# manuelbb-upb/Morbit.jl

Hardware: AMD Instinct MI355X
Metric: RBF build+solve+eval cycles/sec (higher is better)
Workload: dtype f64

## Files before the change

morbit.jl_amd/csrc/backsolve.hip:

```cpp
#include "common.hpp"

namespace mrbf {

namespace bsolve {

constexpr int NB = 128, NTHR = 512;
typedef double v2d __attribute__((ext_vector_type(2)));
typedef double v4d __attribute__((ext_vector_type(4)));
typedef __attribute__((address_space(1))) unsigned gu32;
typedef __attribute__((address_space(1))) double gf64;
typedef __attribute__((address_space(1))) v2d gv2d;

template <int KB>
struct Shared {
    double xs[2][KB][NB];
    int ok;
};

__global__ __launch_bounds__(256) void premul_kernel(const double *__restrict__ L, int64_t lda, const double *__restrict__ linv_all,
                                                     double *__restrict__ Mbuf, int nb, unsigned *__restrict__ flags, int nflags,
                                                     unsigned long long *__restrict__ xb, int nxb) {
    for (int e = blockIdx.x * 256 + threadIdx.x; e < nflags; e += gridDim.x * 256) flags[e] = 0u;
    for (int e = blockIdx.x * 256 + threadIdx.x; e < nxb; e += gridDim.x * 256) xb[e] = ~0ull;
    const int slab = blockIdx.x & 3, t = (blockIdx.x >> 2) & 1, j = blockIdx.x >> 3;
    const int i = j + 1 + t;
    if (i >= nb) return;
    const double *A = L + (int64_t)i * NB + (int64_t)j * NB * lda;
    const double *B = linv_all + (size_t)j * NB * NB;
    double *M = Mbuf + ((size_t)j * 2 + t) * NB * NB;
    const int lane = threadIdx.x & 63, wave = threadIdx.x >> 6, l15 = lane & 15, l4 = lane >> 4;
    const int i0 = 32 * wave, j0 = 32 * slab;
    v4d acc[2][2];
#pragma unroll
    for (int a = 0; a < 2; ++a)
#pragma unroll
        for (int b = 0; b < 2; ++b) acc[a][b] = (v4d){0.0, 0.0, 0.0, 0.0};
    const double *pa = A + (i0 + l15) + (int64_t)(j0 + l4) * lda;
    const double *pb = B + (j0 + l4) + (int64_t)(j0 + l15) * NB;
    constexpr int UK = 8;
    double fa0[2][UK], fa1[2][UK], fb0[2][UK], fb1[2][UK];
    auto burst = [&](int buf) {
#pragma unroll
        for (int u = 0; u < UK; ++u) {
            fa0[buf][u] = pa[(int64_t)4 * u * lda];
            fa1[buf][u] = pa[(int64_t)4 * u * lda + 16];
            fb0[buf][u] = pb[4 * u];
            fb1[buf][u] = pb[4 * u + 16 * NB];
        }
        pa += (int64_t)4 * UK * lda;
        pb += 4 * UK;
    };
    auto mma = [&](int buf) {
#pragma unroll
        for (int u = 0; u < UK; ++u) {
            acc[0][0] = __builtin_amdgcn_mfma_f64_16x16x4f64(fa0[buf][u], fb0[buf][u], acc[0][0], 0, 0, 0);
            acc[0][1] = __builtin_amdgcn_mfma_f64_16x16x4f64(fa0[buf][u], fb1[buf][u], acc[0][1], 0, 0, 0);
            acc[1][0] = __builtin_amdgcn_mfma_f64_16x16x4f64(fa1[buf][u], fb0[buf][u], acc[1][0], 0, 0, 0);
            acc[1][1] = __builtin_amdgcn_mfma_f64_16x16x4f64(fa1[buf][u], fb1[buf][u], acc[1][1], 0, 0, 0);
        }
    };
    const int nburst = (NB - j0) / (4 * UK);
    burst(0);
    for (int b = 0; b < nburst; b += 2) {
        if (b + 1 < nburst) burst(1);
        mma(0);
        if (b + 1 >= nburst) break;
        if (b + 2 < nburst) burst(0);
        mma(1);
    }
#pragma unroll
    for (int a = 0; a < 2; ++a)
#pragma unroll
        for (int b = 0; b < 2; ++b)
#pragma unroll
            for (int r = 0; r < 4; ++r) M[(i0 + 16 * a + l4 + 4 * r) + (size_t)(j0 + 16 * b + l15) * NB] = acc[a][b][r];
}

__device__ __forceinline__ void load_tile(const double *__restrict__ T, int64_t ldt, v2d (&r)[2][8]) {
    const int lane = threadIdx.x & 63, w = threadIdx.x >> 6;
    const double *p = T + (int64_t)(16 * w + 2 * (lane >> 3)) * ldt + 2 * (lane & 7);
#pragma unroll
    for (int cc = 0; cc < 2; ++cc)
#pragma unroll
        for (int u = 0; u < 8; ++u) r[cc][u] = *(const gv2d *)(p + cc * ldt + 16 * u);
}

template <int N>
__device__ __forceinline__ double shl_lanes(double v) {
    const long long b = __double_as_longlong(v);
    const int lo = __builtin_amdgcn_update_dpp((int)b, (int)b, 0x100 + N, 0xf, 0xf, false);
    const int hi = __builtin_amdgcn_update_dpp((int)(b >> 32), (int)(b >> 32), 0x100 + N, 0xf, 0xf, false);
    return __longlong_as_double(((long long)hi << 32) | (unsigned)lo);
}

template <int KB>
__device__ __forceinline__ void tile_dot(const double (*xs)[NB], const v2d (&r)[2][8], double (&out)[2][KB]) {
    const int q = threadIdx.x & 7;
    double acc[2][KB];
#pragma unroll
    for (int cc = 0; cc < 2; ++cc)
#pragma unroll
        for (int l = 0; l < KB; ++l) acc[cc][l] = 0.0;
#pragma unroll
    for (int u = 0; u < 8; ++u) {
#pragma unroll
        for (int l = 0; l < KB; ++l) {
            const v2d x = *(const v2d *)&xs[l][16 * u + 2 * q];
#pragma unroll
            for (int cc = 0; cc < 2; ++cc) acc[cc][l] = fma(r[cc][u][1], x[1], fma(r[cc][u][0], x[0], acc[cc][l]));
        }
    }
#pragma unroll
    for (int cc = 0; cc < 2; ++cc)
#pragma unroll
        for (int l = 0; l < KB; ++l) {
            double v = acc[cc][l];
            v += shl_lanes<4>(v);
            v += shl_lanes<2>(v);
            v += shl_lanes<1>(v);
            out[cc][l] = v;
        }
}

template <int KB>
__device__ __forceinline__ void await_block(Shared<KB> &sh, double (*xs)[NB], const double *glob, int i, double spec, int backoff,
                                            unsigned *abortw, unsigned epoch, unsigned long long spin_ticks, int *status, int code) {
    const int tid = threadIdx.x;
    if (tid >= KB * NB) return;
    const gf64 *src = (const gf64 *)&glob[((size_t)i * KB + tid / NB) * NB + (tid % NB)];
    double v = spec;
    if (__double_as_longlong(v) == -1ll) v = __hip_atomic_load(src, __ATOMIC_RELAXED, __HIP_MEMORY_SCOPE_AGENT);
    unsigned spins = 0;
    unsigned long long t0 = 0;
    while (__double_as_longlong(v) == -1ll) {
        if ((++spins & 63u) == 0u) {
            if (__hip_atomic_load((const gu32 *)abortw, __ATOMIC_RELAXED, __HIP_MEMORY_SCOPE_AGENT) != 0u) {
                sh.ok = 0;
                break;
            }
            const unsigned long long now = wall_clock64();
            if (t0 == 0) t0 = now;
            if (now - t0 > spin_ticks) {
                __hip_atomic_store((gu32 *)abortw, epoch, __ATOMIC_RELAXED, __HIP_MEMORY_SCOPE_AGENT);
                *(__attribute__((address_space(1))) int *)status = code + (i & 0xff);
                sh.ok = 0;
                break;
            }
        }
        for (int b = 0; b < backoff; ++b) __builtin_amdgcn_s_sleep(8);
        v = __hip_atomic_load(src, __ATOMIC_RELAXED, __HIP_MEMORY_SCOPE_AGENT);
    }
    xs[tid / NB][tid % NB] = v;
}

__device__ __forceinline__ void lds_barrier() { asm volatile("s_waitcnt lgkmcnt(0)\n\ts_barrier" ::: "memory"); }

__device__ __forceinline__ void publish(double *dst, v2d v) {
    if (__double_as_longlong(v[0]) == -1ll) v[0] = __longlong_as_double(0x7ff8000000000000ll);
    if (__double_as_longlong(v[1]) == -1ll) v[1] = __longlong_as_double(0x7ff8000000000000ll);
    asm volatile("global_store_dwordx4 %0, %1, off sc1" ::"v"(dst), "v"(v) : "memory");
}

template <int KB>
__global__ __launch_bounds__(NTHR, 1) void backsolve_persistent_kernel(const double *__restrict__ L, int64_t lda, const double *__restrict__ linv_all,
                                                                        const double *__restrict__ Mbuf, double *__restrict__ Y, int64_t ldy, int k0,
                                                                        int nb, unsigned *flags, unsigned epoch, unsigned long long spin_ticks,
                                                                        int *status, int fault, double *__restrict__ xb, double *__restrict__ zb,
                                                                        long long *stamps) {
    __shared__ __attribute__((aligned(16))) Shared<KB> sh;
    const int p = (int)blockIdx.x >> 1;
    const bool finisher = blockIdx.x & 1;
    const int j = nb - 1 - p, tid = threadIdx.x;
    const int lane = tid & 63, col = 16 * (tid >> 6) + 2 * (lane >> 3), q = lane & 7;
    unsigned *abortw = flags + (size_t)nb * 32;
    const int na = nb - 1 - j, npm = na < 2 ? na : 2, npl = na - npm;
    if (tid == 0) sh.ok = 1;
    __syncthreads();
    const double fillv = __longlong_as_double(-1ll);
    if (!finisher) {
        double w[2][KB];
#pragma unroll
        for (int cc = 0; cc < 2; ++cc)
#pragma unroll
            for (int l = 0; l < KB; ++l) w[cc][l] = *(const gf64 *)&Y[(int64_t)(k0 + l) * ldy + (int64_t)j * NB + col + cc];
        const int nst = npl + 1;
        auto fetch = [&](int s, v2d(&r)[2][8]) {
            const double *src = s < npl ? L + (int64_t)(nb - 1 - s) * NB + (int64_t)j * NB * lda : linv_all + (size_t)j * NB * NB;
            load_tile(src, s < npl ? lda : (int64_t)NB, r);
        };
        auto look = [&](int s) {
            const int i = nb - 1 - (s < npl ? s : (npl > 0 ? npl - 1 : 0));
            const int e = tid < KB * NB ? tid : 0;
            return __hip_atomic_load((const gf64 *)&xb[((size_t)i * KB + e / NB) * NB + (e % NB)], __ATOMIC_RELAXED, __HIP_MEMORY_SCOPE_AGENT);
        };
        double spec = fillv, spec2 = fillv;
        auto step = [&](int s, const v2d(&r)[2][8]) -> bool {
            double(*xs)[NB] = sh.xs[s & 1];
            if (s < npl) {
                const int i = nb - 1 - s;
                const int backoff = (i - j - 3) < 24 ? (i - j - 3) : 24;
                await_block<KB>(sh, xs, xb, i, spec, backoff, abortw, epoch, spin_ticks, status, 0x700);
                if (stamps && tid == 0 && s == npl - 1) stamps[256 * 5 + j * 4 + 0] = (long long)wall_clock64();
            } else if (q == 0) {
#pragma unroll
                for (int l = 0; l < KB; ++l) *(v2d *)&xs[l][col] = (v2d){w[0][l], w[1][l]};
            }
            spec = spec2;
            spec2 = look(s + 2);
            if (s + 2 >= npl) spec2 = fillv;
            lds_barrier();
            if (!sh.ok) return false;
            double dsum[2][KB];
            tile_dot<KB>(xs, r, dsum);
#pragma unroll
            for (int cc = 0; cc < 2; ++cc)
#pragma unroll
                for (int l = 0; l < KB; ++l) w[cc][l] = s == npl ? dsum[cc][l] : w[cc][l] - dsum[cc][l];
            return true;
        };
        v2d t0[2][8], t1[2][8], t2[2][8];
        const int o = (3 - nst % 3) % 3, G = (nst + o) / 3;
        if (0 - o >= 0) fetch(0 - o, t0);
        if (1 - o >= 0) fetch(1 - o, t1);
        fetch(2 - o, t2);
        spec = look(0);
        if (npl == 0) spec = fillv;
        spec2 = look(1);
        if (npl <= 1) spec2 = fillv;
        int g = 0;
        if (G >= 2) {
            const int s = -o;
            if (s >= 0 && !step(s, t0)) return;
            fetch(s + 3, t0);
            if (s + 1 >= 0 && !step(s + 1, t1)) return;
            fetch(s + 4, t1);
            if (!step(s + 2, t2)) return;
            fetch(s + 5, t2);
            g = 1;
        }
        for (; g < G - 1; ++g) {
            const int s = 3 * g - o;
            if (!step(s, t0)) return;
            fetch(s + 3, t0);
            if (!step(s + 1, t1)) return;
            fetch(s + 4, t1);
            if (!step(s + 2, t2)) return;
            fetch(s + 5, t2);
        }
        {
            const int s = 3 * (G - 1) - o;
            if (s >= 0 && !step(s, t0)) return;
            if (s + 1 >= 0 && !step(s + 1, t1)) return;
            if (!step(s + 2, t2)) return;
        }
        if (stamps && tid == 0) stamps[256 * 5 + j * 4 + 1] = (long long)wall_clock64();
        if (q == 0) {
#pragma unroll
            for (int l = 0; l < KB; ++l) publish(&zb[((size_t)j * KB + l) * NB + col], (v2d){w[0][l], w[1][l]});
        }
        return;
    }
    v2d tm2[2][8], tm1[2][8];
    if (npm == 2) load_tile(Mbuf + ((size_t)j * 2 + 1) * NB * NB, NB, tm2);
    if (npm >= 1) load_tile(Mbuf + (size_t)j * 2 * NB * NB, NB, tm1);
    double acc[2][KB];
#pragma unroll
    for (int cc = 0; cc < 2; ++cc)
#pragma unroll
        for (int l = 0; l < KB; ++l) acc[cc][l] = 0.0;
    if (npm == 2) {
        await_block<KB>(sh, sh.xs[0], xb, j + 2, fillv, 1, abortw, epoch, spin_ticks, status, 0x700);
        lds_barrier();
        if (!sh.ok) return;
        if (stamps && tid == 0) stamps[256 * 5 + j * 4 + 3] = (long long)wall_clock64();
        tile_dot<KB>(sh.xs[0], tm2, acc);
    }
    v2d zj[KB];
    if (q == 0) {
        unsigned spins = 0;
        unsigned long long t0 = 0;
#pragma unroll
        for (int l = 0; l < KB; ++l) {
            const double *src = &zb[((size_t)j * KB + l) * NB + col];
            while (true) {
                v2d v;
                asm volatile("global_load_dwordx4 %0, %1, off sc1\n\ts_waitcnt vmcnt(0)" : "=v"(v) : "v"(src) : "memory");
                if (__double_as_longlong(v[0]) != -1ll && __double_as_longlong(v[1]) != -1ll) {
                    zj[l] = v;
                    break;
                }
                if ((++spins & 63u) == 0u) {
                    if (__hip_atomic_load((const gu32 *)abortw, __ATOMIC_RELAXED, __HIP_MEMORY_SCOPE_AGENT) != 0u) {
                        sh.ok = 0;
                        break;
                    }
                    const unsigned long long now = wall_clock64();
                    if (t0 == 0) t0 = now;
                    if (now - t0 > spin_ticks) {
                        __hip_atomic_store((gu32 *)abortw, epoch, __ATOMIC_RELAXED, __HIP_MEMORY_SCOPE_AGENT);
                        *(__attribute__((address_space(1))) int *)status = 0x600 + (j & 0xff);
                        sh.ok = 0;
                        break;
                    }
                }
                __builtin_amdgcn_s_sleep(2);
            }
            if (!sh.ok) break;
        }
    }
    if (stamps && tid == 0) stamps[256 * 5 + j * 4 + 2] = (long long)wall_clock64();
    double last[2][KB];
#pragma unroll
    for (int cc = 0; cc < 2; ++cc)
#pragma unroll
        for (int l = 0; l < KB; ++l) last[cc][l] = 0.0;
    if (npm >= 1) {
        if (stamps && tid == 0) stamps[256 * 4 + j] = (long long)wall_clock64();
        await_block<KB>(sh, sh.xs[1], xb, j + 1, fillv, 0, abortw, epoch, spin_ticks, status, 0x700);
        if (stamps && tid == 0) stamps[j * 4 + 0] = (long long)wall_clock64();
        lds_barrier();
        if (!sh.ok) return;
        if (stamps && tid == 0) stamps[j * 4 + 1] = (long long)wall_clock64();
        tile_dot<KB>(sh.xs[1], tm1, last);
    } else {
        lds_barrier();
        if (!sh.ok) return;
    }
    if ((fault & 1) && j == nb / 2) return;
    if (stamps && tid == 0) stamps[j * 4 + 2] = (long long)wall_clock64();
    if (q == 0) {
#pragma unroll
        for (int l = 0; l < KB; ++l) {
            const v2d v = (v2d){(zj[l][0] - acc[0][l]) - last[0][l], (zj[l][1] - acc[1][l]) - last[1][l]};
            publish(&xb[((size_t)j * KB + l) * NB + col], v);
            *(v2d *)&Y[(int64_t)(k0 + l) * ldy + (int64_t)j * NB + col] = v;
        }
    }
}

}

int backsolve_blocked(mrbf_ctx *ctx, int64_t npad, const double *L, int64_t lda, const double *linv_all, double *Y, int64_t ldy, int k);

int backsolve_persistent(mrbf_ctx *ctx, int64_t npad, const double *L, int64_t lda, const double *linv_all, double *Y, int64_t ldy, int k,
                         int *status) {
    using namespace bsolve;
    const int nb = (int)(npad / NB);
    static const int force_old = mrbf_env("MRBF_BACKSOLVE_LAUNCHES") ? atoi(mrbf_env("MRBF_BACKSOLVE_LAUNCHES")) : 0;
    const int ncu = ctx->ncu;
    if (force_old || nb < 3 || nb > ncu || (lda & 1) || (reinterpret_cast<uintptr_t>(L) & 15))
        return backsolve_blocked(ctx, npad, L, lda, linv_all, Y, ldy, k);
    unsigned *flags;
    MRBF_TRY(get_buf(ctx, S_BSOLVE_FLAGS, (size_t)(nb + 1) * 32, &flags));
    const unsigned long long spin_ticks = (unsigned long long)std::max(1, ctx->spin_ms) * 100000ull;
    const int fault = (ctx->debug_fault & 2) ? 1 : 0;
    double *xb, *Mbuf;
    MRBF_TRY(get_buf(ctx, S_BSOLVE_X, (size_t)2 * nb * 4 * NB, &xb));
    MRBF_TRY(get_buf(ctx, S_BSOLVE_M, (size_t)nb * 2 * NB * NB, &Mbuf));
    hipLaunchKernelGGL(premul_kernel, dim3((unsigned)(8 * (nb - 1))), dim3(256), 0, ctx->stream, L, lda, linv_all, Mbuf, nb, flags, (nb + 1) * 32,
                       reinterpret_cast<unsigned long long *>(xb), 2 * nb * 4 * NB);
    static const bool want_stamps = mrbf_env("MRBF_BSOLVE_STAMPS") && atoi(mrbf_env("MRBF_BSOLVE_STAMPS")) != 0;
    long long *stamps = nullptr;
    if (want_stamps) {
        static long long *dbg = nullptr;
        if (!dbg) MRBF_HIP(ctx, hipMalloc(&dbg, (size_t)256 * 9 * sizeof(long long)));
        stamps = dbg;
    }
    unsigned epoch = 0;
    for (int k0 = 0; k0 < k; k0 += 4) {
        const int kb = std::min(4, k - k0);
        ++epoch;
        if (k0 > 0) MRBF_HIP(ctx, hipMemsetAsync(xb, 0xff, (size_t)2 * nb * 4 * NB * sizeof(double), ctx->stream));
#define MRBF_BSP(KBV)                                                                                                          \
    hipLaunchKernelGGL((backsolve_persistent_kernel<KBV>), dim3((unsigned)(2 * nb)), dim3(NTHR), 0, ctx->stream, L, lda, linv_all, Mbuf, Y, ldy, k0, nb, \
                       flags, epoch, spin_ticks, status, fault, xb, xb + (size_t)nb * 4 * NB, stamps)
        if (kb == 1) MRBF_BSP(1); else if (kb == 2) MRBF_BSP(2); else if (kb == 3) MRBF_BSP(3); else MRBF_BSP(4);
#undef MRBF_BSP
    }
    MRBF_HIP(ctx, hipGetLastError());
    if (want_stamps) {
        std::vector<long long> h((size_t)256 * 9);
        MRBF_HIP(ctx, hipMemcpyAsync(h.data(), stamps, h.size() * sizeof(long long), hipMemcpyDeviceToHost, ctx->stream));
        MRBF_HIP(ctx, hipStreamSynchronize(ctx->stream));
        double seen = 0, bar = 0, dot = 0, hop = 0, late = 0;
        int cnt = 0;
        for (int j = 1; j + 2 < nb; ++j) {
            seen += (double)(h[j * 4 + 0] - h[(j + 1) * 4 + 2]);
            bar += (double)(h[j * 4 + 1] - h[j * 4 + 0]);
            dot += (double)(h[j * 4 + 2] - h[j * 4 + 1]);
            hop += (double)(h[j * 4 + 2] - h[(j + 1) * 4 + 2]);
            late += (double)(h[256 * 4 + j] - h[(j + 1) * 4 + 2]);
            ++cnt;
        }
        double a3 = 0, zt = 0, zs = 0, x2 = 0;
        int c2 = 0;
        for (int j = 2; j + 4 < nb; ++j) {
            const long long *S = &h[256 * 5 + j * 4];
            a3 += (double)(S[0] - h[(j + 3) * 4 + 2]);
            zt += (double)(S[1] - S[0]);
            zs += (double)(S[2] - S[1]);
            x2 += (double)(S[3] - h[(j + 2) * 4 + 2]);
            ++c2;
        }
        fprintf(stderr, "[backsolve stamps] streamer: x_{j+3} seen %.2f us after its publication, z_j published %.2f us later, finisher has z_j %.2f us "
                "later; finisher past x_{j+2} %.2f us after that block's publication\n", a3 / c2 / 100.0, zt / c2 / 100.0, zs / c2 / 100.0, x2 / c2 / 100.0);
        fprintf(stderr, "[backsolve stamps] nb %d: publish -> seen %.2f us, seen -> barrier %.2f us, barrier -> publish %.2f us, step %.2f us; "
                "the finisher starts polling %.2f us after the publication\n", nb, seen / cnt / 100.0, bar / cnt / 100.0, dot / cnt / 100.0,
                hop / cnt / 100.0, late / cnt / 100.0);
    }
    return 0;
}

}
```

morbit.jl_amd/csrc/common.hpp:

```cpp
#pragma once
#include <hip/hip_runtime.h>
#include <rocblas/rocblas.h>
#include <rocsolver/rocsolver.h>

#include <cmath>
#include <cstdlib>
#include <cstdint>
#include <cstdio>
#include <cstring>
#include <map>
#include <string>
#include <vector>

#include "../../include/mrbf.h"
#include "descent_problem.hpp"
#include "model_pool.hpp"

namespace mrbf {

struct KP {
    int kid;
    double a, b;
    double a2;
    double sgn;
    int fast;
    int ik;
    double phi0;
};
KP make_kp(int kid, double a, double b);
inline bool kp_nonsmooth(const KP &p) { return (p.kid == MRBF_CUBIC && p.a == 1.0) || (p.kid == MRBF_THIN_PLATE_SPLINE && p.ik == 1); }
int cpd_order(int kid, double a, double b);
inline int poly_dim(int d, int deg) { return deg < 0 ? 0 : (deg == 0 ? 1 : d + 1); }

enum Slot {
    S_XC = 0, S_SQ, S_MEAN, S_PHI, S_PI, S_Q1, S_W1, S_G, S_R, S_TAU, S_RHS, S_T1, S_T2, S_IPIV, S_INFO,
    S_STAGE_A, S_STAGE_B, S_STAGE_C, S_STAGE_D, S_EVAL_E, S_EVAL_A, S_EVAL_J, S_EVAL_SA, S_EVAL_XC, S_EVAL_XSQ,
    S_OUT_A, S_OUT_B, S_CHOL_WS, S_MISC, S_MEGA_JOBS, S_MEGA_FLAGS, S_MEGA_WQ, S_MEGA_IT, S_BSOLVE_FLAGS, S_MEGA_TRACE, S_MEGA_JLOG,
    S_T1W, S_PS_STATE, S_PS_STAT, S_PS_POLISH, S_BSOLVE_X, S_V0, S_QR_INV, S_DIAG_SCR, S_SMALL_WS, S_SMALL_DESC, S_SMALL_FLAGS, S_MEGA_STAT, S_BSOLVE_M, S_SMALL_CL, S_GW_PART, S_GW_RS, S_GW_GP, S_GW_M, S_CHECK_SCAL, S_TAIL_PART, S_PS_RANK, S_SD_IN, S_SD_OUT, S_SD_WS, S_NS_IN, S_NS_OUT, S_NS_WS, S_SD_STEP, S_SD_BATCH, S_AFF_BATCH, S_NS_BATCH, S_R4_BATCH, S_DB_BOX, S_DB_GATHER, S_DB_WS, S_SMALL_LU, S_EVAL_BATCH, S_HESS_WS, S_HESS_OUT, S_NSLOTS
};
}

namespace mrbf {
namespace mega {
struct Edge {
    int head, tail_c0, srows_edge, pstream_edge;
    int shalf, sh_head, sh_tail_c0;
    int tfull1;
    int xhalf;
};
struct TableParams {
    int slack, slack_chain, first, win, srows, half_cols, tail_half, tail_half_w, chainq;
    Edge edge;
};
constexpr bool operator==(const TableParams &a, const TableParams &b) {
    return a.slack == b.slack && a.slack_chain == b.slack_chain && a.first == b.first && a.win == b.win && a.srows == b.srows &&
           a.half_cols == b.half_cols && a.tail_half == b.tail_half && a.tail_half_w == b.tail_half_w && a.chainq == b.chainq &&
           a.edge.head == b.edge.head && a.edge.tail_c0 == b.edge.tail_c0 && a.edge.srows_edge == b.edge.srows_edge &&
           a.edge.pstream_edge == b.edge.pstream_edge && a.edge.shalf == b.edge.shalf && a.edge.sh_head == b.edge.sh_head &&
           a.edge.sh_tail_c0 == b.edge.sh_tail_c0 && a.edge.tfull1 == b.edge.tfull1 && a.edge.xhalf == b.edge.xhalf;
}
struct Knobs {
    int grid = 512, dedicated = 64, look = 2, quiet = 1, slack = 3, half_cols = 0, first_window = 1, wbias = 4, xhalf = 1, chainq = 0, cboost = 12, panel_dma = 1;
    int min = 256, max = 32768;
    int chain = 0, slack_chain = 0, win = 0, pstream = 0, srows = 0;
    int shalf = -1, shalf_head = -1, head = -1, tail = -1, reserve = -1, tail_half = -1, tail_half_w = -1, xchain = -1, quiet_tail = -1;
    int tfull = -1;
};
}
struct MegaTables {
    int nt, mt;
    mega::TableParams params;
    void *block, *jobs, *wq;
    int npanel, nbulk, nchainjobs, nwin;
    unsigned long long stamp;
};
struct PotrfOpts {
    int impl = 0;
    bool any_size = false;
    int xreal = 0;
    bool info_clean = false;
};
struct EvalHints {
    bool population = false;
    bool check_call = false;
    const double *pre_xq = nullptr;
};
}

struct mrbf_ctx {
    int device = 0;
    int ncu = 256;
    hipStream_t own_stream = nullptr;
    hipStream_t stream = nullptr;
    rocblas_handle blas = nullptr;
    mrbf::Buf slots[mrbf::S_NSLOTS];
    hipEvent_t ev[8] = {};
    hipStream_t panel_stream = nullptr;
    hipEvent_t evx[4] = {};
    hipStream_t bulk_stream = nullptr;
    int bulk_masked = 0;
    int bulk_grid = 384;
    mrbf::mega::Knobs mega;
    std::string err;
    std::vector<mrbf::Buf> model_pool;
    int gram_mode = 0, residual = 1, force_path = 0, chol_impl = 0, eval_impl = 0, timing = 1, diag_impl = 0, chol_window = 0;
    int spin_ms = 1000, debug_fault = 0;
    unsigned long long *mega_stat_dev = nullptr;
    long mega_stat_shape = 0;
    int mega_stat_pending = 0;
    char *pin_base = nullptr;
    size_t pin_off = 0;
    bool pin_armed = false;
    struct PinOut {
        void *user;
        const void *pin;
        size_t bytes;
    };
    std::vector<PinOut> pin_out;
    unsigned long long *hpin = nullptr;
    float last_device_ms = 0.f;
    int slow_launches = 0;
    int small_nc = 4;
    int small_cluster_ok = 0;
    int small_timeouts = 0;
    int small_fit_max_n = 512;
    int small_lu = 0;
    int live_models = 0, live_round4 = 0;
    int live_dbs = 0;
    unsigned ps_rank_epoch = 0;
    int ps_multi_off = 0;
    std::map<long, float> mega_best_ms;
    std::vector<mrbf::MegaTables> mega_tables;
    unsigned long long mega_table_clock = 0;
};

struct mrbf_model {
    int64_t n = 0, npad = 0;
    int d = 0, dpad = 0, k = 0, q = 0, deg = -1;
    mrbf::KP kp{};
    double *C = nullptr;
    double *Xc = nullptr;
    double *sq = nullptr;
    double *mean = nullptr;
    double *W = nullptr;
    double *Wc = nullptr;
    double *lam = nullptr;
    void *block = nullptr;
    size_t block_bytes = 0;
    mrbf_ctx *owner = nullptr;
    mrbf::ModelSlab *slab = nullptr;
};

struct mrbf_db {
    mrbf_ctx *ctx = nullptr;
    int d = 0, k = 0;
    int64_t n = 0, cap = 0;
    double *sites = nullptr, *values = nullptr;
};

namespace mrbf {

int fail(mrbf_ctx *ctx, int code, const char *fmt, ...);
#define MRBF_HIP(ctx, call)                                                                                  \
    do {                                                                                                      \
        hipError_t e__ = (call);                                                                              \
        if (e__ != hipSuccess)                                                                                \
            return mrbf::fail(ctx, e__ == hipErrorOutOfMemory ? MRBF_ENOMEM : MRBF_EHIP, "%s: %s (%s:%d)", #call, \
                              hipGetErrorString(e__), __FILE__, __LINE__);                                    \
    } while (0)
#define MRBF_BLAS(ctx, call)                                                                                 \
    do {                                                                                                      \
        rocblas_status s__ = (call);                                                                          \
        if (s__ != rocblas_status_success)                                                                    \
            return mrbf::fail(ctx, MRBF_EBLAS, "%s: rocblas status %d (%s:%d)", #call, (int)s__, __FILE__, __LINE__); \
    } while (0)
#define MRBF_TRY(call)             \
    do {                           \
        int rc__ = (call);         \
        if (rc__ != 0) return rc__; \
    } while (0)

int get_buf(mrbf_ctx *ctx, Slot s, size_t bytes, void **out);
template <class T>
inline int get_buf(mrbf_ctx *ctx, Slot s, size_t count, T **out) {
    return get_buf(ctx, s, count * sizeof(T), (void **)out);
}
bool is_device_ptr(const void *p);
int db_reserve(mrbf_ctx *ctx, mrbf_db *db, int64_t needed);
int stage_in(mrbf_ctx *ctx, Slot s, const double *user, size_t count, const double **dev);
int stage_out(mrbf_ctx *ctx, Slot s, double *user, size_t count, double **dev);
int finish_out(mrbf_ctx *ctx, double *user, const double *dev, size_t count);
int input_fetch(mrbf_ctx *ctx, const double *src, size_t count, double *dst);
int input_view(mrbf_ctx *ctx, const double *user, size_t count, double *&arena, const double **dev);
int output_put(mrbf_ctx *ctx, double *dst, const double *src, size_t count);
int fetch_linear_rows(mrbf_ctx *ctx, const mrbf_ps_problem *prob, int d, double *A, double *b);
descent::Shape descent_shape(const mrbf_ps_problem *prob, const mrbf_model *const *models, int64_t n_starts,
                             std::vector<descent::SlotShape> &slots);
void pin_reset(mrbf_ctx *ctx);
void pin_flush(mrbf_ctx *ctx);
void pin_discard(mrbf_ctx *ctx);
char *pin_take(mrbf_ctx *ctx, size_t bytes);
struct PinGuard {
    mrbf_ctx *ctx;
    bool flushed = false;
    explicit PinGuard(mrbf_ctx *c) : ctx(c) { pin_reset(c); }
    void flush() {
        pin_flush(ctx);
        flushed = true;
    }
    ~PinGuard() {
        if (!flushed) pin_discard(ctx);
    }
    PinGuard(const PinGuard &) = delete;
    PinGuard &operator=(const PinGuard &) = delete;
};
enum HpinSlot : int {
    HPIN_FIT_FLAGS = 0,
    HPIN_FIT_SCAL = 4,
    HPIN_SMALL_FLAGS = 8,
    HPIN_SMALL_SCAL = 12,
    HPIN_SMALL_CHK = 16,
    HPIN_RESIDUAL = 20,
    HPIN_R4_COUNT = 24,
    HPIN_MEGA_STAT = 63,
};

inline int64_t round_up(int64_t x, int64_t m) { return (x + m - 1) / m * m; }

inline const char *mrbf_env(const char *name) {
    const char *gate = std::getenv("MRBF_EXPERIMENTS");
    if (!gate || std::atoi(gate) == 0) return nullptr;
    return std::getenv(name);
}

int launch_center_pad(mrbf_ctx *ctx, const double *X, int64_t n, int d, const double *mean_or_null, double *mean_out,
                      double *Xc, int64_t npad, int dpad, double *sq);
int launch_poly_matrix(mrbf_ctx *ctx, const double *C, int64_t n, int d, int q, double *Pi, int64_t ldpi);
int launch_transpose(mrbf_ctx *ctx, const double *in, int64_t rows, int64_t cols, double *out);
int launch_gram(mrbf_ctx *ctx, int mode, const double *C, const double *Xc, const double *sq, int64_t n, int64_t npad,
                int d, int dpad, const KP &kp, double *Phi, int64_t ld);
int launch_cross_gram(mrbf_ctx *ctx, const double *X, int64_t m, const double *C, int64_t n, int d, const KP &kp, double *K);
bool gram_w_applies(const mrbf_ctx *ctx, const mrbf_model *M);
int launch_gram_w(mrbf_ctx *ctx, const mrbf_model *M, double *Phi, int64_t ld, double **Wpart_out, double **rspart_out, int *nseg_out);
int launch_projection_small(mrbf_ctx *ctx, const mrbf_model *M, const double *Wpart, const double *rspart, int nseg, const double *linv,
                            const double *Q1, double *W1, double *G, double *scal, int *flags, int K2, int skip, double *PA, double *PB,
                            double *v0);
int eval_model(mrbf_ctx *ctx, const mrbf_model *M, int64_t m, const double *Xdev, double *vals_dev, double *jac_dev,
               mrbf_eval_info *info, EvalHints hints = {});
int hess_call(mrbf_ctx *ctx, const mrbf_model *M, int64_t m, const double *X, const std::vector<int32_t> &rows, double *hess_out,
              mrbf_hess_info *info, int64_t stage_bytes);
int potrf_blocked_tall(mrbf_ctx *ctx, int64_t ncols, int64_t mrows, double *A, int64_t lda, int *dinfo, double *linv_all, PotrfOpts opt = {});
int potrf_mega_tall(mrbf_ctx *ctx, int64_t ncols, int64_t mrows, double *A, int64_t lda, int *dinfo, double *linv_all, PotrfOpts opt = {});
mega::Knobs mega_knobs_from_env();
int potrf_lower(mrbf_ctx *ctx, int impl, int64_t n, double *A, int64_t lda, int *info_host);
int fit_model(mrbf_ctx *ctx, mrbf_model *M, const double *Ydev, mrbf_fit_info *info);
int build_model_shell(mrbf_ctx *ctx, int64_t n, int d, int k, const double *Cdev, int kid, double a, double b, int deg,
                      mrbf_model **out);
void destroy_model(mrbf_ctx *ctx, mrbf_model *M);
void model_set_dims(mrbf_model *M, int64_t n, int d, int k, int kid, double a, double b, int deg);
size_t model_block_layout(const mrbf_model *M, size_t off[7]);
void model_carve(mrbf_model *M, char *base, const size_t off[7]);
int model_block_acquire(mrbf_ctx *ctx, size_t total, void **p, size_t *bytes);
void model_block_release(mrbf_ctx *ctx, void *p, size_t bytes, bool slab = false);
int fit_check(mrbf_ctx *ctx, mrbf_model *M, const double *Y, mrbf_fit_info *info);
int mega_collect_stat(mrbf_ctx *ctx);
int mega_stat_enqueue(mrbf_ctx *ctx);
int mega_stat_finish(mrbf_ctx *ctx);

}
```

morbit.jl_amd/csrc/eval_fused.hip:

```cpp
#include <type_traits>

#include "radial.hpp"
#ifndef MRBF_EVAL_DBG
#define MRBF_EVAL_DBG 0
#endif
#include "small.hpp"

namespace mrbf {

typedef double v4d __attribute__((ext_vector_type(4)));
typedef double v2d __attribute__((ext_vector_type(2)));

constexpr int EQ = 64;
constexpr int EC = 64;

template <int KID, bool FAST, int KOUT, bool JAC, bool FINAL>
__global__ __launch_bounds__(256, 2) void eval_fused_kernel(EvalDesc one, const EvalDesc *__restrict__ many, int l0) {
    constexpr int D = 64, DT = D / 16, LDC = D + 2;
    __shared__ __attribute__((aligned(16))) double Cs[EC * LDC];
    __shared__ double Ws[KOUT * EC];
    __shared__ double Sq[EC];
    const EvalDesc &E = many ? many[blockIdx.z] : one;
    if (many && ((int64_t)blockIdx.x * EQ >= E.mpad || (int)blockIdx.y >= E.nsplit)) return;
    const double *__restrict__ Xq = E.Xq;
    const double *__restrict__ Cc = E.Cc;
    const double *__restrict__ csq = E.csq;
    const double *__restrict__ Wc = E.Wc;
    const int64_t npad = E.npad, mpad = E.mpad;
    const int tiles_per_split = E.tiles_per_split;
    const KP kp = E.kp;
    const int tid = threadIdx.x, lane = tid & 63, wave = tid >> 6;
    const int l15 = lane & 15, l4 = lane >> 4;
    const int64_t q0 = (int64_t)blockIdx.x * EQ;
    const int split = blockIdx.y;
    const int64_t qrow = q0 + wave * 16 + l15;

    double xb[D / 4];
#pragma unroll
    for (int s = 0; s < D / 4; ++s) xb[s] = Xq[qrow * D + 4 * s + l4];
    const double xs = E.xsq[qrow];

    v4d JT[KOUT][DT];
    double vsum[KOUT], sasum[KOUT];
#pragma unroll
    for (int l = 0; l < KOUT; ++l) {
        vsum[l] = 0.0;
        sasum[l] = 0.0;
#pragma unroll
        for (int t = 0; t < DT; ++t) JT[l][t] = (v4d){0.0, 0.0, 0.0, 0.0};
    }

    const int64_t c_begin = (int64_t)split * tiles_per_split * EC;
    const int ntiles_all = E.ntiles;
    const int nsub = __builtin_amdgcn_readfirstlane(E.nsub);
    const int my_tiles = min(tiles_per_split, ntiles_all - split * tiles_per_split);
    constexpr int NLD = 2 * DT;
    v2d stg[NLD];
    auto load_tile = [&](int64_t c0) {
        const v2d *src = reinterpret_cast<const v2d *>(Cc + c0 * D);
#pragma unroll
        for (int u = 0; u < NLD; ++u) stg[u] = src[tid + 256 * u];
    };
    auto store_tile = [&]() {
#pragma unroll
        for (int u = 0; u < NLD; ++u) {
            const int e = (tid + 256 * u) * 2;
            const int row = e / D, col = e % D;
            *(v2d *)&Cs[row * LDC + col] = stg[u];
        }
    };
    constexpr int NSC = ((KOUT + 1) * EC + 255) / 256;
    double stg_s[NSC];
    auto load_scalars = [&](int64_t c0) {
#pragma unroll
        for (int u = 0; u < NSC; ++u) {
            const int e = tid + 256 * u;
            if (e < EC)
                stg_s[u] = csq[c0 + e];
            else if (e < (KOUT + 1) * EC)
                stg_s[u] = Wc[(int64_t)(l0 + (e - EC) / EC) * npad + c0 + ((e - EC) % EC)];
        }
    };
    load_tile(c_begin);
    load_scalars(c_begin);
    for (int tile = 0; tile < my_tiles; ++tile) {
        const int64_t c0 = c_begin + (int64_t)tile * EC;
        __syncthreads();
        store_tile();
#pragma unroll
        for (int u = 0; u < NSC; ++u) {
            const int e = tid + 256 * u;
            if (e < EC)
                Sq[e] = stg_s[u];
            else if (e < (KOUT + 1) * EC)
                Ws[e - EC] = stg_s[u];
        }
        __syncthreads();
        if (tile + 1 < my_tiles) {
            load_tile(c0 + EC);
            load_scalars(c0 + EC);
        }
#pragma unroll
        for (int ct = 0; ct < 4; ++ct) {
            if ((int)(c0 >> 4) + ct >= nsub) break;
            v4d S = {0.0, 0.0, 0.0, 0.0};
            const double *crow = &Cs[(16 * ct + l15) * LDC + l4];
#pragma unroll
            for (int s = 0; s < D / 4; ++s) S = __builtin_amdgcn_mfma_f64_16x16x4f64(crow[4 * s], xb[s], S, 0, 0, 0);
            v4d Aw[KOUT];
#pragma unroll
            for (int r = 0; r < 4; ++r) {
                const int c = 16 * ct + l4 + 4 * r;
                double s2 = fma(-2.0, S[r], xs + Sq[c]);
                s2 = s2 > 0.0 ? s2 : 0.0;
                double phi, psi;
                rbf_phi_psi_t<KID, FAST>(s2, kp, phi, psi);
#pragma unroll
                for (int l = 0; l < KOUT; ++l) {
                    const double w = Ws[l * EC + c];
                    vsum[l] = fma(w, phi, vsum[l]);
                    if constexpr (JAC) {
                        const double a = w * psi;
                        sasum[l] += a;
                        Aw[l][r] = a;
                    }
                }
            }
            if (JAC) {
#pragma unroll
                for (int tt = 0; tt < DT; ++tt) {
#pragma unroll
                    for (int s = 0; s < 4; ++s) {
                        const double cop = Cs[(16 * ct + 4 * s + l4) * LDC + 16 * tt + l15];
#pragma unroll
                        for (int l = 0; l < KOUT; ++l) JT[l][tt] = __builtin_amdgcn_mfma_f64_16x16x4f64(cop, Aw[l][s], JT[l][tt], 0, 0, 0);
                    }
                }
            }
        }
    }
#pragma unroll
    for (int l = 0; l < KOUT; ++l) {
        vsum[l] += __shfl_xor(vsum[l], 16);
        vsum[l] += __shfl_xor(vsum[l], 32);
        sasum[l] += __shfl_xor(sasum[l], 16);
        sasum[l] += __shfl_xor(sasum[l], 32);
    }
    if constexpr (!FINAL) {
        double *__restrict__ vpart = E.vpart, *__restrict__ sapart = E.sapart, *__restrict__ gpart = E.gpart;
        if (l4 == 0) {
#pragma unroll
            for (int l = 0; l < KOUT; ++l) {
                vpart[((int64_t)split * mpad + qrow) * KOUT + l] = vsum[l];
                sapart[((int64_t)split * mpad + qrow) * KOUT + l] = sasum[l];
            }
        }
        if (JAC) {
            __syncthreads();
            double *T = Cs + wave * 16 * LDC;
#pragma unroll
            for (int l = 0; l < KOUT; ++l) {
#pragma unroll
                for (int tt = 0; tt < DT; ++tt)
#pragma unroll
                    for (int r = 0; r < 4; ++r) T[l15 * LDC + 16 * tt + l4 + 4 * r] = JT[l][tt][r];
                __syncthreads();
                for (int e = lane; e < 16 * D; e += 64) {
                    const int qq = e / D, t = e % D;
                    gpart[(((int64_t)split * mpad + q0 + wave * 16 + qq) * KOUT + l) * D + t] = T[qq * LDC + t];
                }
                __syncthreads();
            }
        }
    } else {
        const int d = E.d, k = E.k, q = E.q;
        const int64_t m = E.m;
        const double *__restrict__ lam = E.lam;
        double *__restrict__ vals = E.vals;
        double *__restrict__ jac = E.jac;
        if (vals) {
            __syncthreads();
            double *Lm = Cs;
            for (int e = tid; e < (KOUT + 1) * D; e += 256) {
                const int l = e / D, t = e % D;
                Lm[e] = (t < d && q > 1) ? (l < KOUT ? (l0 + l < k ? lam[(int64_t)(t + 1) * k + l0 + l] : 0.0) : E.mean[t]) : 0.0;
            }
            __syncthreads();
#pragma unroll
            for (int l = 0; l < KOUT; ++l) {
                double acc = 0.0, cst = 0.0;
#pragma unroll
                for (int s = 0; s < D / 4; ++s) acc = fma(Lm[l * D + 4 * s + l4], xb[s], acc);
                for (int t = lane; t < D; t += 64) cst = fma(Lm[l * D + t], Lm[KOUT * D + t], cst);
                for (int off = 32; off > 0; off >>= 1) cst += __shfl_xor(cst, off);
                acc += __shfl_xor(acc, 16);
                acc += __shfl_xor(acc, 32);
                double v = vsum[l];
                if (q > 0 && l0 + l < k) v += lam[l0 + l];
                if (q > 1) v += acc + cst;
                if (l4 == 0 && qrow < m && l0 + l < k) vals[qrow * k + l0 + l] = v;
            }
        }
        if (JAC && jac) {
            __syncthreads();
            double *T = Cs + wave * 16 * LDC;
            double *SA = Ws;
#pragma unroll
            for (int l = 0; l < KOUT; ++l)
                if (l4 == 0) SA[l * EQ + wave * 16 + l15] = sasum[l];
#pragma unroll
            for (int l = 0; l < KOUT; ++l) {
#pragma unroll
                for (int tt = 0; tt < DT; ++tt)
#pragma unroll
                    for (int r = 0; r < 4; ++r) T[l15 * LDC + 16 * tt + l4 + 4 * r] = JT[l][tt][r];
                __syncthreads();
                if (l0 + l < k) {
                    for (int e = lane; e < 16 * D; e += 64) {
                        const int qq = e / D, t = e % D;
                        const int64_t row = q0 + wave * 16 + qq;
                        if (row < m && t < d) {
                            double v = fma(SA[l * EQ + wave * 16 + qq], Xq[row * D + t], -T[qq * LDC + t]);
                            if (q > 1) v += lam[(int64_t)(t + 1) * k + l0 + l];
                            jac[row * (int64_t)k * d + (int64_t)t * k + l0 + l] = v;
                        }
                    }
                }
                __syncthreads();
            }
        }
    }
}

template <int KID, bool FAST, int KOUT, int H, int ECT, bool JAC, bool FINAL>
__global__ __launch_bounds__(512, 2) void eval_fused_split_kernel(EvalDesc one, const EvalDesc *__restrict__ many, int l0) {
    constexpr int D = 2 * H, LDC = D + 2, LDT = 65, NCT = ECT / 16, HT = H / 16;
    static_assert(8 * 16 * LDT <= ECT * LDC + 2 * 8 * 256, "epilogue transpose area");
    __shared__ __attribute__((aligned(16))) double smem[ECT * LDC + 2 * 8 * 256];
    double *Cs = smem;
    double *Sx = smem + ECT * LDC;
    __shared__ double Ws[KOUT * ECT];
    __shared__ double Sq[ECT];
    const EvalDesc &E = many ? many[blockIdx.z] : one;
    if (many && ((int64_t)blockIdx.x * EQ >= E.mpad || (int)blockIdx.y >= E.nsplit)) return;
    const double *__restrict__ Xq = E.Xq;
    const double *__restrict__ Cc = E.Cc;
    const double *__restrict__ csq = E.csq;
    const double *__restrict__ Wc = E.Wc;
    const int64_t npad = E.npad, mpad = E.mpad;
    const KP kp = E.kp;
    const int tid = threadIdx.x, lane = tid & 63, wave = tid >> 6, grp = wave >> 2, qw = wave & 3;
    const int l15 = lane & 15, l4 = lane >> 4;
    const int64_t q0 = (int64_t)blockIdx.x * EQ;
    const int split = blockIdx.y;
    const int64_t qrow = q0 + qw * 16 + l15;
    double xb[H / 4];
#pragma unroll
    for (int s = 0; s < H / 4; ++s) xb[s] = Xq[qrow * D + H * grp + 4 * s + l4];
    const double xs = E.xsq[qrow];
    v4d JT[KOUT][HT];
    double vsum[KOUT], sasum[KOUT];
#pragma unroll
    for (int l = 0; l < KOUT; ++l) {
        vsum[l] = 0.0;
        sasum[l] = 0.0;
#pragma unroll
        for (int t = 0; t < HT; ++t) JT[l][t] = (v4d){0.0, 0.0, 0.0, 0.0};
    }
    const int64_t c_begin = (int64_t)split * E.tiles_per_split * EC;
    const int ntiles_all = E.ntiles;
    const int nsub = __builtin_amdgcn_readfirstlane(E.nsub);
    const int my_tiles = min(E.tiles_per_split, ntiles_all - split * E.tiles_per_split) * (EC / ECT);
    constexpr int NLD = ECT * D / 2 / 512;
    v2d stg[NLD];
    auto load_tile = [&](int64_t c0) {
        const v2d *src = reinterpret_cast<const v2d *>(Cc + c0 * D);
#pragma unroll
        for (int u = 0; u < NLD; ++u) stg[u] = src[tid + 512 * u];
    };
    auto store_tile = [&]() {
#pragma unroll
        for (int u = 0; u < NLD; ++u) {
            const int e = (tid + 512 * u) * 2;
            const int row = e / D, col = e % D;
            *(v2d *)&Cs[row * LDC + col] = stg[u];
        }
    };
    static_assert((KOUT + 1) * ECT <= 512, "one staged scalar per thread");
    double stg_w = 0.0;
    auto load_scalars = [&](int64_t c0) {
        if (tid < ECT)
            stg_w = csq[c0 + tid];
        else if (tid < (KOUT + 1) * ECT)
            stg_w = Wc[(int64_t)(l0 + (tid - ECT) / ECT) * npad + c0 + ((tid - ECT) % ECT)];
    };
    load_tile(c_begin);
    load_scalars(c_begin);
    for (int tile = 0; tile < my_tiles; ++tile) {
        const int64_t c0 = c_begin + (int64_t)tile * ECT;
        __syncthreads();
        store_tile();
        if (tid < ECT)
            Sq[tid] = stg_w;
        else if (tid < (KOUT + 1) * ECT)
            Ws[tid - ECT] = stg_w;
        __syncthreads();
        if (tile + 1 < my_tiles) {
            load_tile(c0 + ECT);
            load_scalars(c0 + ECT);
        }
#pragma unroll
        for (int ct = 0; ct < NCT; ++ct) {
            if ((int)(c0 >> 4) + ct >= nsub) break;
            v4d Sp = {0.0, 0.0, 0.0, 0.0};
            const double *crow = &Cs[(16 * ct + l15) * LDC + H * grp + l4];
#pragma unroll
            for (int s = 0; s < H / 4; ++s) Sp = __builtin_amdgcn_mfma_f64_16x16x4f64(crow[4 * s], xb[s], Sp, 0, 0, 0);
            const int par = (tile * NCT + ct) & 1;
            double *mine = &Sx[(par * 8 + wave) * 256];
            const double *theirs = &Sx[(par * 8 + (wave ^ 4)) * 256];
#pragma unroll
            for (int r = 0; r < 4; ++r) mine[r * 64 + lane] = Sp[r];
            __syncthreads();
            v4d S;
#pragma unroll
            for (int r = 0; r < 4; ++r) {
                const double o = theirs[r * 64 + lane];
                S[r] = grp == 0 ? Sp[r] + o : o + Sp[r];
            }
            v4d Aw[KOUT];
#pragma unroll
            for (int r = 0; r < 4; ++r) {
                const int c = 16 * ct + l4 + 4 * r;
                double s2 = fma(-2.0, S[r], xs + Sq[c]);
                s2 = s2 > 0.0 ? s2 : 0.0;
                double phi, psi;
                rbf_phi_psi_t<KID, FAST>(s2, kp, phi, psi);
#pragma unroll
                for (int l = 0; l < KOUT; ++l) {
                    const double w = Ws[l * ECT + c];
                    vsum[l] = fma(w, phi, vsum[l]);
                    if constexpr (JAC) {
                        const double a = w * psi;
                        sasum[l] += a;
                        Aw[l][r] = a;
                    }
                }
            }
            if (JAC && !(MRBF_EVAL_DBG & 2)) {
#pragma unroll
                for (int tt = 0; tt < HT; ++tt) {
#pragma unroll
                    for (int s = 0; s < 4; ++s) {
                        const double cop = Cs[(16 * ct + 4 * s + l4) * LDC + H * grp + 16 * tt + l15];
#pragma unroll
                        for (int l = 0; l < KOUT; ++l) JT[l][tt] = __builtin_amdgcn_mfma_f64_16x16x4f64(cop, Aw[l][s], JT[l][tt], 0, 0, 0);
                    }
                }
            }
        }
    }
#pragma unroll
    for (int l = 0; l < KOUT; ++l) {
        vsum[l] += __shfl_xor(vsum[l], 16);
        vsum[l] += __shfl_xor(vsum[l], 32);
        sasum[l] += __shfl_xor(sasum[l], 16);
        sasum[l] += __shfl_xor(sasum[l], 32);
    }
    const int d = E.d, k = E.k, q = E.q;
    const int64_t m = E.m;
    const double *__restrict__ lam = E.lam;
    double *__restrict__ vals = E.vals;
    double *__restrict__ jac = E.jac;
    if constexpr (!FINAL) {
        if (l4 == 0 && grp == 0) {
#pragma unroll
            for (int l = 0; l < KOUT; ++l) {
                E.vpart[((int64_t)split * mpad + qrow) * KOUT + l] = vsum[l];
                E.sapart[((int64_t)split * mpad + qrow) * KOUT + l] = sasum[l];
            }
        }
    } else if (vals) {
        __syncthreads();
        double *Lm = Sx;
        double *Pp = Sx + (KOUT + 1) * D;
        for (int e = tid; e < (KOUT + 1) * D; e += 512) {
            const int l = e / D, t = e % D;
            Lm[e] = (t < d && q > 1) ? (l < KOUT ? (l0 + l < k ? lam[(int64_t)(t + 1) * k + l0 + l] : 0.0) : E.mean[t]) : 0.0;
        }
        __syncthreads();
        double accs[KOUT], csts[KOUT];
#pragma unroll
        for (int l = 0; l < KOUT; ++l) {
            double acc = 0.0, cst = 0.0;
#pragma unroll
            for (int s = 0; s < H / 4; ++s) acc = fma(Lm[l * D + H * grp + 4 * s + l4], xb[s], acc);
            for (int t = lane; t < D; t += 64) cst = fma(Lm[l * D + t], Lm[KOUT * D + t], cst);
            for (int off = 32; off > 0; off >>= 1) cst += __shfl_xor(cst, off);
            acc += __shfl_xor(acc, 16);
            acc += __shfl_xor(acc, 32);
            accs[l] = acc;
            csts[l] = cst;
            if (grp == 1 && l4 == 0) Pp[l * EQ + qw * 16 + l15] = acc;
        }
        __syncthreads();
        if (grp == 0 && l4 == 0 && qrow < m) {
#pragma unroll
            for (int l = 0; l < KOUT; ++l) {
                if (l0 + l >= k) continue;
                double v = vsum[l];
                if (q > 0) v += lam[l0 + l];
                if (q > 1) v += (accs[l] + Pp[l * EQ + qw * 16 + l15]) + csts[l];
                vals[qrow * k + l0 + l] = v;
            }
        }
    }
    if (JAC && (!FINAL || jac) && !(MRBF_EVAL_DBG & 1)) {
        __syncthreads();
        double *T = smem + wave * 16 * LDT;
        double *SA = Ws;
        __shared__ double SAs[KOUT * EQ];
        SA = SAs;
        if (FINAL && grp == 0 && l4 == 0) {
#pragma unroll
            for (int l = 0; l < KOUT; ++l) SA[l * EQ + qw * 16 + l15] = sasum[l];
        }
        bool paired = false;
        if constexpr (FINAL && KOUT == 2)
            paired = (k & 1) == 0 && (l0 & 1) == 0 && l0 + 1 < k && !(MRBF_EVAL_DBG & 64) &&
                     (((uintptr_t)jac | (uintptr_t)lam) & 15) == 0;
        if constexpr (FINAL && KOUT == 2) {
            if (paired) {
                constexpr int LDP = 33;
                static_assert(8 * 2 * 16 * LDP <= ECT * LDC + 2 * 8 * 256, "paired Jacobian transpose area");
                double *T2 = smem + wave * (2 * 16 * LDP);
#pragma unroll
                for (int hq = 0; hq < H / 32; ++hq) {
#pragma unroll
                    for (int l = 0; l < 2; ++l)
#pragma unroll
                        for (int tt = 0; tt < 2; ++tt)
#pragma unroll
                            for (int r = 0; r < 4; ++r) T2[(l * 16 + l15) * LDP + 16 * tt + l4 + 4 * r] = JT[l][2 * hq + tt][r];
                    __syncthreads();
                    for (int e = lane; e < 16 * 32; e += 64) {
                        const int qq = e >> 5, t = e & 31, col = H * grp + 32 * hq + t;
                        const int64_t row = q0 + qw * 16 + qq;
                        if (row < m && col < d) {
                            const double x = Xq[row * D + col];
                            v2d v;
                            v.x = fma(SA[qw * 16 + qq], x, -T2[qq * LDP + t]);
                            v.y = fma(SA[EQ + qw * 16 + qq], x, -T2[(16 + qq) * LDP + t]);
                            if (q > 1) {
                                const v2d lm = *(const v2d *)&lam[(int64_t)(col + 1) * k + l0];
                                v.x += lm.x;
                                v.y += lm.y;
                            }
                            *(v2d *)&jac[row * (int64_t)k * d + (int64_t)col * k + l0] = v;
                        }
                    }
                    __syncthreads();
                }
            }
        }
#pragma unroll
        for (int l = 0; l < KOUT; ++l) {
            if (paired) break;
#pragma unroll
            for (int hc = 0; hc < H / 64; ++hc) {
#pragma unroll
                for (int tt = 0; tt < 4; ++tt)
#pragma unroll
                    for (int r = 0; r < 4; ++r) T[l15 * LDT + 16 * tt + l4 + 4 * r] = JT[l][4 * hc + tt][r];
                __syncthreads();
                for (int e = lane; e < 16 * 64; e += 64) {
                    const int qq = e / 64, t = e % 64, col = H * grp + 64 * hc + t;
                    const int64_t row = q0 + qw * 16 + qq;
                    if constexpr (!FINAL) {
                        E.gpart[(((int64_t)split * mpad + row) * KOUT + l) * D + col] = T[qq * LDT + t];
                    } else {
                        if (l0 + l < k && row < m && col < d) {
                            double v = fma(SA[l * EQ + qw * 16 + qq], Xq[row * D + col], -T[qq * LDT + t]);
                            if (q > 1) v += lam[(int64_t)(col + 1) * k + l0 + l];
                            jac[row * (int64_t)k * d + (int64_t)col * k + l0 + l] = v;
                        }
                    }
                }
                __syncthreads();
            }
        }
    }
}

template <int KID, bool FAST, int KOUT>
__global__ __launch_bounds__(512, 1) void eval_vals256_kernel(EvalDesc one, const EvalDesc *__restrict__ many, int l0) {
    constexpr int D = 256, H = 128, ECT = 32, LDC = D + 2, NCT = ECT / 16, EQW = 128;
    __shared__ __attribute__((aligned(16))) double Cs[ECT * LDC];
    __shared__ double Ws[KOUT * ECT];
    __shared__ double Sq[ECT];
    const EvalDesc &E = many ? many[blockIdx.z] : one;
    if (many && ((int64_t)blockIdx.x * EQW >= E.mpad || (int)blockIdx.y >= E.nsplit)) return;
    const double *__restrict__ Xq = E.Xq;
    const double *__restrict__ Cc = E.Cc;
    const double *__restrict__ csq = E.csq;
    const double *__restrict__ Wc = E.Wc;
    const int64_t npad = E.npad, mpad = E.mpad;
    const KP kp = E.kp;
    const int tid = threadIdx.x, lane = tid & 63, wave = tid >> 6;
    const int l15 = lane & 15, l4 = lane >> 4;
    const int64_t q0 = (int64_t)blockIdx.x * EQW;
    const int split = blockIdx.y;
    const int64_t qrow = q0 + wave * 16 + l15;
    const bool qin = qrow < mpad;
    const int64_t qld = qin ? qrow : mpad - 1;
    double xb[D / 4];
#pragma unroll
    for (int s = 0; s < D / 4; ++s) xb[s] = Xq[qld * D + 4 * s + l4];
    const double xs = E.xsq[qld];
    double vsum[KOUT];
#pragma unroll
    for (int l = 0; l < KOUT; ++l) vsum[l] = 0.0;
    const int64_t c_begin = (int64_t)split * E.tiles_per_split * EC;
    const int nsub = __builtin_amdgcn_readfirstlane(E.nsub);
    const int my_tiles = min(E.tiles_per_split, E.ntiles - split * E.tiles_per_split) * (EC / ECT);
    constexpr int NLD = ECT * D / 2 / 512;
    v2d stg[NLD];
    auto load_tile = [&](int64_t c0) {
        const v2d *src = reinterpret_cast<const v2d *>(Cc + c0 * D);
#pragma unroll
        for (int u = 0; u < NLD; ++u) stg[u] = src[tid + 512 * u];
    };
    static_assert((KOUT + 1) * ECT <= 512, "one staged scalar per thread");
    double stg_w = 0.0;
    auto load_scalars = [&](int64_t c0) {
        if (tid < ECT)
            stg_w = csq[c0 + tid];
        else if (tid < (KOUT + 1) * ECT)
            stg_w = Wc[(int64_t)(l0 + (tid - ECT) / ECT) * npad + c0 + ((tid - ECT) % ECT)];
    };
    load_tile(c_begin);
    load_scalars(c_begin);
    for (int tile = 0; tile < my_tiles; ++tile) {
        const int64_t c0 = c_begin + (int64_t)tile * ECT;
        __syncthreads();
#pragma unroll
        for (int u = 0; u < NLD; ++u) {
            const int e = (tid + 512 * u) * 2;
            *(v2d *)&Cs[(e / D) * LDC + (e % D)] = stg[u];
        }
        if (tid < ECT)
            Sq[tid] = stg_w;
        else if (tid < (KOUT + 1) * ECT)
            Ws[tid - ECT] = stg_w;
        __syncthreads();
        if (tile + 1 < my_tiles) {
            load_tile(c0 + ECT);
            load_scalars(c0 + ECT);
        }
#pragma unroll
        for (int ct = 0; ct < NCT; ++ct) {
            if ((int)(c0 >> 4) + ct >= nsub) break;
            v4d S0 = {0.0, 0.0, 0.0, 0.0}, S1 = {0.0, 0.0, 0.0, 0.0};
            const double *crow = &Cs[(16 * ct + l15) * LDC + l4];
#pragma unroll
            for (int s = 0; s < H / 4; ++s) {
                S0 = __builtin_amdgcn_mfma_f64_16x16x4f64(crow[4 * s], xb[s], S0, 0, 0, 0);
                S1 = __builtin_amdgcn_mfma_f64_16x16x4f64(crow[H + 4 * s], xb[H / 4 + s], S1, 0, 0, 0);
            }
#pragma unroll
            for (int r = 0; r < 4; ++r) {
                const int c = 16 * ct + l4 + 4 * r;
                double s2 = fma(-2.0, S0[r] + S1[r], xs + Sq[c]);
                s2 = s2 > 0.0 ? s2 : 0.0;
                double phi, psi;
                rbf_phi_psi_t<KID, FAST>(s2, kp, phi, psi);
#pragma unroll
                for (int l = 0; l < KOUT; ++l) vsum[l] = fma(Ws[l * ECT + c], phi, vsum[l]);
            }
        }
    }
#pragma unroll
    for (int l = 0; l < KOUT; ++l) {
        vsum[l] += __shfl_xor(vsum[l], 16);
        vsum[l] += __shfl_xor(vsum[l], 32);
    }
    if (l4 == 0 && qin) {
#pragma unroll
        for (int l = 0; l < KOUT; ++l) {
            E.vpart[((int64_t)split * mpad + qrow) * KOUT + l] = vsum[l];
            E.sapart[((int64_t)split * mpad + qrow) * KOUT + l] = 0.0;
        }
    }
}

template <int KOUT>
__global__ __launch_bounds__(128) void eval_combine_kernel(EvalDesc one, const EvalDesc *__restrict__ many, int l0, int D) {
    const EvalDesc &E = many ? many[blockIdx.y] : one;
    const int64_t p = blockIdx.x, m = E.m, mpad = E.mpad;
    if (p >= m) return;
    const double *__restrict__ vpart = E.vpart, *__restrict__ sapart = E.sapart, *__restrict__ gpart = E.gpart;
    const double *__restrict__ Xq = E.Xq, *__restrict__ Xorig = E.X, *__restrict__ lam = E.lam;
    double *__restrict__ vals = E.vals, *__restrict__ jac = E.jac;
    const int nsplit = E.nsplit, d = E.d, k = E.k, q = E.q;
    __shared__ double sa[KOUT], sv[KOUT];
    __shared__ double pdot[KOUT][128];
    const int tid = threadIdx.x;
    if (tid < KOUT && l0 + tid < k) {
        double v = 0.0, a = 0.0;
        for (int s0 = 0; s0 < nsplit; s0 += 8) {
            double xv[8], xa[8];
#pragma unroll
            for (int u = 0; u < 8; ++u) {
                xv[u] = s0 + u < nsplit ? vpart[((int64_t)(s0 + u) * mpad + p) * KOUT + tid] : 0.0;
                xa[u] = s0 + u < nsplit ? sapart[((int64_t)(s0 + u) * mpad + p) * KOUT + tid] : 0.0;
            }
#pragma unroll
            for (int u = 0; u < 8; ++u)
                if (s0 + u < nsplit) {
                    v += xv[u];
                    a += xa[u];
                }
        }
        sa[tid] = a;
        sv[tid] = v;
    }
    if (vals && q > 1) {
#pragma unroll
        for (int l = 0; l < KOUT; ++l) {
            double acc = 0.0;
            if (l0 + l < k)
                for (int t = tid; t < d; t += 128) acc = fma(lam[(int64_t)(t + 1) * k + l0 + l], Xorig[p * d + t], acc);
            pdot[l][tid] = acc;
        }
    }
    __syncthreads();
    if (vals && tid < KOUT && l0 + tid < k) {
        double v = sv[tid];
        if (q > 0) v += lam[l0 + tid];
        if (q > 1) {
            const int nt = d < 128 ? d : 128;
            double dsum = 0.0;
            for (int t = 0; t < nt; ++t) dsum += pdot[tid][t];
            v += dsum;
        }
        vals[p * k + l0 + tid] = v;
    }
    for (int e = tid; e < KOUT * d; e += blockDim.x) {
        const int l = e / d, t = e % d;
        if (l0 + l >= k) continue;
        double g = 0.0;
        for (int s0 = 0; s0 < nsplit; s0 += 8) {
            double x[8];
#pragma unroll
            for (int u = 0; u < 8; ++u) x[u] = s0 + u < nsplit ? gpart[(((int64_t)(s0 + u) * mpad + p) * KOUT + l) * D + t] : 0.0;
#pragma unroll
            for (int u = 0; u < 8; ++u)
                if (s0 + u < nsplit) g += x[u];
        }
        double v = fma(sa[l], Xq[p * D + t], -g);
        if (q > 1) v += lam[(int64_t)(t + 1) * k + l0 + l];
        jac[p * (int64_t)k * d + (int64_t)t * k + l0 + l] = v;
    }
}

template <int KOUT>
__global__ __launch_bounds__(256) void eval_combine_vals_kernel(EvalDesc one, const EvalDesc *__restrict__ many, int l0) {
    const EvalDesc &E = many ? many[blockIdx.y] : one;
    const int lane = threadIdx.x & 63, wave = threadIdx.x >> 6;
    const int64_t p = (int64_t)blockIdx.x * 4 + wave, m = E.m, mpad = E.mpad;
    const bool active = p < m;
    const double *__restrict__ vpart = E.vpart, *__restrict__ Xorig = E.X, *__restrict__ lam = E.lam;
    const int nsplit = E.nsplit, d = E.d, k = E.k, q = E.q;
    __shared__ double pdot[4][KOUT][128];
    double v = 0.0;
    if (active && lane < KOUT && l0 + lane < k) {
        for (int s0 = 0; s0 < nsplit; s0 += 8) {
            double x[8];
#pragma unroll
            for (int u = 0; u < 8; ++u) x[u] = s0 + u < nsplit ? vpart[((int64_t)(s0 + u) * mpad + p) * KOUT + lane] : 0.0;
#pragma unroll
            for (int u = 0; u < 8; ++u)
                if (s0 + u < nsplit) v += x[u];
        }
    }
    if (q > 1) {
#pragma unroll
        for (int l = 0; l < KOUT; ++l)
#pragma unroll
            for (int h = 0; h < 2; ++h) {
                const int t0 = lane + 64 * h;
                double acc = 0.0;
                if (active && l0 + l < k)
                    for (int t = t0; t < d; t += 128) acc = fma(lam[(int64_t)(t + 1) * k + l0 + l], Xorig[p * d + t], acc);
                pdot[wave][l][t0] = acc;
            }
    }
    __syncthreads();
    if (active && lane < KOUT && l0 + lane < k) {
        if (q > 0) v += lam[l0 + lane];
        if (q > 1) {
            const int nt = d < 128 ? d : 128;
            double dsum = 0.0;
            for (int t = 0; t < nt; ++t) dsum += pdot[wave][lane][t];
            v += dsum;
        }
        if (E.vals) E.vals[p * k + l0 + lane] = v;
    }
}

__global__ void center_pad_batch_kernel(const EvalDesc *__restrict__ many, int Dfixed) {
    const EvalDesc &E = many[blockIdx.y];
    const int D = Dfixed > 0 ? Dfixed : (E.d <= 64 ? 64 : 128);
    const int lane = threadIdx.x & 63;
    const int64_t row = (int64_t)blockIdx.x * (blockDim.x >> 6) + (threadIdx.x >> 6);
    if (row >= E.mpad) return;
    double s = 0.0;
    for (int t = lane; t < D; t += 64) {
        double v = 0.0;
        if (row < E.m && t < E.d) v = E.X[row * E.d + t] - E.mean[t];
        E.Xq[row * D + t] = v;
        s = fma(v, v, s);
    }
    for (int off = 32; off > 0; off >>= 1) s += __shfl_xor(s, off);
    if (lane == 0) E.xsq[row] = s;
}

int eval_nsplit(const mrbf_ctx *ctx, int64_t m, int ntiles, bool check_call, bool population) {
    const int64_t mpad = round_up(m, EQ);
    const int slots = 2 * ctx->ncu;
    const int64_t qtiles = mpad / EQ;
    constexpr int small_split = 8;
    const bool small_batch = !check_call && qtiles * 8 <= slots;
    if (ntiles >= 4 && ntiles <= 8 && small_batch) return std::min(small_split, ntiles);
    if (population && !check_call && ntiles >= 4 && ntiles <= 8 && qtiles * 2 <= slots) return (int)std::min<int64_t>(ntiles, slots / qtiles);
    if (ntiles <= 8) return 1;
    constexpr double comb_small = 0.1, comb = 0.75;
    int nsplit = 1;
    double best_cost = 1e300;
    for (int s = 1; s <= std::min(ntiles, 32); ++s) {
        const int tps_s = (ntiles + s - 1) / s;
        if ((int64_t)(s - 1) * tps_s >= ntiles) continue;
        const double rounds = std::ceil((double)(qtiles * s) / slots);
        const double cost = rounds * tps_s + (small_batch ? comb_small : comb) * s;
        if (cost < best_cost) {
            best_cost = cost;
            nsplit = s;
        }
    }
    const int force_split = mrbf_env("MRBF_EVAL_NSPLIT") ? atoi(mrbf_env("MRBF_EVAL_NSPLIT")) : 0;
    if (force_split > 0 && force_split <= ntiles && (int64_t)(force_split - 1) * ((ntiles + force_split - 1) / force_split) < ntiles)
        nsplit = force_split;
    return nsplit;
}

int outputs_per_pass(int k, int D, bool want_jac) { return (k < 2 || (D == 256 && want_jac)) ? 1 : 2; }

template <int KID, bool FAST, int KOUT, bool JAC, bool FINAL>
static int launch_pass(mrbf_ctx *ctx, int D, dim3 grid, dim3 cgrid, const EvalDesc &one, const EvalDesc *many, int l0) {
    hipStream_t st = ctx->stream;
    if (D == 64) {
        hipLaunchKernelGGL((eval_fused_kernel<KID, FAST, KOUT, JAC, FINAL>), grid, dim3(256), 0, st, one, many, l0);
    } else if (D == 128) {
        hipLaunchKernelGGL((eval_fused_split_kernel<KID, FAST, KOUT, 64, 64, JAC, FINAL>), grid, dim3(512), 0, st, one, many, l0);
    } else if constexpr (JAC && KOUT == 1) {
        hipLaunchKernelGGL((eval_fused_split_kernel<KID, FAST, 1, 128, 32, true, FINAL>), grid, dim3(512), 0, st, one, many, l0);
    } else if constexpr (JAC) {
        return fail(ctx, MRBF_EHIP, "eval_fused: a pass with Jacobians at D = 256 carries one output");
    } else if constexpr (FINAL) {
        hipLaunchKernelGGL((eval_fused_split_kernel<KID, FAST, KOUT, 128, 32, false, true>), grid, dim3(512), 0, st, one, many, l0);
    } else {
        hipLaunchKernelGGL((eval_vals256_kernel<KID, FAST, KOUT>), dim3((grid.x + 1) / 2, grid.y, grid.z), dim3(512), 0, st, one, many, l0);
    }
    if constexpr (!FINAL && JAC)
        hipLaunchKernelGGL(eval_combine_kernel<KOUT>, cgrid, dim3(128), 0, st, one, many, l0, D);
    else if constexpr (!FINAL)
        hipLaunchKernelGGL(eval_combine_vals_kernel<KOUT>, dim3((cgrid.x + 3) / 4, cgrid.y), dim3(256), 0, st, one, many, l0);
    return 0;
}

template <class F>
static int with_bool(bool b, F &&f) {
    return b ? f(std::true_type{}) : f(std::false_type{});
}

static int run_passes(mrbf_ctx *ctx, const KP &kp, int D, int k, bool want_jac, bool final_, dim3 grid, dim3 cgrid, const EvalDesc &one,
                      const EvalDesc *many) {
    const int KO = outputs_per_pass(k, D, want_jac);
    for (int l0 = 0; l0 < k; l0 += KO) {
        const bool two = std::min(KO, k - l0) == 2;
        MRBF_DISPATCH_KID(kp.kid, {
            constexpr bool HAS_FAST = KID == MRBF_MULTIQUADRIC || KID == MRBF_INV_MULTIQUADRIC || KID == MRBF_CUBIC;
            MRBF_TRY(with_bool(HAS_FAST && kp.fast, [&](auto fast) {
                return with_bool(two, [&](auto two_) {
                    return with_bool(want_jac, [&](auto jac) {
                        return with_bool(final_, [&](auto fin) {
                            return launch_pass<KID, HAS_FAST && decltype(fast)::value, decltype(two_)::value ? 2 : 1, decltype(jac)::value, decltype(fin)::value>(
                                ctx, D, grid, cgrid, one, many, l0);
                        });
                    });
                });
            }));
        });
    }
    MRBF_HIP(ctx, hipGetLastError());
    return 0;
}

int center_pad_batch(mrbf_ctx *ctx, const EvalDesc *dev_descs, int count, int64_t max_mpad) {
    if (count <= 0 || max_mpad <= 0) return 0;
    hipLaunchKernelGGL(center_pad_batch_kernel, dim3((unsigned)((max_mpad + 3) / 4), (unsigned)count), dim3(256), 0, ctx->stream, dev_descs, 0);
    MRBF_HIP(ctx, hipGetLastError());
    return 0;
}

constexpr int DIFF_CH = 256;

__device__ __forceinline__ void nonsmooth_phi_psi(const KP &p, double s, double &phi, double &psi) {
    if (s <= 0.0) {
        phi = 0.0;
        psi = 0.0;
    } else if (p.kid == MRBF_CUBIC) {
        const double r = sqrt(s);
        phi = p.sgn * r;
        psi = p.sgn / r;
    } else {
        const double lg = log(s);
        phi = p.sgn * s * (0.5 * lg);
        psi = p.sgn * (lg + 1.0);
    }
}

__global__ __launch_bounds__(256) void eval_diff_kernel(EvalDesc one, const EvalDesc *__restrict__ many, int want_jac) {
    extern __shared__ double dsm[];
    const EvalDesc &E = many ? many[blockIdx.y] : one;
    const int64_t p = blockIdx.x, n = E.n, npad = E.npad;
    if (p >= E.m) return;
    const int d = E.d, k = E.k, q = E.q;
    const double *__restrict__ C = E.C, *__restrict__ Wc = E.Wc, *__restrict__ lam = E.lam;
    double *__restrict__ vals = E.vals, *__restrict__ jac = want_jac ? E.jac : nullptr;
    const KP kp = E.kp;
    double *xs = dsm, *ph = dsm + d, *ps = ph + DIFF_CH;
    const int tid = threadIdx.x, lane = tid & 63, wave = tid >> 6;
    for (int t = tid; t < d; t += 256) xs[t] = E.X[p * d + t];
    __syncthreads();
    if (vals)
        for (int l = tid; l < k; l += 256) {
            double v = q > 0 ? lam[l] : 0.0;
            if (q > 1)
                for (int t = 0; t < d; ++t) v = fma(lam[(int64_t)(t + 1) * k + l], xs[t], v);
            vals[p * k + l] = v;
        }
    if (jac)
        for (int64_t e = tid; e < (int64_t)k * d; e += 256) jac[p * (int64_t)k * d + e] = q > 1 ? lam[k + e] : 0.0;
    for (int64_t c0 = 0; c0 < n; c0 += DIFF_CH) {
        const int nc = (int)min((int64_t)DIFF_CH, n - c0);
        __syncthreads();
        for (int ci = wave; ci < nc; ci += 4) {
            const double *cr = C + (c0 + ci) * d;
            double s = 0.0;
            for (int t = lane; t < d; t += 64) {
                const double df = xs[t] - cr[t];
                s = fma(df, df, s);
            }
            for (int off = 32; off > 0; off >>= 1) s += __shfl_xor(s, off);
            if (lane == 0) nonsmooth_phi_psi(kp, s, ph[ci], ps[ci]);
        }
        __syncthreads();
        if (vals)
            for (int l = tid; l < k; l += 256) {
                const double *w = Wc + (int64_t)l * npad + c0;
                double v = vals[p * k + l];
                for (int ci = 0; ci < nc; ++ci) v = fma(w[ci], ph[ci], v);
                vals[p * k + l] = v;
            }
        if (jac)
            for (int64_t e = tid; e < (int64_t)k * d; e += 256) {
                const int t = (int)(e / k), l = (int)(e % k);
                const double *w = Wc + (int64_t)l * npad + c0;
                const double x = xs[t];
                double g = jac[p * (int64_t)k * d + e];
                for (int ci = 0; ci < nc; ++ci) g = fma(w[ci] * ps[ci], x - C[(c0 + ci) * d + t], g);
                jac[p * (int64_t)k * d + e] = g;
            }
    }
}

static int launch_eval_diff(mrbf_ctx *ctx, int64_t max_m, int max_d, const EvalDesc &one, const EvalDesc *many, int count, bool want_jac) {
    if (max_m <= 0 || count <= 0) return 0;
    const size_t lds = ((size_t)max_d + 2 * DIFF_CH) * sizeof(double);
    hipLaunchKernelGGL(eval_diff_kernel, dim3((unsigned)max_m, (unsigned)count), dim3(256), lds, ctx->stream, one, many, want_jac ? 1 : 0);
    MRBF_HIP(ctx, hipGetLastError());
    return 0;
}

int eval_diff(mrbf_ctx *ctx, const mrbf_model *M, int64_t m, const double *X, double *vals, double *jac) {
    EvalDesc E;
    std::memset(&E, 0, sizeof(E));
    eval_desc_model(E, M, m, 1);
    E.X = X;
    E.vals = vals;
    E.jac = jac;
    return launch_eval_diff(ctx, m, M->d, E, nullptr, 1, jac != nullptr);
}

int eval_fused_batch(mrbf_ctx *ctx, const KP &kp, int D, int k, bool want_jac, const EvalDesc *host_descs, const EvalDesc *dev_descs, int count,
                     bool centred) {
    if (count <= 0) return 0;
    if (D != 64 && D != 128 && D != 256) return fail(ctx, MRBF_EHIP, "eval_fused_batch needs dpad in {64, 128, 256}");
    for (int p = 0; p < count; ++p)
        if (kp_nonsmooth(host_descs[p].kp) != kp_nonsmooth(kp))
            return fail(ctx, MRBF_EHIP, "eval_fused_batch: descriptor %d and its group differ in kp_nonsmooth", p);
    if (kp_nonsmooth(kp)) {
        int64_t max_m = 0;
        for (int p = 0; p < count; ++p) max_m = std::max(max_m, host_descs[p].m);
        return launch_eval_diff(ctx, max_m, D, host_descs[0], dev_descs, count, want_jac);
    }
    int64_t max_mpad = 0, max_m = 0;
    int max_split = 1;
    for (int p = 0; p < count; ++p) {
        max_mpad = std::max(max_mpad, host_descs[p].mpad);
        max_m = std::max(max_m, host_descs[p].m);
        max_split = std::max(max_split, host_descs[p].nsplit);
    }
    if (max_split > 1)
        for (int p = 0; p < count; ++p)
            if (host_descs[p].nsplit == 1 && host_descs[p].m > 0)
                return fail(ctx, MRBF_EHIP, "eval_fused_batch: descriptor %d is unsplit in a group that splits the centre range", p);
    if (!centred)
        hipLaunchKernelGGL(center_pad_batch_kernel, dim3((unsigned)((max_mpad + 3) / 4), (unsigned)count), dim3(256), 0, ctx->stream, dev_descs, D);
    dim3 grid((unsigned)(max_mpad / EQ), (unsigned)max_split, (unsigned)count);
    dim3 cgrid((unsigned)max_m, (unsigned)count);
    return run_passes(ctx, kp, D, k, want_jac, max_split == 1, grid, cgrid, host_descs[0], dev_descs);
}

int eval_fused(mrbf_ctx *ctx, const mrbf_model *M, int64_t m, const double *X, double *vals, double *jac, mrbf_eval_info *info, EvalHints hints) {
    const int d = M->d, k = M->k;
    const int D = (M->dpad <= 64) ? 64 : (M->dpad <= 128 ? 128 : 256);
    if (M->dpad > 256) return fail(ctx, MRBF_EHIP, "eval_fused supports d <= 256");
    if (D != M->dpad) return fail(ctx, MRBF_EHIP, "eval_fused needs dpad in {64, 128, 256} (got %d)", M->dpad);
    const int64_t mpad = round_up(m, EQ);
    const int ntiles = (int)((M->n + EC - 1) / EC);
    const int nsplit = eval_nsplit(ctx, m, ntiles, hints.check_call, hints.population);
    const int KO = outputs_per_pass(k, D, jac != nullptr);
    EvalDesc E;
    std::memset(&E, 0, sizeof(E));
    eval_desc_model(E, M, m, nsplit);
    E.X = X;
    MRBF_TRY(get_buf(ctx, S_EVAL_XC, (size_t)mpad * D, &E.Xq));
    MRBF_TRY(get_buf(ctx, S_EVAL_XSQ, (size_t)mpad, &E.xsq));
    if (nsplit > 1) {
        MRBF_TRY(get_buf(ctx, S_EVAL_SA, (size_t)nsplit * mpad * KO * 2, &E.vpart));
        E.sapart = E.vpart + (size_t)nsplit * mpad * KO;
        if (jac) MRBF_TRY(get_buf(ctx, S_EVAL_J, (size_t)nsplit * mpad * KO * D, &E.gpart));
    }
    E.vals = vals;
    E.jac = jac;
    const bool timing = ctx->timing && info;
    if (timing) MRBF_HIP(ctx, hipEventRecord(ctx->ev[4], ctx->stream));
    if (!(hints.pre_xq && hints.pre_xq == E.Xq)) MRBF_TRY(launch_center_pad(ctx, X, m, d, M->mean, nullptr, E.Xq, mpad, D, E.xsq));
    dim3 grid((unsigned)(mpad / EQ), (unsigned)nsplit);
    MRBF_TRY(run_passes(ctx, M->kp, D, k, jac != nullptr, nsplit == 1, grid, dim3((unsigned)m), E, nullptr));
    if (timing) {
        MRBF_HIP(ctx, hipEventRecord(ctx->ev[7], ctx->stream));
        MRBF_HIP(ctx, hipEventSynchronize(ctx->ev[7]));
        float t;
        MRBF_HIP(ctx, hipEventElapsedTime(&t, ctx->ev[4], ctx->ev[7]));
        info->ms_total = t;
        info->ms_kernel = t;
    }
    return 0;
}

}
```

morbit.jl_amd/csrc/gram_fused.hip:

```cpp
#include "radial.hpp"

namespace mrbf {

typedef double v4d __attribute__((ext_vector_type(4)));
typedef double v2d __attribute__((ext_vector_type(2)));

constexpr int GW_LDT = 66;

template <int KID, bool FAST>
__global__ __launch_bounds__(256, 2) void gram_w_kernel(const double *__restrict__ Xc, const double *__restrict__ sq, int64_t n,
                                                        int64_t npad, double *__restrict__ Phi, int64_t ld, KP p, int nt, int nseg,
                                                        int seglen, double *__restrict__ Wpart, double *__restrict__ rspart, int dbg) {
    __shared__ __attribute__((aligned(16))) double T[2][64 * GW_LDT];
    __shared__ double Tsq[2][64];
    const int tid = threadIdx.x, lane = tid & 63, wave = tid >> 6;
    const int l15 = lane & 15, l4 = lane >> 4;
    const int seg = blockIdx.x % nseg, I = nt - 1 - (int)(blockIdx.x / nseg);
    const int jt0 = seg * seglen;
    const int jt1 = (jt0 + seglen < nt) ? jt0 + seglen : nt;
    const int64_t iw0 = (int64_t)I * 128 + 32 * wave;
    double bI[2][16];
#pragma unroll
    for (int it = 0; it < 2; ++it)
#pragma unroll
        for (int ks = 0; ks < 16; ++ks) bI[it][ks] = Xc[(iw0 + it * 16 + l15) * 64 + ks * 4 + l4];
    double sqi[2];
#pragma unroll
    for (int it = 0; it < 2; ++it) sqi[it] = sq[iw0 + it * 16 + l15];
    v4d wacc[4][2];
#pragma unroll
    for (int tt = 0; tt < 4; ++tt)
#pragma unroll
        for (int it = 0; it < 2; ++it) wacc[tt][it] = (v4d){0.0, 0.0, 0.0, 0.0};
    double rs[2] = {0.0, 0.0};
    const int nh = 2 * (jt1 - jt0);
    if (nh > 0) {
        const double *src = Xc + (int64_t)jt0 * 128 * 64;
        const double *ssq = sq + (int64_t)jt0 * 128;
        v2d pf[4];
        double pfsq = 0.0;
        if (tid < 64) pfsq = ssq[tid];
#pragma unroll 1
        for (int half = 0; half < 2; ++half) {
#pragma unroll
            for (int u = 0; u < 4; ++u) pf[u] = *(const v2d *)(src + (tid + 256 * (4 * half + u)) * 2);
#pragma unroll
            for (int u = 0; u < 4; ++u) {
                const int e = (tid + 256 * (4 * half + u)) * 2;
                *(v2d *)&T[0][(e >> 6) * GW_LDT + (e & 63)] = pf[u];
            }
        }
        if (tid < 64) Tsq[0][tid] = pfsq;
        __syncthreads();
#pragma unroll 1
        for (int h = 0; h < nh; ++h) {
            const int buf = h & 1;
            const double *Tb = T[buf];
            const int64_t jb = (int64_t)jt0 * 128 + 64 * h;
            const bool store = (jt0 + (h >> 1)) <= I && !(dbg & 1);
            const bool full = jb + 64 <= n && (int64_t)I * 128 + 128 <= n;
            const bool edge = jb + 64 > n || (jt0 + (h >> 1)) == I;
            const bool more = h + 1 < nh && !(dbg & 16);
            const double *s2 = src + (int64_t)(h + 1) * 64 * 64;
            if (more && tid < 64) pfsq = ssq[64 * (h + 1) + tid];
#pragma unroll 1
            for (int sub = 0; sub < 2; ++sub) {
                const double *Ts = Tb + sub * 32 * GW_LDT;
                if (more) {
#pragma unroll
                    for (int u = 0; u < 4; ++u) pf[u] = *(const v2d *)(s2 + (tid + 256 * (4 * sub + u)) * 2);
                }
                v4d acc[2][2];
#pragma unroll
                for (int jt = 0; jt < 2; ++jt)
#pragma unroll
                    for (int it = 0; it < 2; ++it) acc[jt][it] = (v4d){0.0, 0.0, 0.0, 0.0};
                if (!(dbg & 8))
#pragma unroll
                for (int ks = 0; ks < 16; ++ks) {
                    double a[2];
#pragma unroll
                    for (int jt = 0; jt < 2; ++jt) a[jt] = Ts[(jt * 16 + l15) * GW_LDT + ks * 4 + l4];
#pragma unroll
                    for (int jt = 0; jt < 2; ++jt)
#pragma unroll
                        for (int it = 0; it < 2; ++it)
                            acc[jt][it] = __builtin_amdgcn_mfma_f64_16x16x4f64(a[jt], bI[it][ks], acc[jt][it], 0, 0, 0);
                }
                if (more) {
#pragma unroll
                    for (int u = 0; u < 4; ++u) {
                        const int e = (tid + 256 * (4 * sub + u)) * 2;
                        *(v2d *)&T[buf ^ 1][(e >> 6) * GW_LDT + (e & 63)] = pf[u];
                    }
                    if (sub == 0 && tid < 64) Tsq[buf ^ 1][tid] = pfsq;
                }
                if (edge || !FAST) {
#pragma unroll
                    for (int jt = 0; jt < 2; ++jt)
#pragma unroll
                        for (int r = 0; r < 4; ++r) {
                            const int jl = sub * 32 + jt * 16 + l4 + 4 * r;
                            const int64_t gj = jb + jl;
                            const double sqj = Tsq[buf][jl];
#pragma unroll
                            for (int it = 0; it < 2; ++it) {
                                const int64_t gi = iw0 + it * 16 + l15;
                                double s = fma(-2.0, acc[jt][it][r], sqi[it] + sqj);
                                s = s > 0.0 ? s : 0.0;
                                if (gi == gj) s = 0.0;
                                double v = (dbg & 2) ? s : rbf_phi_t<KID, FAST>(s, p);
                                v = gj < n ? v : 0.0;
                                acc[jt][it][r] = v;
                                rs[it] += v;
                            }
                        }
                } else {
#pragma unroll
                    for (int jt = 0; jt < 2; ++jt)
#pragma unroll
                        for (int r = 0; r < 4; ++r) {
                            const double sqj = Tsq[buf][sub * 32 + jt * 16 + l4 + 4 * r];
#pragma unroll
                            for (int it = 0; it < 2; ++it) {
                                double s = fma(-2.0, acc[jt][it][r], sqi[it] + sqj);
                                s = s > 0.0 ? s : 0.0;
                                const double v = (dbg & 2) ? s : rbf_phi_t<KID, FAST>(s, p);
                                acc[jt][it][r] = v;
                                rs[it] += v;
                            }
                        }
                }
                if (store) {
                    double *dst = Phi + (jb + sub * 32 + l4) * ld + iw0 + l15;
                    if (full) {
#pragma unroll
                        for (int jt = 0; jt < 2; ++jt)
#pragma unroll
                            for (int r = 0; r < 4; ++r)
#pragma unroll
                                for (int it = 0; it < 2; ++it) dst[(int64_t)(jt * 16 + 4 * r) * ld + it * 16] = acc[jt][it][r];
                    } else {
#pragma unroll
                        for (int jt = 0; jt < 2; ++jt)
#pragma unroll
                            for (int r = 0; r < 4; ++r)
#pragma unroll
                                for (int it = 0; it < 2; ++it) {
                                    const int64_t gj = jb + sub * 32 + jt * 16 + l4 + 4 * r, gi = iw0 + it * 16 + l15;
                                    if (gi < n && gj < n) dst[(int64_t)(jt * 16 + 4 * r) * ld + it * 16] = acc[jt][it][r];
                                }
                    }
                }
                if (!(dbg & 4))
#pragma unroll
                for (int jt = 0; jt < 2; ++jt) {
#pragma unroll
                    for (int r = 0; r < 4; ++r) {
                        double aw[4];
#pragma unroll
                        for (int tt = 0; tt < 4; ++tt) aw[tt] = Ts[(jt * 16 + 4 * r + l4) * GW_LDT + tt * 16 + l15];
#pragma unroll
                        for (int tt = 0; tt < 4; ++tt)
#pragma unroll
                            for (int it = 0; it < 2; ++it)
                                wacc[tt][it] = __builtin_amdgcn_mfma_f64_16x16x4f64(aw[tt], acc[jt][it][r], wacc[tt][it], 0, 0, 0);
                    }
                }
            }
            __syncthreads();
        }
    }
#pragma unroll
    for (int tt = 0; tt < 4; ++tt)
#pragma unroll
        for (int r = 0; r < 4; ++r) {
            const int t = tt * 16 + l4 + 4 * r;
#pragma unroll
            for (int it = 0; it < 2; ++it) Wpart[((int64_t)seg * 64 + t) * npad + iw0 + it * 16 + l15] = wacc[tt][it][r];
        }
#pragma unroll
    for (int it = 0; it < 2; ++it) {
        double x = rs[it];
        x += __shfl_xor(x, 16);
        x += __shfl_xor(x, 32);
        if (l4 == 0) rspart[(int64_t)seg * npad + iw0 + it * 16 + l15] = x;
    }
}

__device__ __forceinline__ double sum_partials(const double *__restrict__ p, int cnt, int64_t stride) {
    double sp[8] = {0.0, 0.0, 0.0, 0.0, 0.0, 0.0, 0.0, 0.0};
    int c = 0;
    for (; c + 32 <= cnt; c += 32) {
        double v[32];
#pragma unroll
        for (int u = 0; u < 32; ++u) v[u] = p[(int64_t)(c + u) * stride];
#pragma unroll
        for (int u = 0; u < 32; ++u) sp[u & 7] += v[u];
    }
    for (; c + 8 <= cnt; c += 8) {
        double v[8];
#pragma unroll
        for (int u = 0; u < 8; ++u) v[u] = p[(int64_t)(c + u) * stride];
#pragma unroll
        for (int u = 0; u < 8; ++u) sp[u] += v[u];
    }
    for (int u = 0; c + u < cnt; ++u) sp[u] += p[(int64_t)(c + u) * stride];
    return ((sp[0] + sp[1]) + (sp[2] + sp[3])) + ((sp[4] + sp[5]) + (sp[6] + sp[7]));
}

constexpr int PJ_LS = 68;
constexpr int PJ_QP = 80;

__device__ __forceinline__ v4d pj_tile(const double *As, const double *Bs, int mt, int nt, int K, int l15, int l4) {
    v4d acc = {0.0, 0.0, 0.0, 0.0};
    const double *ap = As + (mt * 16 + l15) * PJ_LS + l4;
    const double *bp = Bs + (nt * 16 + l15) * PJ_LS + l4;
    for (int k = 0; k < K; k += 4) acc = __builtin_amdgcn_mfma_f64_16x16x4f64(ap[k], bp[k], acc, 0, 0, 0);
    return acc;
}

__global__ __launch_bounds__(256) void proj_reduce_kernel(const double *__restrict__ Wpart, const double *__restrict__ rspart, int nseg,
                                                          int64_t npad, int64_t n, int d, int q, const double *__restrict__ linv,
                                                          const double *__restrict__ Q1, double rsqrtn, double *__restrict__ W1,
                                                          double *__restrict__ Gp, double *__restrict__ trp) {
    __shared__ double Ws[64 * PJ_LS];
    __shared__ double Ls[64 * PJ_LS];
    __shared__ double W1s[PJ_QP * PJ_LS];
    __shared__ double Qs[PJ_QP * PJ_LS];
    const int tid = threadIdx.x, i = tid & 63, g = tid >> 6;
    const int lane = tid & 63, wave = tid >> 6, l15 = lane & 15, l4 = lane >> 4;
    const int64_t R0 = (int64_t)blockIdx.x * 64;
    const bool live = R0 + i < n;
    constexpr int Q4 = PJ_QP / 4;
    double qv[Q4];
#pragma unroll
    for (int u = 0; u < Q4; ++u) {
        const int a = g + 4 * u;
        qv[u] = (a < q && live) ? Q1[R0 + i + (int64_t)a * npad] : 0.0;
    }
    const double rsv = (g == 0 && live) ? sum_partials(rspart + R0 + i, nseg, npad) * rsqrtn : 0.0;
    if (q > 1) {
        double lv[16];
#pragma unroll
        for (int u = 0; u < 16; ++u) {
            const int e = tid + 256 * u, c = e & 63, t = e >> 6;
            lv[u] = (c < d && t <= c) ? linv[c + (int64_t)t * 128] : 0.0;
        }
#pragma unroll
        for (int half = 0; half < 2; ++half) {
            double sv[8] = {0.0, 0.0, 0.0, 0.0, 0.0, 0.0, 0.0, 0.0};
            for (int s0 = 0; s0 < nseg; s0 += 8) {
                double wv[8][8];
#pragma unroll
                for (int u = 0; u < 8; ++u)
#pragma unroll
                    for (int sgm = 0; sgm < 8; ++sgm) {
                        const int t = g * 16 + half * 8 + u;
                        wv[u][sgm] = s0 + sgm < nseg ? Wpart[((int64_t)(s0 + sgm) * 64 + t) * npad + R0 + i] : 0.0;
                    }
#pragma unroll
                for (int u = 0; u < 8; ++u)
                    sv[u] += ((wv[u][0] + wv[u][1]) + (wv[u][2] + wv[u][3])) + ((wv[u][4] + wv[u][5]) + (wv[u][6] + wv[u][7]));
            }
#pragma unroll
            for (int u = 0; u < 8; ++u) Ws[i * PJ_LS + (g * 16 + half * 8 + u)] = live ? sv[u] : 0.0;
        }
#pragma unroll
        for (int u = 0; u < 16; ++u) {
            const int e = tid + 256 * u;
            Ls[(e & 63) * PJ_LS + (e >> 6)] = lv[u];
        }
    }
#pragma unroll
    for (int u = 0; u < Q4; ++u) {
        const int a = g + 4 * u;
        Qs[a * PJ_LS + i] = qv[u];
        if (a > d || q == 1) W1s[a * PJ_LS + i] = 0.0;
    }
    if (g == 0) {
        W1s[i] = rsv;
        W1[R0 + i] = rsv;
    }
    __syncthreads();
    if (q > 1) {
#pragma unroll 1
        for (int tile = wave; tile < 16; tile += 4) {
            const int ct = tile >> 2, it = tile & 3;
            const v4d acc = pj_tile(Ls, Ws, ct, it, 64, l15, l4);
#pragma unroll
            for (int r = 0; r < 4; ++r) {
                const int c = ct * 16 + l4 + 4 * r, ii = it * 16 + l15;
                if (c < d) {
                    W1s[(1 + c) * PJ_LS + ii] = acc[r];
                    W1[R0 + ii + (int64_t)(1 + c) * npad] = acc[r];
                }
            }
        }
    }
    __syncthreads();
    double *out = Gp + (size_t)blockIdx.x * q * q;
    const int qt = (q + 15) >> 4;
#pragma unroll 1
    for (int tile = wave; tile < qt * qt; tile += 4) {
        const int at = tile % qt, bt = tile / qt;
        const v4d acc = pj_tile(Qs, W1s, at, bt, 64, l15, l4);
#pragma unroll
        for (int r = 0; r < 4; ++r) {
            const int a = at * 16 + l4 + 4 * r, bb = bt * 16 + l15;
            if (a < q && bb < q) out[a + bb * q] = acc[r];
            if (at == bt && a == bb && a < q) Ls[a] = acc[r];
        }
    }
    __syncthreads();
    if (tid == 0) {
        double tr = 0.0;
        for (int a = 0; a < q; ++a) tr += Ls[a];
        trp[blockIdx.x] = tr;
    }
}

__global__ __launch_bounds__(256) void proj_shift_kernel(const double *__restrict__ Gp, const double *__restrict__ trp, int nchunks, int q,
                                                         double nphi0, double nmq, double *__restrict__ G, double *__restrict__ Mh,
                                                         double *__restrict__ scal, int *__restrict__ flags) {
    __shared__ double dg[256];
    __shared__ double smu;
    const int tid = threadIdx.x;
    const size_t qq = (size_t)q * q;
    const int idx = blockIdx.x * 256 + tid;
    const double *p0 = Gp + (idx < (int)qq ? idx : 0);
    double tv = 0.0;
    for (int c = tid; c < nchunks; c += 256) tv += trp[c];
    double s0[8] = {0, 0, 0, 0, 0, 0, 0, 0};
    int c = 0;
    for (; c + 64 <= nchunks; c += 64) {
        double v0[64];
#pragma unroll
        for (int u = 0; u < 64; ++u) v0[u] = p0[(size_t)(c + u) * qq];
#pragma unroll
        for (int u = 0; u < 64; ++u) s0[u & 7] += v0[u];
    }
    for (; c < nchunks; ++c) s0[c & 7] += p0[(size_t)c * qq];
    const double gv = ((s0[0] + s0[1]) + (s0[2] + s0[3])) + ((s0[4] + s0[5]) + (s0[6] + s0[7]));
    dg[tid] = tv;
    __syncthreads();
    for (int w = 128; w > 0; w >>= 1) {
        if (tid < w) dg[tid] += dg[tid + w];
        __syncthreads();
    }
    if (tid == 0) {
        const double tr = dg[0];
        const double mu = (nphi0 - tr) / nmq;
        const bool ok = mu > 0.0 && mu < 1e300;
        smu = ok ? mu : 1.0;
        if (blockIdx.x == 0) {
            scal[0] = tr;
            scal[1] = smu;
            flags[2] = ok ? 0 : 1;
        }
    }
    __syncthreads();
    if (idx < (int)qq) {
        G[idx] = gv;
        Mh[idx] = 0.5 * gv + ((idx % q) == (idx / q) ? 0.5 * smu : 0.0);
    }
}

__global__ __launch_bounds__(256) void proj_panels_kernel(const double *__restrict__ Q1, const double *__restrict__ W1,
                                                          const double *__restrict__ Mh, int64_t n, int64_t npad, int q, int K2, int skip,
                                                          double *__restrict__ PA, double *__restrict__ PB, double *__restrict__ v0) {
    __shared__ double Qs[64 * PJ_LS];
    __shared__ double Ms[PJ_QP * PJ_LS];
    const int tid = threadIdx.x, i = tid & 63, g = tid >> 6;
    const int lane = tid & 63, wave = tid >> 6, l15 = lane & 15, l4 = lane >> 4;
    const int64_t R0 = (int64_t)blockIdx.x * 64;
    const bool live = R0 + i < n;
    constexpr int QA = 17;
    double qv[QA];
#pragma unroll
    for (int u = 0; u < QA; ++u) {
        const int a = g + 4 * u;
        qv[u] = (a < q && live) ? Q1[R0 + i + (int64_t)a * npad] : 0.0;
    }
    constexpr int ME = (PJ_QP * PJ_LS + 255) / 256;
    double mv[ME];
#pragma unroll
    for (int u = 0; u < ME; ++u) {
        const int e = tid + 256 * u, bb = e / PJ_LS, a = e % PJ_LS;
        mv[u] = (a < q && bb < q) ? Mh[a + bb * q] : 0.0;
    }
#pragma unroll
    for (int u = 0; u < ME; ++u) {
        const int e = tid + 256 * u;
        if (e < PJ_QP * PJ_LS) Ms[e] = mv[u];
    }
#pragma unroll
    for (int u = 0; u < QA; ++u) Qs[i * PJ_LS + g + 4 * u] = qv[u];
    __syncthreads();
    const int qq = q - skip, qt = (q + 15) >> 4, K = (q + 3) & ~3;
#pragma unroll 1
    for (int tile = wave; tile < qt * 4; tile += 4) {
        const int bt = tile >> 2, it = tile & 3;
        const v4d acc = pj_tile(Ms, Qs, bt, it, K, l15, l4);
        const int ii = it * 16 + l15;
        const bool lv = R0 + ii < n;
        double w1[4], qb[4];
#pragma unroll
        for (int r = 0; r < 4; ++r) {
            const int b = bt * 16 + l4 + 4 * r;
            w1[r] = (b < q && lv) ? W1[R0 + ii + (int64_t)b * npad] : 0.0;
            qb[r] = b < q ? Qs[ii * PJ_LS + b] : 0.0;
        }
#pragma unroll
        for (int r = 0; r < 4; ++r) {
            const int b = bt * 16 + l4 + 4 * r;
            if (b >= q) continue;
            const double v = lv ? w1[r] - acc[r] : 0.0;
            if (b >= skip) {
                const int c = b - skip;
                PA[R0 + ii + (int64_t)c * npad] = qb[r];
                PB[R0 + ii + (int64_t)c * npad] = v;
                PA[R0 + ii + (int64_t)(qq + c) * npad] = v;
                PB[R0 + ii + (int64_t)(qq + c) * npad] = qb[r];
            } else {
                v0[R0 + ii] = v;
            }
        }
    }
    for (int c = 2 * qq + g; c < K2; c += 4) {
        PA[R0 + i + (int64_t)c * npad] = 0.0;
        PB[R0 + i + (int64_t)c * npad] = 0.0;
    }
}

bool gram_w_applies(const mrbf_ctx *ctx, const mrbf_model *M) {
    static const int on = mrbf_env("MRBF_GRAM_FUSED") ? atoi(mrbf_env("MRBF_GRAM_FUSED")) : 1;
    if (!on || ctx->gram_mode != 0) return false;
    if (M->dpad != 64 || M->q < 1 || M->q > 65 || M->n < 1024) return false;
    if (kp_nonsmooth(M->kp)) return false;
    return M->kp.fast || M->kp.kid == MRBF_GAUSSIAN || M->kp.kid == MRBF_THIN_PLATE_SPLINE;
}

int launch_gram_w(mrbf_ctx *ctx, const mrbf_model *M, double *Phi, int64_t ld, double **Wpart_out, double **rspart_out, int *nseg_out) {
    const int nt = (int)(M->npad / 128);
    static const int dbg = mrbf_env("MRBF_GW_DBG") ? atoi(mrbf_env("MRBF_GW_DBG")) : 0;
    static const int wgs = mrbf_env("MRBF_GW_WGS") ? atoi(mrbf_env("MRBF_GW_WGS")) : 512;
    int nseg = wgs / nt;
    if (nseg < 1) nseg = 1;
    if (nseg > nt) nseg = nt;
    const int seglen = (nt + nseg - 1) / nseg;
    nseg = (nt + seglen - 1) / seglen;
    double *Wpart, *rspart;
    MRBF_TRY(get_buf(ctx, S_GW_PART, (size_t)nseg * 64 * M->npad, &Wpart));
    MRBF_TRY(get_buf(ctx, S_GW_RS, (size_t)nseg * M->npad, &rspart));
    const dim3 grid((unsigned)(nt * nseg));
    if (M->kp.fast) {
        MRBF_DISPATCH_KID(M->kp.kid, hipLaunchKernelGGL((gram_w_kernel<KID, true>), grid, dim3(256), 0, ctx->stream, M->Xc, M->sq, M->n,
                                                        M->npad, Phi, ld, M->kp, nt, nseg, seglen, Wpart, rspart, dbg));
    } else if (M->kp.kid == MRBF_GAUSSIAN) {
        hipLaunchKernelGGL((gram_w_kernel<MRBF_GAUSSIAN, false>), grid, dim3(256), 0, ctx->stream, M->Xc, M->sq, M->n, M->npad, Phi, ld,
                           M->kp, nt, nseg, seglen, Wpart, rspart, dbg);
    } else {
        hipLaunchKernelGGL((gram_w_kernel<MRBF_THIN_PLATE_SPLINE, false>), grid, dim3(256), 0, ctx->stream, M->Xc, M->sq, M->n, M->npad,
                           Phi, ld, M->kp, nt, nseg, seglen, Wpart, rspart, dbg);
    }
    MRBF_HIP(ctx, hipGetLastError());
    *Wpart_out = Wpart;
    *rspart_out = rspart;
    *nseg_out = nseg;
    return 0;
}

int launch_projection_small(mrbf_ctx *ctx, const mrbf_model *M, const double *Wpart, const double *rspart, int nseg, const double *linv,
                            const double *Q1, double *W1, double *G, double *scal, int *flags, int K2, int skip, double *PA, double *PB,
                            double *v0) {
    const int64_t n = M->n, npad = M->npad;
    const int q = M->q, nch = (int)(npad / 64);
    double *Gp, *Mh;
    MRBF_TRY(get_buf(ctx, S_GW_GP, (size_t)nch * q * q + nch, &Gp));
    MRBF_TRY(get_buf(ctx, S_GW_M, (size_t)q * q, &Mh));
    double *trp = Gp + (size_t)nch * q * q;
    hipLaunchKernelGGL(proj_reduce_kernel, dim3((unsigned)nch), dim3(256), 0, ctx->stream, Wpart, rspart, nseg, npad, n, M->d, q, linv, Q1,
                       1.0 / std::sqrt((double)n), W1, Gp, trp);
    hipLaunchKernelGGL(proj_shift_kernel, dim3((unsigned)((q * q + 255) / 256)), dim3(256), 0, ctx->stream, Gp, trp, nch, q,
                       (double)n * M->kp.phi0, (double)std::max<int64_t>(n - q, 1), G, Mh, scal, flags);
    hipLaunchKernelGGL(proj_panels_kernel, dim3((unsigned)nch), dim3(256), 0, ctx->stream, Q1, W1, Mh, n, npad, q, K2, skip, PA, PB, v0);
    MRBF_HIP(ctx, hipGetLastError());
    return 0;
}

}
```

morbit.jl_amd/csrc/prep.hip:

```cpp
#include "common.hpp"

namespace mrbf {

__global__ void column_mean_kernel(const double *__restrict__ X, int64_t n, int d, double *__restrict__ mean) {
    __shared__ double red[256];
    const int t = blockIdx.x;
    if (t >= d) {
        if (threadIdx.x == 0) mean[t] = 0.0;
        return;
    }
    double s = 0.0;
    for (int64_t i = threadIdx.x; i < n; i += blockDim.x) s += X[i * d + t];
    red[threadIdx.x] = s;
    __syncthreads();
    for (int w = 128; w > 0; w >>= 1) {
        if ((int)threadIdx.x < w) red[threadIdx.x] += red[threadIdx.x + w];
        __syncthreads();
    }
    if (threadIdx.x == 0) mean[t] = red[0] / (double)n;
}

__global__ void center_pad_kernel(const double *__restrict__ X, int64_t n, int d, const double *__restrict__ mean,
                                  double *__restrict__ Xc, int64_t npad, int dpad, double *__restrict__ sq) {
    const int lane = threadIdx.x & 63;
    const int64_t row = (int64_t)blockIdx.x * (blockDim.x >> 6) + (threadIdx.x >> 6);
    if (row >= npad) return;
    double s = 0.0;
    for (int t = lane; t < dpad; t += 64) {
        double v = 0.0;
        if (row < n && t < d) v = X[row * d + t] - mean[t];
        Xc[row * dpad + t] = v;
        s = fma(v, v, s);
    }
    for (int off = 32; off > 0; off >>= 1) s += __shfl_xor(s, off);
    if (lane == 0) sq[row] = s;
}

int launch_center_pad(mrbf_ctx *ctx, const double *X, int64_t n, int d, const double *mean_or_null, double *mean_out,
                      double *Xc, int64_t npad, int dpad, double *sq) {
    const double *mean = mean_or_null;
    if (!mean) {
        hipLaunchKernelGGL(column_mean_kernel, dim3(dpad > d ? dpad : d), dim3(256), 0, ctx->stream, X, n, d, mean_out);
        mean = mean_out;
    }
    const int rows_per_block = 4;
    hipLaunchKernelGGL(center_pad_kernel, dim3((unsigned)((npad + rows_per_block - 1) / rows_per_block)), dim3(256), 0,
                       ctx->stream, X, n, d, mean, Xc, npad, dpad, sq);
    MRBF_HIP(ctx, hipGetLastError());
    return 0;
}

__global__ void poly_matrix_kernel(const double *__restrict__ C, int64_t n, int d, int q, double *__restrict__ Pi,
                                   int64_t ld) {
    const int64_t i = (int64_t)blockIdx.x * blockDim.x + threadIdx.x;
    if (i >= n) return;
    for (int t = 0; t < q; ++t) Pi[i + (int64_t)t * ld] = (t == 0) ? 1.0 : C[i * d + (t - 1)];
}

int launch_poly_matrix(mrbf_ctx *ctx, const double *C, int64_t n, int d, int q, double *Pi, int64_t ldpi) {
    if (q <= 0 || n <= 0) return 0;
    hipLaunchKernelGGL(poly_matrix_kernel, dim3((unsigned)((n + 255) / 256)), dim3(256), 0, ctx->stream, C, n, d, q, Pi,
                       ldpi);
    MRBF_HIP(ctx, hipGetLastError());
    return 0;
}

__global__ void transpose_kernel(const double *__restrict__ in, int64_t rows, int64_t cols, double *__restrict__ out) {
    const int64_t idx = (int64_t)blockIdx.x * blockDim.x + threadIdx.x;
    if (idx >= rows * cols) return;
    const int64_t r = idx / cols, c = idx % cols;
    out[c * rows + r] = in[idx];
}

int launch_transpose(mrbf_ctx *ctx, const double *in, int64_t rows, int64_t cols, double *out) {
    if (rows * cols <= 0) return 0;
    hipLaunchKernelGGL(transpose_kernel, dim3((unsigned)((rows * cols + 255) / 256)), dim3(256), 0, ctx->stream, in, rows,
                       cols, out);
    MRBF_HIP(ctx, hipGetLastError());
    return 0;
}

}
```

morbit.jl_amd/csrc/solve.hip:

```cpp
#include "common.hpp"
#include "small.hpp"

namespace mrbf {

__global__ void fit_publish_kernel(const int *__restrict__ dinfo, const double *__restrict__ scal, const unsigned long long *__restrict__ dstat,
                                   int *__restrict__ hflags, double *__restrict__ hscal, unsigned long long *__restrict__ hstat) {
    const int t = threadIdx.x;
    if (t < 4) hflags[t] = dinfo[t];
    if (t >= 4 && t < 6 && scal) hscal[t - 4] = scal[t - 4];
    if (t == 6 && dstat && hstat) hstat[0] = dstat[0];
}

__global__ void fill_saddle_kernel(const double *__restrict__ Pi, int64_t n, int q, double *__restrict__ S, int64_t N) {
    const int64_t idx = (int64_t)blockIdx.x * blockDim.x + threadIdx.x;
    const int64_t tot = n * q;
    if (idx < tot) {
        const int64_t i = idx % n;
        const int t = (int)(idx / n);
        const double v = Pi[idx];
        S[i + (n + t) * N] = v;
        S[(n + t) + i * N] = v;
    } else if (idx < tot + (int64_t)q * q) {
        const int64_t r = idx - tot;
        S[(n + r % q) + (n + r / q) * N] = 0.0;
    }
}

__global__ void rhs_from_values_kernel(const double *__restrict__ Y, int64_t n, int k, double *__restrict__ B, int64_t N) {
    const int64_t idx = (int64_t)blockIdx.x * blockDim.x + threadIdx.x;
    if (idx >= N * k) return;
    const int64_t i = idx % N;
    const int l = (int)(idx / N);
    B[idx] = (i < n) ? Y[i * k + l] : 0.0;
}

__global__ void scatter_solution_kernel(const double *__restrict__ B, int64_t ldB, int64_t n, int64_t npad, int k, int q,
                                        int64_t lam_row0, double *__restrict__ W, double *__restrict__ Wc,
                                        double *__restrict__ lam, const double *__restrict__ lamsrc, int64_t ldlam) {
    const int64_t idx = (int64_t)blockIdx.x * blockDim.x + threadIdx.x;
    if (idx < npad * k) {
        const int64_t i = idx % npad;
        const int l = (int)(idx / npad);
        const double v = (i < n) ? B[i + l * ldB] : 0.0;
        Wc[idx] = v;
        if (i < n) W[i * k + l] = v;
    } else if (idx < npad * k + (int64_t)q * k) {
        const int64_t r = idx - npad * k;
        const int t = (int)(r % q), l = (int)(r / q);
        lam[(int64_t)t * k + l] = lamsrc[lam_row0 + t + l * ldlam];
    }
}

__global__ void copy_upper_kernel(const double *__restrict__ A, int64_t lda, int q, double *__restrict__ R) {
    const int idx = blockIdx.x * blockDim.x + threadIdx.x;
    if (idx >= q * q) return;
    const int i = idx % q, j = idx / q;
    R[idx] = (i <= j) ? A[i + (int64_t)j * lda] : 0.0;
}

__global__ void trace_kernel(const double *__restrict__ G, int q, double *__restrict__ out) {
    __shared__ double red[256];
    double s = 0.0;
    for (int i = threadIdx.x; i < q; i += 256) s += G[i + (int64_t)i * q];
    red[threadIdx.x] = s;
    __syncthreads();
    for (int w = 128; w > 0; w >>= 1) {
        if ((int)threadIdx.x < w) red[threadIdx.x] += red[threadIdx.x + w];
        __syncthreads();
    }
    if (threadIdx.x == 0) out[0] = red[0];
}

__global__ void max_abs_kernel(const double *__restrict__ v, int64_t cnt, double *__restrict__ out) {
    __shared__ double red[256];
    double s = 0.0;
    for (int64_t i = threadIdx.x; i < cnt; i += 256) s = fmax(s, fabs(v[i]));
    red[threadIdx.x] = s;
    __syncthreads();
    for (int w = 128; w > 0; w >>= 1) {
        if ((int)threadIdx.x < w) red[threadIdx.x] = fmax(red[threadIdx.x], red[threadIdx.x + w]);
        __syncthreads();
    }
    if (threadIdx.x == 0) out[0] = red[0];
}

__global__ void residual_kernel(const double *__restrict__ a, const double *__restrict__ b, int64_t cnt,
                                double *__restrict__ out) {
    __shared__ double r0[256], r1[256];
    double s0 = 0.0, s1 = 0.0;
    for (int64_t i = threadIdx.x; i < cnt; i += 256) {
        const double df = a[i] - b[i];
        s0 = fma(df, df, s0);
        s1 = fma(b[i], b[i], s1);
    }
    r0[threadIdx.x] = s0;
    r1[threadIdx.x] = s1;
    __syncthreads();
    for (int w = 128; w > 0; w >>= 1) {
        if ((int)threadIdx.x < w) {
            r0[threadIdx.x] += r0[threadIdx.x + w];
            r1[threadIdx.x] += r1[threadIdx.x + w];
        }
        __syncthreads();
    }
    if (threadIdx.x == 0) {
        out[0] = r0[0];
        out[1] = r1[0];
    }
}

static inline unsigned nblk(int64_t cnt) { return (unsigned)((cnt + 255) / 256); }

void model_block_release(mrbf_ctx *ctx, void *p, size_t bytes, bool slab) {
    if (!ctx) {
        (void)hipFree(p);
        return;
    }
    model_pool_release(ctx->model_pool, p, bytes, slab, [](void *q) { (void)hipFree(q); });
}

void destroy_model(mrbf_ctx *ctx, mrbf_model *M) {
    if (!M) return;
    if (ctx && (M->block || M->slab)) --ctx->live_models;
    if (M->block) model_block_release(ctx, M->block, M->block_bytes);
    if (M->slab && slab_drop(M->slab)) {
        model_block_release(ctx, M->slab->p, M->slab->bytes, true);
        delete M->slab;
    }
    delete M;
}

void model_set_dims(mrbf_model *M, int64_t n, int d, int k, int kid, double a, double b, int deg) {
    M->n = n;
    M->d = d;
    M->k = k;
    M->deg = deg;
    M->q = poly_dim(d, deg);
    M->npad = round_up(n, 128);
    M->dpad = (d <= 64) ? 64 : (d <= 128 ? 128 : (d <= 256 ? 256 : (int)round_up(d, 16)));
    M->kp = make_kp(kid, a, b);
}

size_t model_block_layout(const mrbf_model *M, size_t off[7]) {
    const size_t cnt[7] = {(size_t)M->n * M->d, (size_t)M->npad * M->dpad, (size_t)M->npad, (size_t)M->dpad, (size_t)M->n * M->k,
                           (size_t)M->npad * M->k, (size_t)std::max(M->q, 1) * M->k};
    size_t at = 0;
    for (int i = 0; i < 7; ++i) {
        off[i] = at;
        at += (std::max<size_t>(cnt[i], 2) * sizeof(double) + 255) & ~size_t(255);
    }
    return at;
}

void model_carve(mrbf_model *M, char *base, const size_t off[7]) {
    M->C = (double *)(base + off[0]);
    M->Xc = (double *)(base + off[1]);
    M->sq = (double *)(base + off[2]);
    M->mean = (double *)(base + off[3]);
    M->W = (double *)(base + off[4]);
    M->Wc = (double *)(base + off[5]);
    M->lam = (double *)(base + off[6]);
}

int model_block_acquire(mrbf_ctx *ctx, size_t total, void **p, size_t *bytes) {
    hipError_t e = hipSuccess;
    auto alloc = [&](size_t b) -> void * {
        void *q = nullptr;
        e = hipMalloc(&q, b);
        return e == hipSuccess ? q : nullptr;
    };
    if (!model_pool_acquire(ctx->model_pool, total, p, bytes, alloc, [](void *q) { (void)hipFree(q); }))
        return fail(ctx, MRBF_ENOMEM, "model allocation failed: %s", hipGetErrorString(e));
    return 0;
}

int build_model_shell(mrbf_ctx *ctx, int64_t n, int d, int k, const double *Cdev, int kid, double a, double b, int deg,
                      mrbf_model **out) {
    mrbf_model *M = new mrbf_model();
    model_set_dims(M, n, d, k, kid, a, b, deg);
    size_t off[7];
    const size_t total = model_block_layout(M, off);
    const int rc_block = model_block_acquire(ctx, total, &M->block, &M->block_bytes);
    if (rc_block != 0) {
        delete M;
        return rc_block;
    }
    ++ctx->live_models;
    M->owner = ctx;
    model_carve(M, (char *)M->block, off);
    auto init = [&]() -> int {
        if (Cdev != M->C)
            MRBF_HIP(ctx, hipMemcpyAsync(M->C, Cdev, (size_t)n * d * sizeof(double), hipMemcpyDeviceToDevice, ctx->stream));
        MRBF_TRY(launch_center_pad(ctx, M->C, n, d, nullptr, M->mean, M->Xc, M->npad, M->dpad, M->sq));
        return 0;
    };
    const int rc = init();
    if (rc != 0) {
        destroy_model(ctx, M);
        return rc;
    }
    *out = M;
    return 0;
}

static int read_info(mrbf_ctx *ctx, const int *dinfo, int *hinfo) {
    MRBF_HIP(ctx, hipMemcpyAsync(hinfo, dinfo, sizeof(int), hipMemcpyDeviceToHost, ctx->stream));
    MRBF_HIP(ctx, hipStreamSynchronize(ctx->stream));
    return 0;
}

void fill_small_prob(const mrbf_ctx *ctx, const mrbf_model *M, const double *Y, double *ws, int *flags, double *scal, int *cl, smallfit::Prob *P);
static int fit_lu(mrbf_ctx *ctx, mrbf_model *M, const double *Y, mrbf_fit_info *info) {
    const int64_t n = M->n, N = n + M->q;
    const int k = M->k, q = M->q;
    double *S, *B, *Pi = nullptr;
    int *ipiv, *dinfo;
    MRBF_TRY(get_buf(ctx, S_PHI, (size_t)N * N, &S));
    MRBF_TRY(get_buf(ctx, S_RHS, (size_t)N * k, &B));
    MRBF_TRY(get_buf(ctx, S_IPIV, (size_t)N, &ipiv));
    MRBF_TRY(get_buf(ctx, S_INFO, (size_t)4, &dinfo));
    hipLaunchKernelGGL(rhs_from_values_kernel, dim3(nblk(N * k)), dim3(256), 0, ctx->stream, Y, n, k, B, N);
    MRBF_HIP(ctx, hipEventRecord(ctx->ev[0], ctx->stream));
    MRBF_TRY(launch_gram(ctx, ctx->gram_mode, M->C, M->Xc, M->sq, n, M->npad, M->d, M->dpad, M->kp, S, N));
    MRBF_HIP(ctx, hipEventRecord(ctx->ev[1], ctx->stream));
    if (q > 0) {
        MRBF_TRY(get_buf(ctx, S_PI, (size_t)n * q, &Pi));
        MRBF_TRY(launch_poly_matrix(ctx, M->C, n, M->d, q, Pi, n));
        hipLaunchKernelGGL(fill_saddle_kernel, dim3(nblk(n * q + (int64_t)q * q)), dim3(256), 0, ctx->stream, Pi, n, q, S, N);
    }
    MRBF_HIP(ctx, hipGetLastError());
    MRBF_HIP(ctx, hipEventRecord(ctx->ev[5], ctx->stream));
    MRBF_BLAS(ctx, rocsolver_dgetrf(ctx->blas, (int)N, (int)N, S, (int)N, ipiv, dinfo));
    MRBF_HIP(ctx, hipEventRecord(ctx->ev[2], ctx->stream));
    int hinfo = 0;
    MRBF_TRY(read_info(ctx, dinfo, &hinfo));
    info->factor_info = hinfo;
    info->path = MRBF_PATH_LU;
    if (hinfo != 0) return fail(ctx, MRBF_ESINGULAR, "saddle matrix is singular (getrf info = %d, N = %lld)", hinfo, (long long)N);
    MRBF_BLAS(ctx, rocsolver_dgetrs(ctx->blas, rocblas_operation_none, (int)N, k, S, (int)N, ipiv, B, (int)N));
    hipLaunchKernelGGL(scatter_solution_kernel, dim3(nblk(M->npad * k + (int64_t)q * k)), dim3(256), 0, ctx->stream, B, N, n,
                       M->npad, k, q, n, M->W, M->Wc, M->lam, B, N);
    MRBF_HIP(ctx, hipGetLastError());
    MRBF_HIP(ctx, hipEventRecord(ctx->ev[3], ctx->stream));
    MRBF_HIP(ctx, hipEventSynchronize(ctx->ev[3]));
    MRBF_HIP(ctx, hipEventElapsedTime(&info->ms_gram, ctx->ev[0], ctx->ev[1]));
    MRBF_HIP(ctx, hipEventElapsedTime(&info->ms_project, ctx->ev[1], ctx->ev[5]));
    MRBF_HIP(ctx, hipEventElapsedTime(&info->ms_factor, ctx->ev[5], ctx->ev[2]));
    MRBF_HIP(ctx, hipEventElapsedTime(&info->ms_solve, ctx->ev[2], ctx->ev[3]));
    return 0;
}

static int fit_small_lu(mrbf_ctx *ctx, mrbf_model *M, const double *Y, mrbf_fit_info *info) {
    smallfit::Prob P;
    double *ws, *scal;
    int *flags;
    MRBF_TRY(get_buf(ctx, S_SMALL_LU, small_lu_scratch_doubles(M->n, M->q), &ws));
    MRBF_TRY(get_buf(ctx, S_SMALL_FLAGS, (size_t)4, &flags));
    MRBF_TRY(get_buf(ctx, S_MISC, (size_t)8, &scal));
    fill_small_prob(ctx, M, Y, ws, flags, scal, nullptr, &P);
    int hflags_local[4] = {0, 0, 0, 0};
    int *hflags = ctx->hpin ? reinterpret_cast<int *>(ctx->hpin + HPIN_SMALL_FLAGS) : hflags_local;
    MRBF_HIP(ctx, hipEventRecord(ctx->ev[0], ctx->stream));
    MRBF_TRY(launch_small_lu(ctx, &P, 1, nullptr));
    MRBF_HIP(ctx, hipEventRecord(ctx->ev[1], ctx->stream));
    MRBF_HIP(ctx, hipMemcpyAsync(hflags, flags, 4 * sizeof(int), hipMemcpyDeviceToHost, ctx->stream));
    MRBF_HIP(ctx, hipStreamSynchronize(ctx->stream));
    info->factor_info = hflags[0];
    info->path = MRBF_PATH_LU;
    if (hflags[0] != 0)
        return fail(ctx, MRBF_ESINGULAR, "saddle matrix is singular (getrf info = %d, N = %lld)", hflags[0], (long long)(M->n + M->q));
    MRBF_HIP(ctx, hipEventElapsedTime(&info->ms_factor, ctx->ev[0], ctx->ev[1]));
    return 0;
}

__global__ void scale_rows_pinv_kernel(double *__restrict__ T, int N, int k, const double *__restrict__ sv) {
    const int idx = blockIdx.x * blockDim.x + threadIdx.x;
    if (idx >= N * k) return;
    const int i = idx % N;
    const double s = sv[i], cut = (double)N * 2.220446049250313e-16 * sv[0];
    T[idx] = (s > cut) ? T[idx] / s : 0.0;
}

static int fit_minnorm(mrbf_ctx *ctx, mrbf_model *M, const double *Y, mrbf_fit_info *info) {
    const int64_t n = M->n, N = n + M->q;
    const int k = M->k, q = M->q;
    const double one = 1.0, zero = 0.0;
    double *S, *B, *Pi, *U, *VT, *sv, *E, *T;
    int *dinfo;
    MRBF_TRY(get_buf(ctx, S_PHI, (size_t)N * N, &S));
    MRBF_TRY(get_buf(ctx, S_RHS, (size_t)N * k, &B));
    MRBF_TRY(get_buf(ctx, S_PI, (size_t)n * q, &Pi));
    MRBF_TRY(get_buf(ctx, S_Q1, (size_t)N * N, &U));
    MRBF_TRY(get_buf(ctx, S_W1, (size_t)N * N, &VT));
    MRBF_TRY(get_buf(ctx, S_TAU, (size_t)2 * N, &sv));
    MRBF_TRY(get_buf(ctx, S_T1, (size_t)N * k, &T));
    MRBF_TRY(get_buf(ctx, S_INFO, (size_t)4, &dinfo));
    E = sv + N;
    hipLaunchKernelGGL(rhs_from_values_kernel, dim3(nblk(N * k)), dim3(256), 0, ctx->stream, Y, n, k, B, N);
    MRBF_HIP(ctx, hipEventRecord(ctx->ev[0], ctx->stream));
    MRBF_TRY(launch_gram(ctx, ctx->gram_mode, M->C, M->Xc, M->sq, n, M->npad, M->d, M->dpad, M->kp, S, N));
    MRBF_HIP(ctx, hipEventRecord(ctx->ev[1], ctx->stream));
    MRBF_TRY(launch_poly_matrix(ctx, M->C, n, M->d, q, Pi, n));
    hipLaunchKernelGGL(fill_saddle_kernel, dim3(nblk(n * q + (int64_t)q * q)), dim3(256), 0, ctx->stream, Pi, n, q, S, N);
    MRBF_HIP(ctx, hipGetLastError());
    MRBF_BLAS(ctx, rocsolver_dgesvd(ctx->blas, rocblas_svect_all, rocblas_svect_all, (int)N, (int)N, S, (int)N, sv, U, (int)N, VT,
                                    (int)N, E, rocblas_outofplace, dinfo));
    MRBF_HIP(ctx, hipEventRecord(ctx->ev[2], ctx->stream));
    int hinfo = 0;
    MRBF_TRY(read_info(ctx, dinfo, &hinfo));
    info->factor_info = hinfo;
    info->path = MRBF_PATH_MINNORM;
    if (hinfo != 0) return fail(ctx, MRBF_ESINGULAR, "SVD of the saddle matrix did not converge (info = %d)", hinfo);
    MRBF_BLAS(ctx, rocblas_dgemm(ctx->blas, rocblas_operation_transpose, rocblas_operation_none, (int)N, k, (int)N, &one, U, (int)N,
                                 B, (int)N, &zero, T, (int)N));
    hipLaunchKernelGGL(scale_rows_pinv_kernel, dim3(nblk(N * k)), dim3(256), 0, ctx->stream, T, (int)N, k, sv);
    MRBF_BLAS(ctx, rocblas_dgemm(ctx->blas, rocblas_operation_transpose, rocblas_operation_none, (int)N, k, (int)N, &one, VT, (int)N,
                                 T, (int)N, &zero, B, (int)N));
    hipLaunchKernelGGL(scatter_solution_kernel, dim3(nblk(M->npad * k + (int64_t)q * k)), dim3(256), 0, ctx->stream, B, N, n,
                       M->npad, k, q, n, M->W, M->Wc, M->lam, B, N);
    MRBF_HIP(ctx, hipGetLastError());
    MRBF_HIP(ctx, hipEventRecord(ctx->ev[3], ctx->stream));
    MRBF_HIP(ctx, hipEventSynchronize(ctx->ev[3]));
    MRBF_HIP(ctx, hipEventElapsedTime(&info->ms_gram, ctx->ev[0], ctx->ev[1]));
    MRBF_HIP(ctx, hipEventElapsedTime(&info->ms_factor, ctx->ev[1], ctx->ev[2]));
    MRBF_HIP(ctx, hipEventElapsedTime(&info->ms_solve, ctx->ev[2], ctx->ev[3]));
    return 0;
}

int backsolve_blocked(mrbf_ctx *ctx, int64_t npad, const double *L, int64_t lda, const double *linv_all, double *Y, int64_t ldy, int k);
int backsolve_persistent(mrbf_ctx *ctx, int64_t npad, const double *L, int64_t lda, const double *linv_all, double *Y, int64_t ldy, int k,
                         int *status);
int launch_update_lower(mrbf_ctx *ctx, const double *A, int64_t lda, const double *B, int64_t ldb, double *C, int64_t ldc, int64_t nt, int K,
                        const double *cvec, double cs, int64_t cn);
int launch_pad_identity(mrbf_ctx *ctx, double *A, int64_t n, int64_t npad, int64_t ld);
int tsmm_tn(mrbf_ctx *ctx, int64_t n, int p, int r, double alpha, const double *A, int64_t lda, const double *B, int64_t ldb, double beta,
            double *C, int64_t ldc);
int symm_panel(mrbf_ctx *ctx, int64_t n, int64_t npad, int q, const double *Phi, int64_t ld, const double *Q, int64_t ldq, double *W,
               int64_t ldwo, bool const_first, double cval);

__global__ void set_rhs_rows_kernel(double *__restrict__ A, int64_t ld, int64_t npad, int xt, const double *__restrict__ B, int k) {
    const int64_t idx = (int64_t)blockIdx.x * blockDim.x + threadIdx.x;
    if (idx >= npad * xt) return;
    const int l = (int)(idx % xt);
    const int64_t i = idx / xt;
    A[(npad + l) + i * ld] = (l < k) ? B[i + (int64_t)l * npad] : 0.0;
}
__global__ void get_rhs_rows_kernel(const double *__restrict__ A, int64_t ld, int64_t npad, double *__restrict__ B, int k) {
    const int64_t idx = (int64_t)blockIdx.x * blockDim.x + threadIdx.x;
    if (idx >= npad * k) return;
    const int l = (int)(idx % k);
    const int64_t i = idx / k;
    B[i + (int64_t)l * npad] = A[(npad + l) + i * ld];
}
__global__ void xc_to_tall_kernel(const double *__restrict__ Xc, int64_t n, int d, int dpad, double *__restrict__ Tall, int64_t lt,
                                  int64_t dq) {
    const int64_t idx = (int64_t)blockIdx.x * blockDim.x + threadIdx.x;
    if (idx >= n * d) return;
    const int64_t i = idx / d;
    const int t = (int)(idx % d);
    Tall[(dq + i) + (int64_t)t * lt] = Xc[i * dpad + t];
}
__global__ void build_q1_kernel(const double *__restrict__ Tall, int64_t lt, int64_t dq, int64_t n, int64_t npad, int q,
                                double *__restrict__ Q1) {
    const int64_t idx = (int64_t)blockIdx.x * blockDim.x + threadIdx.x;
    if (idx >= npad * q) return;
    const int64_t i = idx % npad;
    const int t = (int)(idx / npad);
    double v = 0.0;
    if (i < n) v = (t == 0) ? 1.0 / sqrt((double)n) : Tall[(dq + i) + (int64_t)(t - 1) * lt];
    Q1[idx] = v;
}
__global__ void shift_from_trace_kernel(double *__restrict__ scal, double nphi0, double nmq, int *__restrict__ flags) {
    const double mu = (nphi0 - scal[0]) / nmq;
    const bool ok = mu > 0.0 && mu < 1e300;
    scal[1] = ok ? mu : 1.0;
    flags[2] = ok ? 0 : 1;
}

__global__ void build_panels_kernel(const double *__restrict__ Q1, const double *__restrict__ W, const double *__restrict__ scal,
                                    int64_t n, int64_t npad, int q, int K2, int skip, double *__restrict__ PA, double *__restrict__ PB,
                                    double *__restrict__ v0) {
    const int64_t idx = (int64_t)blockIdx.x * blockDim.x + threadIdx.x;
    if (idx >= npad * K2) return;
    const double mu = scal[1];
    const int64_t i = idx % npad;
    const int t = (int)(idx / npad);
    const int qq = q - skip;
    double a = 0.0, b = 0.0;
    if (i < n && t < 2 * qq) {
        const int tt = t % qq + skip;
        const double qv = Q1[i + (int64_t)tt * npad];
        const double vv = fma(-0.5 * mu, qv, W[i + (int64_t)tt * npad]);
        a = (t < qq) ? qv : vv;
        b = (t < qq) ? vv : qv;
    }
    PA[idx] = a;
    PB[idx] = b;
    if (skip && t == 0) v0[i] = (i < n) ? fma(-0.5 * mu, Q1[i], W[i]) : 0.0;
}
__global__ __launch_bounds__(64) void finish_lambda_kernel(double *__restrict__ T1, int q, int k, double sqrtn, const double *__restrict__ mean) {
    __shared__ double part[64];
    const int l = blockIdx.x, tid = threadIdx.x;
    if (l >= k) return;
    double acc = 0.0;
    for (int t = 1 + tid; t < q; t += 64) acc = fma(mean[t - 1], T1[t + (int64_t)l * q], acc);
    part[tid] = acc;
    __syncthreads();
    if (tid == 0) {
        double dsum = 0.0;
        for (int u = 0; u < 64; ++u) dsum += part[u];
        T1[(int64_t)l * q] = T1[(int64_t)l * q] / sqrtn - dsum;
    }
}

__global__ __launch_bounds__(256) void sub_qt_kernel(double *__restrict__ B, int64_t ldb, const double *__restrict__ Q, int64_t ldq,
                                                     const double *__restrict__ T, int64_t n, int q, int k) {
    __shared__ double part[4][64];
    const int r = threadIdx.x & 63, g = threadIdx.x >> 6;
    const int64_t row = (int64_t)blockIdx.x * 64 + r;
    for (int l = 0; l < k; ++l) {
        double s0 = 0.0, s1 = 0.0;
        if (row < n) {
            int t = g;
            for (; t + 4 < q; t += 8) {
                s0 = fma(Q[row + (int64_t)t * ldq], T[t + (int64_t)l * q], s0);
                s1 = fma(Q[row + (int64_t)(t + 4) * ldq], T[t + 4 + (int64_t)l * q], s1);
            }
            if (t < q) s0 = fma(Q[row + (int64_t)t * ldq], T[t + (int64_t)l * q], s0);
        }
        __syncthreads();
        part[g][r] = s0 + s1;
        __syncthreads();
        if (g == 0 && row < n) B[row + (int64_t)l * ldb] -= (part[0][r] + part[1][r]) + (part[2][r] + part[3][r]);
    }
}

__global__ __launch_bounds__(256) void apply_linv_t_kernel(const double *__restrict__ inv, int d, double *__restrict__ X, int64_t ldx, int k) {
    __shared__ double bs[128];
    const int j = threadIdx.x & 127, half = threadIdx.x >> 7;
    __shared__ double part[2][128];
    for (int l = 0; l < k; ++l) {
        __syncthreads();
        if (threadIdx.x < 128) bs[threadIdx.x] = threadIdx.x < d ? X[threadIdx.x + (int64_t)l * ldx] : 0.0;
        __syncthreads();
        double v = 0.0;
        if (j < d) {
            const double *col = inv + (int64_t)j * 128;
            for (int i = j + half; i < d; i += 2) v = fma(col[i], bs[i], v);
        }
        part[half][j] = v;
        __syncthreads();
        if (half == 0 && j < d) X[j + (int64_t)l * ldx] = part[0][j] + part[1][j];
    }
}

__global__ __launch_bounds__(256) void trsm_lt_small_kernel(const double *__restrict__ L, int64_t ldl, int d, double *__restrict__ X,
                                                            int64_t ldx, int k) {
    __shared__ double xs[256];
    const int j = threadIdx.x;
    for (int l = 0; l < k; ++l) {
        double v = j < d ? X[j + (int64_t)l * ldx] : 0.0;
        for (int c = d - 1; c >= 0; --c) {
            if (j == c) {
                v /= L[c + (int64_t)c * ldl];
                xs[c] = v;
            }
            __syncthreads();
            if (j < c) v -= L[c + (int64_t)j * ldl] * xs[c];
            __syncthreads();
        }
        if (j < d) X[j + (int64_t)l * ldx] = v;
    }
}

__global__ __launch_bounds__(256) void tail_dots_kernel(const double *__restrict__ Bw, int64_t ldb, const double *__restrict__ Q1,
                                                        const double *__restrict__ Wm, int64_t ldq, int64_t n, int q, int k,
                                                        double *__restrict__ part) {
    __shared__ double ws[64 * 16];
    __shared__ double red[4][2][64];
    const int tid = threadIdx.x, g = tid >> 6, lane = tid & 63;
    const int64_t R0 = (int64_t)blockIdx.x * 64;
    for (int e = tid; e < 64 * k; e += 256) {
        const int i = e & 63, l = e >> 6;
        ws[e] = R0 + i < n ? Bw[R0 + i + (int64_t)l * ldb] : 0.0;
    }
    __syncthreads();
    for (int a0 = 0; a0 < q; a0 += 64) {
        const int a = a0 + lane;
        double qv[16], wv[16];
#pragma unroll
        for (int u = 0; u < 16; ++u) {
            const int64_t r = R0 + 16 * g + u;
            const bool ok = a < q && r < n;
            qv[u] = ok ? Q1[r + (int64_t)a * ldq] : 0.0;
            wv[u] = ok ? Wm[r + (int64_t)a * ldq] : 0.0;
        }
        for (int l = 0; l < k; ++l) {
            double s0 = 0.0, s1 = 0.0;
#pragma unroll
            for (int u = 0; u < 16; ++u) {
                const double w = ws[l * 64 + 16 * g + u];
                s0 = fma(qv[u], w, s0);
                s1 = fma(wv[u], w, s1);
            }
            __syncthreads();
            red[g][0][lane] = s0;
            red[g][1][lane] = s1;
            __syncthreads();
            if (g == 0 && a < q) {
                double *o = part + ((size_t)blockIdx.x * 2 * k + l) * q + a;
                o[0] = (red[0][0][lane] + red[1][0][lane]) + (red[2][0][lane] + red[3][0][lane]);
                o[(size_t)k * q] = (red[0][1][lane] + red[1][1][lane]) + (red[2][1][lane] + red[3][1][lane]);
            }
        }
    }
}

__global__ __launch_bounds__(1024) void tail_coeff_kernel(const double *__restrict__ part, int nch, int q, int k, int d, const double *__restrict__ T1,
                                                         const double *__restrict__ G, double cg, const double *__restrict__ LxInv,
                                                         double sqrtn, const double *__restrict__ mean, double *__restrict__ T2,
                                                         double *__restrict__ lam_out) {
    __shared__ double t2[129 * 16], zz[129 * 16], xx[129 * 16];
    const int tid = threadIdx.x, nthr = blockDim.x;
    for (int e = tid; e < 2 * k * q; e += nthr) {
        double sv = 0.0;
        for (int c0 = 0; c0 < nch; c0 += 32) {
            double v[32];
#pragma unroll
            for (int u = 0; u < 32; ++u) v[u] = c0 + u < nch ? part[(size_t)(c0 + u) * 2 * k * q + e] : 0.0;
#pragma unroll
            for (int u = 0; u < 32; ++u) sv += v[u];
        }
        if (e < k * q)
            t2[e] = sv;
        else
            zz[e - k * q] = sv;
    }
    __syncthreads();
    for (int e = tid; e < k * q; e += nthr) {
        const int l = e / q, a = e % q;
        double corr = 0.0;
        for (int b0 = 0; b0 < q; b0 += 16) {
            double gv[16];
#pragma unroll
            for (int u = 0; u < 16; ++u) gv[u] = b0 + u < q ? G[b0 + u + (int64_t)a * q] : 0.0;
#pragma unroll
            for (int u = 0; u < 16; ++u) corr = fma(gv[u], b0 + u < q ? t2[l * q + b0 + u] : 0.0, corr);
        }
        zz[e] = T1[a + (int64_t)l * q] - zz[e] + cg * corr;
        T2[a + (int64_t)l * q] = t2[e];
    }
    __syncthreads();
    for (int e = tid; e < k * d; e += nthr) {
        const int l = e / d, j = e % d;
        double acc = 0.0;
        for (int i0 = j; i0 < d; i0 += 16) {
            double iv[16];
#pragma unroll
            for (int u = 0; u < 16; ++u) iv[u] = i0 + u < d ? LxInv[i0 + u + (int64_t)j * 128] : 0.0;
#pragma unroll
            for (int u = 0; u < 16; ++u) acc = fma(iv[u], i0 + u < d ? zz[l * q + 1 + i0 + u] : 0.0, acc);
        }
        xx[l * q + 1 + j] = acc;
    }
    __syncthreads();
    if (tid < k) {
        const int l = tid;
        double dsum = 0.0;
        for (int t0 = 1; t0 < q; t0 += 16) {
            double mv[16];
#pragma unroll
            for (int u = 0; u < 16; ++u) mv[u] = t0 + u < q ? mean[t0 + u - 1] : 0.0;
#pragma unroll
            for (int u = 0; u < 16; ++u) dsum = fma(mv[u], t0 + u < q ? xx[l * q + t0 + u] : 0.0, dsum);
        }
        xx[l * q] = zz[l * q] / sqrtn - dsum;
    }
    __syncthreads();
    for (int e = tid; e < k * q; e += nthr) lam_out[(e % q) + (int64_t)(e / q) * q] = xx[e];
}

__global__ __launch_bounds__(256) void tail_apply_kernel(const double *__restrict__ Bw, int64_t ldb, const double *__restrict__ Q1, int64_t ldq,
                                                         const double *__restrict__ T2, const double *__restrict__ lamsrc, int64_t n,
                                                         int64_t npad, int q, int k, double *__restrict__ W, double *__restrict__ Wc,
                                                         double *__restrict__ lam) {
    __shared__ double part4[4][64];
    const int tid = threadIdx.x, r = tid & 63, g = tid >> 6;
    const int64_t row = (int64_t)blockIdx.x * 64 + r;
    for (int l = 0; l < k; ++l) {
        double s0 = 0.0, s1 = 0.0;
        if (row < n) {
            int t = g;
            for (; t + 4 < q; t += 8) {
                s0 = fma(Q1[row + (int64_t)t * ldq], T2[t + (int64_t)l * q], s0);
                s1 = fma(Q1[row + (int64_t)(t + 4) * ldq], T2[t + 4 + (int64_t)l * q], s1);
            }
            if (t < q) s0 = fma(Q1[row + (int64_t)t * ldq], T2[t + (int64_t)l * q], s0);
        }
        __syncthreads();
        part4[g][r] = s0 + s1;
        __syncthreads();
        if (g == 0 && row < npad) {
            const double v = row < n ? Bw[row + (int64_t)l * ldb] - ((part4[0][r] + part4[1][r]) + (part4[2][r] + part4[3][r])) : 0.0;
            Wc[row + (int64_t)l * npad] = v;
            if (row < n) W[row * k + l] = v;
        }
    }
    if (blockIdx.x == 0)
        for (int e = tid; e < q * k; e += 256) lam[(int64_t)(e % q) * k + e / q] = lamsrc[(e % q) + (int64_t)(e / q) * q];
}

static int fit_chol(mrbf_ctx *ctx, mrbf_model *M, const double *Y, mrbf_fit_info *info, int *not_pd, int *gave_up, int impl = 0) {
    const int64_t n = M->n, npad = M->npad;
    const int k = M->k, q = M->q, d = M->d;
    const double one = 1.0, mhalf = -0.5;
    *not_pd = 0;
    *gave_up = 0;
    if (impl == 0) impl = ctx->chol_impl;
    const bool builtin = impl != 1;
    PotrfOpts popt;
    popt.impl = impl;
    const int xt = builtin ? (int)round_up(k, 128) : 0;
    const int64_t ld = npad + xt;
    double *Phi, *B;
    int *dinfo;
    MRBF_TRY(get_buf(ctx, S_PHI, (size_t)ld * npad, &Phi));
    MRBF_TRY(get_buf(ctx, S_RHS, (size_t)npad * k, &B));
    MRBF_TRY(get_buf(ctx, S_INFO, (size_t)4, &dinfo));
    MRBF_HIP(ctx, hipMemsetAsync(dinfo, 0, 4 * sizeof(int), ctx->stream));
    const bool tailq = q > 1 && tail_basis_applies(M) && M->k == k;
    if (!tailq) hipLaunchKernelGGL(rhs_from_values_kernel, dim3(nblk(npad * k)), dim3(256), 0, ctx->stream, Y, n, k, B, npad);
    double *Q1 = nullptr, *Wm = nullptr, *G = nullptr, *T1 = nullptr, *scal = nullptr, *Tall = nullptr, *LxInv = nullptr;
    int64_t lt = 0, dq = 0;
    info->mu = 0.0;
    hipStream_t main_stream = ctx->stream;
    const bool side = q > 0 && ctx->panel_stream && ctx->panel_stream != main_stream && n >= 2048;
    const bool fused = q > 0 && gram_w_applies(ctx, M) && (q == 1 || round_up(d, 128) == 128);
    if (q > 0) {
        MRBF_TRY(get_buf(ctx, S_Q1, (size_t)npad * q, &Q1));
        MRBF_TRY(get_buf(ctx, S_W1, (size_t)npad * q, &Wm));
        MRBF_TRY(get_buf(ctx, S_G, (size_t)q * q, &G));
        MRBF_TRY(get_buf(ctx, S_T1, (size_t)q * k, &T1));
        MRBF_TRY(get_buf(ctx, S_MISC, (size_t)8, &scal));
        if (side) {
            MRBF_HIP(ctx, hipEventRecord(ctx->evx[0], main_stream));
            MRBF_HIP(ctx, hipStreamWaitEvent(ctx->panel_stream, ctx->evx[0], 0));
            ctx->stream = ctx->panel_stream;
        }
        struct RestoreStream {
            mrbf_ctx *c;
            hipStream_t s;
            ~RestoreStream() { c->stream = s; }
        } restore{ctx, main_stream};
        if (tailq) {
            double *scratch;
            MRBF_TRY(get_buf(ctx, S_PI, tail_basis_scratch_doubles(), &scratch));
            MRBF_TRY(get_buf(ctx, S_QR_INV, (size_t)128 * 128, &LxInv));
            MRBF_TRY(launch_tail_basis(ctx, M, Y, scratch, LxInv, T1, Q1, B, builtin ? Phi : nullptr, ld, xt, dinfo));
        } else if (q > 1) {
            dq = round_up(d, 128);
            lt = dq + npad;
            MRBF_TRY(get_buf(ctx, S_PI, (size_t)lt * dq, &Tall));
            MRBF_HIP(ctx, hipMemsetAsync(Tall, 0, (size_t)lt * dq * sizeof(double), ctx->stream));
            hipLaunchKernelGGL(xc_to_tall_kernel, dim3(nblk(n * d)), dim3(256), 0, ctx->stream, M->Xc, n, d, M->dpad, Tall, lt, dq);
            MRBF_TRY(tsmm_tn(ctx, n, d, d, 1.0, Tall + dq, lt, Tall + dq, lt, 0.0, Tall, lt));
            MRBF_TRY(launch_pad_identity(ctx, Tall, d, dq, lt));
            if (dq == 128) MRBF_TRY(get_buf(ctx, S_QR_INV, (size_t)128 * 128, &LxInv));
            MRBF_TRY(potrf_blocked_tall(ctx, dq, lt, Tall, lt, dinfo + 1, LxInv, popt));
        }
        if (!tailq) hipLaunchKernelGGL(build_q1_kernel, dim3(nblk(npad * q)), dim3(256), 0, ctx->stream, Tall, lt, dq, n, npad, q, Q1);
        if (!fused) MRBF_HIP(ctx, hipMemsetAsync(Wm, 0, (size_t)npad * q * sizeof(double), ctx->stream));
        if (!tailq) {
            MRBF_TRY(tsmm_tn(ctx, n, q, k, 1.0, Q1, npad, B, npad, 0.0, T1, q));
            hipLaunchKernelGGL(sub_qt_kernel, dim3((unsigned)((n + 63) / 64)), dim3(256), 0, ctx->stream, B, npad, Q1, npad, T1, n, q, k);
            if (builtin) hipLaunchKernelGGL(set_rhs_rows_kernel, dim3(nblk(npad * xt)), dim3(256), 0, ctx->stream, Phi, ld, npad, xt, B, k);
        }
        if (side) MRBF_HIP(ctx, hipEventRecord(ctx->evx[1], ctx->stream));
    }
    ctx->stream = main_stream;
    MRBF_HIP(ctx, hipEventRecord(ctx->ev[0], ctx->stream));
    double *Wpart = nullptr, *rspart = nullptr;
    int nseg = 0;
    if (fused)
        MRBF_TRY(launch_gram_w(ctx, M, Phi, ld, &Wpart, &rspart, &nseg));
    else
        MRBF_TRY(launch_gram(ctx, ctx->gram_mode, M->C, M->Xc, M->sq, n, M->npad, M->d, M->dpad, M->kp, Phi, ld));
    MRBF_HIP(ctx, hipEventRecord(ctx->ev[1], ctx->stream));
    if (side) MRBF_HIP(ctx, hipStreamWaitEvent(ctx->stream, ctx->evx[1], 0));
    if (fused) {
        const int skip = (q > 1 && round_up(2 * (q - 1), 16) < round_up(2 * q, 16)) ? 1 : 0;
        const int K2 = (int)round_up(2 * (q - skip), 16);
        double *PA, *PB, *v0 = nullptr;
        MRBF_TRY(get_buf(ctx, S_STAGE_C, (size_t)npad * K2, &PA));
        MRBF_TRY(get_buf(ctx, S_STAGE_D, (size_t)npad * K2, &PB));
        if (skip) MRBF_TRY(get_buf(ctx, S_V0, (size_t)npad, &v0));
        MRBF_TRY(launch_projection_small(ctx, M, Wpart, rspart, nseg, LxInv, Q1, Wm, G, scal, dinfo, K2, skip, PA, PB, v0));
        MRBF_TRY(launch_update_lower(ctx, PA, npad, PB, npad, Phi, ld, npad / 128, K2, v0, 1.0 / std::sqrt((double)n), n));
    } else if (q > 0) {
        MRBF_TRY(symm_panel(ctx, n, npad, q, Phi, ld, Q1, npad, Wm, npad, true, 1.0 / std::sqrt((double)n)));
        MRBF_TRY(tsmm_tn(ctx, n, q, q, 1.0, Q1, npad, Wm, npad, 0.0, G, q));
        hipLaunchKernelGGL(trace_kernel, dim3(1), dim3(256), 0, ctx->stream, G, q, scal);
        MRBF_BLAS(ctx, rocblas_dgemm(ctx->blas, rocblas_operation_none, rocblas_operation_none, (int)n, q, q, &mhalf, Q1, (int)npad,
                                     G, q, &one, Wm, (int)npad));
        hipLaunchKernelGGL(shift_from_trace_kernel, dim3(1), dim3(1), 0, ctx->stream, scal, (double)n * M->kp.phi0,
                           (double)std::max<int64_t>(n - q, 1), dinfo);
        const int skip = (q > 1 && round_up(2 * (q - 1), 16) < round_up(2 * q, 16)) ? 1 : 0;
        const int K2 = (int)round_up(2 * (q - skip), 16);
        double *PA, *PB, *v0 = nullptr;
        MRBF_TRY(get_buf(ctx, S_STAGE_C, (size_t)npad * K2, &PA));
        MRBF_TRY(get_buf(ctx, S_STAGE_D, (size_t)npad * K2, &PB));
        if (skip) MRBF_TRY(get_buf(ctx, S_V0, (size_t)npad, &v0));
        hipLaunchKernelGGL(build_panels_kernel, dim3(nblk(npad * K2)), dim3(256), 0, ctx->stream, Q1, Wm, scal, n, npad, q, K2, skip, PA, PB, v0);
        MRBF_TRY(launch_update_lower(ctx, PA, npad, PB, npad, Phi, ld, npad / 128, K2, v0, 1.0 / std::sqrt((double)n), n));
    }
    MRBF_HIP(ctx, hipEventRecord(ctx->ev[2], ctx->stream));
    int hinfo = 0;
    double *linv_all = nullptr;
    if (builtin) {
        MRBF_TRY(get_buf(ctx, S_CHOL_WS, (size_t)npad * 128, &linv_all));
        MRBF_TRY(launch_pad_identity(ctx, Phi, n, npad, ld));
        if (q == 0) hipLaunchKernelGGL(set_rhs_rows_kernel, dim3(nblk(npad * xt)), dim3(256), 0, ctx->stream, Phi, ld, npad, xt, B, k);
        popt.xreal = k;
        popt.info_clean = true;
        MRBF_TRY(potrf_blocked_tall(ctx, npad, npad + xt, Phi, ld, dinfo, linv_all, popt));
        MRBF_HIP(ctx, hipEventRecord(ctx->ev[3], ctx->stream));
    } else {
        int *dpot;
        MRBF_TRY(get_buf(ctx, S_IPIV, (size_t)4, &dpot));
        MRBF_BLAS(ctx, rocsolver_dpotrf(ctx->blas, rocblas_fill_lower, (int)n, Phi, (int)ld, dpot));
        MRBF_HIP(ctx, hipMemcpyAsync(dinfo, dpot, sizeof(int), hipMemcpyDeviceToDevice, ctx->stream));
        MRBF_HIP(ctx, hipEventRecord(ctx->ev[3], ctx->stream));
    }
    double *T1w = nullptr;
    if (q > 0) MRBF_TRY(get_buf(ctx, S_T1W, (size_t)q * k, &T1w));
    auto solve_tail = [&](bool persistent) -> int {
        if (builtin) {
            hipLaunchKernelGGL(get_rhs_rows_kernel, dim3(nblk(npad * k)), dim3(256), 0, ctx->stream, Phi, ld, npad, B, k);
            if (persistent)
                MRBF_TRY(backsolve_persistent(ctx, npad, Phi, ld, linv_all, B, npad, k, dinfo + 3));
            else
                MRBF_TRY(backsolve_blocked(ctx, npad, Phi, ld, linv_all, B, npad, k));
        } else {
            MRBF_BLAS(ctx, rocsolver_dpotrs(ctx->blas, rocblas_fill_lower, (int)n, k, Phi, (int)ld, B, (int)npad));
        }
        static const int tail3 = mrbf_env("MRBF_TAIL3") ? atoi(mrbf_env("MRBF_TAIL3")) : 1;
        if (tail3 && q > 0 && q <= 129 && k <= 16 && (q == 1 || LxInv)) {
            const int nch = (int)(npad / 64);
            double *T2, *part;
            MRBF_TRY(get_buf(ctx, S_T2, (size_t)q * k, &T2));
            MRBF_TRY(get_buf(ctx, S_TAIL_PART, (size_t)nch * 2 * k * q, &part));
            hipLaunchKernelGGL(tail_dots_kernel, dim3((unsigned)nch), dim3(256), 0, ctx->stream, B, npad, Q1, Wm, npad, n, q, k, part);
            hipLaunchKernelGGL(tail_coeff_kernel, dim3(1), dim3(1024), 0, ctx->stream, part, nch, q, k, q > 1 ? d : 0, T1, G, fused ? 1.0 : 0.5, LxInv,
                               std::sqrt((double)n), M->mean, T2, T1w);
            hipLaunchKernelGGL(tail_apply_kernel, dim3((unsigned)nch), dim3(256), 0, ctx->stream, B, npad, Q1, npad, T2, T1w, n, M->npad, q, k, M->W,
                               M->Wc, M->lam);
            MRBF_HIP(ctx, hipGetLastError());
            return 0;
        }
        if (q > 0) {
            double *T2;
            MRBF_TRY(get_buf(ctx, S_T2, (size_t)q * k, &T2));
            MRBF_HIP(ctx, hipMemcpyAsync(T1w, T1, (size_t)q * k * sizeof(double), hipMemcpyDeviceToDevice, ctx->stream));
            MRBF_TRY(tsmm_tn(ctx, n, q, k, 1.0, Q1, npad, B, npad, 0.0, T2, q));
            hipLaunchKernelGGL(sub_qt_kernel, dim3((unsigned)((n + 63) / 64)), dim3(256), 0, ctx->stream, B, npad, Q1, npad, T2, n, q, k);
            MRBF_TRY(tsmm_tn(ctx, n, q, k, -1.0, Wm, npad, B, npad, 1.0, T1w, q));
            if (q > 1) {
                if (LxInv)
                    hipLaunchKernelGGL(apply_linv_t_kernel, dim3(1), dim3(256), 0, ctx->stream, LxInv, d, T1w + 1, (int64_t)q, k);
                else if (d <= 256)
                    hipLaunchKernelGGL(trsm_lt_small_kernel, dim3(1), dim3(256), 0, ctx->stream, Tall, lt, d, T1w + 1, (int64_t)q, k);
                else
                    MRBF_BLAS(ctx, rocblas_dtrsm(ctx->blas, rocblas_side_left, rocblas_fill_lower, rocblas_operation_transpose,
                                                 rocblas_diagonal_non_unit, d, k, &one, Tall, (int)lt, T1w + 1, q));
            }
            hipLaunchKernelGGL(finish_lambda_kernel, dim3((unsigned)k), dim3(64), 0, ctx->stream, T1w, q, k, std::sqrt((double)n), M->mean);
        }
        hipLaunchKernelGGL(scatter_solution_kernel, dim3(nblk(M->npad * k + (int64_t)q * k)), dim3(256), 0, ctx->stream, B, npad, n,
                           M->npad, k, q, (int64_t)0, M->W, M->Wc, M->lam, T1w ? T1w : B, (int64_t)q);
        MRBF_HIP(ctx, hipGetLastError());
        return 0;
    };
    MRBF_TRY(solve_tail(true));
    MRBF_HIP(ctx, hipEventRecord(ctx->ev[4], ctx->stream));
    {
        int hflags_local[4] = {0, 0, 0, 0};
        double hscal_local[2] = {0.0, 0.0};
        int *hflags = ctx->hpin ? reinterpret_cast<int *>(ctx->hpin + HPIN_FIT_FLAGS) : hflags_local;
        double *hscal = ctx->hpin ? reinterpret_cast<double *>(ctx->hpin + HPIN_FIT_SCAL) : hscal_local;
        hscal[0] = hscal[1] = 0.0;
        static const int publish = mrbf_env("MRBF_FIT_PUBLISH") ? atoi(mrbf_env("MRBF_FIT_PUBLISH")) : 1;
        if (ctx->hpin && publish) {
            unsigned long long *hstat = nullptr;
            const unsigned long long *dstat = nullptr;
            if (ctx->mega_stat_pending && ctx->mega_stat_dev) {
                ctx->hpin[HPIN_MEGA_STAT] = ~0ull;
                hstat = &ctx->hpin[HPIN_MEGA_STAT];
                dstat = ctx->mega_stat_dev;
                ctx->mega_stat_pending = 2;
            }
            hipLaunchKernelGGL(fit_publish_kernel, dim3(1), dim3(64), 0, ctx->stream, (const int *)dinfo, q > 0 ? (const double *)scal : nullptr, dstat,
                               hflags, hscal, hstat);
        } else {
        MRBF_HIP(ctx, hipMemcpyAsync(hflags, dinfo, 4 * sizeof(int), hipMemcpyDeviceToHost, ctx->stream));
        if (q > 0) MRBF_HIP(ctx, hipMemcpyAsync(hscal, scal, 2 * sizeof(double), hipMemcpyDeviceToHost, ctx->stream));
        MRBF_TRY(mega_stat_enqueue(ctx));
        }
        MRBF_HIP(ctx, hipStreamSynchronize(ctx->stream));
        MRBF_TRY(mega_stat_finish(ctx));
        info->ms_factor_device = ctx->last_device_ms;
        hinfo = hflags[0];
        if (hinfo < 0) {
            *gave_up = 1;
            info->giveup_code = -hinfo;
            return 0;
        }
        info->factor_info = hinfo;
        if (q > 0) info->mu = hscal[1];
        if (hflags[1] < 0) {
            *gave_up = 1;
            info->giveup_code = -hflags[1];
            return 0;
        }
        if (hflags[1] != 0) {
            *not_pd = 1;
            info->factor_info = -2;
            return 0;
        }
        if (hflags[2] != 0) {
            *not_pd = 1;
            info->factor_info = -1;
            return 0;
        }
        if (hinfo != 0) {
            *not_pd = 1;
            return 0;
        }
        if (hflags[3] != 0) {
            info->fallbacks |= MRBF_FB_BACKSOLVE_BLOCKED;
            info->giveup_code = hflags[3];
            MRBF_TRY(solve_tail(false));
            MRBF_HIP(ctx, hipEventRecord(ctx->ev[4], ctx->stream));
        }
    }
    MRBF_HIP(ctx, hipEventSynchronize(ctx->ev[4]));
    MRBF_HIP(ctx, hipEventElapsedTime(&info->ms_gram, ctx->ev[0], ctx->ev[1]));
    MRBF_HIP(ctx, hipEventElapsedTime(&info->ms_project, ctx->ev[1], ctx->ev[2]));
    MRBF_HIP(ctx, hipEventElapsedTime(&info->ms_factor, ctx->ev[2], ctx->ev[3]));
    MRBF_HIP(ctx, hipEventElapsedTime(&info->ms_solve, ctx->ev[3], ctx->ev[4]));
    info->path = q > 0 ? MRBF_PATH_PROJ_CHOL : MRBF_PATH_CHOL;
    return 0;
}

void fill_small_prob(const mrbf_ctx *ctx, const mrbf_model *M, const double *Y, double *ws, int *flags, double *scal, int *cl, smallfit::Prob *P) {
    P->n = (int)M->n;
    P->d = M->d;
    P->k = M->k;
    P->q = M->q;
    P->deg = M->deg;
    P->n16 = (int)round_up(M->n, 16);
    P->npad = (int)M->npad;
    P->dpad = M->dpad;
    P->q16 = (int)round_up(std::max(M->q, 1), 16);
    P->kp = M->kp;
    P->C = M->C;
    P->Y = Y;
    P->Xc = M->Xc;
    P->sq = M->sq;
    P->mean = M->mean;
    P->W = M->W;
    P->Wc = M->Wc;
    P->lam = M->lam;
    P->ws = ws;
    P->flags = flags;
    P->scal = scal;
    P->stamps = nullptr;
    P->cl = cl;
    P->spin_ticks = (unsigned long long)std::max(1, ctx->spin_ms) * 100000ull;
    P->fault = (ctx->debug_fault & 4) ? 1 : 0;
    P->mean_given = 0;
}
int small_fit_verdict(const mrbf_model *M, const int *hflags, const double *hscal, mrbf_fit_info *info) {
    info->path = M->q > 0 ? MRBF_PATH_PROJ_CHOL : MRBF_PATH_CHOL;
    info->mu = M->q > 0 ? hscal[1] : 0.0;
    info->factor_info = hflags[0];
    if (hflags[1] != 0) {
        info->factor_info = -2;
        return 1;
    }
    if (hflags[2] != 0) {
        info->factor_info = -1;
        return 1;
    }
    return hflags[0] != 0 ? 1 : 0;
}
static int fit_check_enqueue(mrbf_ctx *ctx, mrbf_model *M, const double *Y, double *h, hipEvent_t e0, hipEvent_t e1);
static int fit_check_finish(mrbf_ctx *ctx, const mrbf_model *M, const double *h, mrbf_fit_info *info, hipEvent_t e0, hipEvent_t e1);
static int fit_small(mrbf_ctx *ctx, mrbf_model *M, const double *Y, mrbf_fit_info *info, int *not_pd, int force_nc, int *nc_used,
                     bool *checked = nullptr) {
    *not_pd = 0;
    if (checked) *checked = false;
    smallfit::Prob P;
    const smallfit::Carve cv = smallfit::carve((int)M->npad, (int)round_up(std::max(M->q, 1), 16));
    double *ws, *scal;
    int *flags;
    MRBF_TRY(get_buf(ctx, S_SMALL_WS, cv.total, &ws));
    MRBF_TRY(get_buf(ctx, S_SMALL_FLAGS, (size_t)4, &flags));
    MRBF_TRY(get_buf(ctx, S_MISC, (size_t)8, &scal));
    int *cl;
    MRBF_TRY(get_buf(ctx, S_SMALL_CL, (size_t)smallfit::CL_WORDS, &cl));
    fill_small_prob(ctx, M, Y, ws, flags, scal, cl, &P);
    static const int want_stamps = mrbf_env("MRBF_SMALL_STAMPS") ? atoi(mrbf_env("MRBF_SMALL_STAMPS")) : 0;
    long long *dstamps = nullptr;
    if (want_stamps) {
        MRBF_TRY(get_buf(ctx, S_SMALL_DESC, (size_t)16, &dstamps));
        P.stamps = dstamps;
    }
    int hflags_local[4] = {0, 0, 0, 0};
    double hscal_local[2] = {0.0, 0.0}, hchk_local[3] = {0, 0, 0};
    int *hflags = ctx->hpin ? reinterpret_cast<int *>(ctx->hpin + HPIN_SMALL_FLAGS) : hflags_local;
    double *hscal = ctx->hpin ? reinterpret_cast<double *>(ctx->hpin + HPIN_SMALL_SCAL) : hscal_local;
    double *hchk = ctx->hpin ? reinterpret_cast<double *>(ctx->hpin + HPIN_SMALL_CHK) : hchk_local;
    int nc = force_nc > 0 ? force_nc : small_fit_cluster(ctx, 1);
    for (int attempt = 0; attempt < 2; ++attempt) {
        MRBF_HIP(ctx, hipMemsetAsync(cl, 0, smallfit::CL_WORDS * sizeof(int), ctx->stream));
        MRBF_HIP(ctx, hipEventRecord(ctx->ev[0], ctx->stream));
        MRBF_TRY(launch_small_fit(ctx, &P, 1, nullptr, nc));
        MRBF_HIP(ctx, hipEventRecord(ctx->ev[1], ctx->stream));
        MRBF_HIP(ctx, hipMemcpyAsync(hflags, flags, 4 * sizeof(int), hipMemcpyDeviceToHost, ctx->stream));
        MRBF_HIP(ctx, hipMemcpyAsync(hscal, scal, 2 * sizeof(double), hipMemcpyDeviceToHost, ctx->stream));
        hchk[0] = hchk[1] = hchk[2] = 0.0;
        const bool with_check = checked && ctx->residual;
        if (with_check) MRBF_TRY(fit_check_enqueue(ctx, M, Y, hchk, ctx->ev[2], ctx->ev[3]));
        MRBF_HIP(ctx, hipStreamSynchronize(ctx->stream));
        if (with_check && hflags[3] == 0 && hflags[0] == 0 && hflags[1] == 0 && hflags[2] == 0) {
            MRBF_TRY(fit_check_finish(ctx, M, hchk, info, ctx->ev[2], ctx->ev[3]));
            *checked = true;
        }
        if (nc == 1) break;
        if (hflags[3] == 0) {
            ctx->small_timeouts = 0;
            break;
        }
        if (hflags[3] == 2 || ++ctx->small_timeouts >= 3) ctx->small_nc = 1;
        nc = 1;
    }
    *nc_used = nc;
    MRBF_HIP(ctx, hipEventElapsedTime(&info->ms_factor, ctx->ev[0], ctx->ev[1]));
    if (want_stamps) {
        long long hs[16];
        MRBF_HIP(ctx, hipMemcpy(hs, dstamps, sizeof(hs), hipMemcpyDeviceToHost));
        static const char *names[] = {"centre", "gram", "Q1", "W,G,mu,V", "K update", "rhs", "potrf", "solves", "tail"};
        fprintf(stderr, "small fit n=%lld d=%d q=%d (%d workgroup%s): %.3f ms |", (long long)M->n, M->d, M->q, nc, nc == 1 ? "" : "s", info->ms_factor);
        for (int i = 0; i < 9; ++i) fprintf(stderr, " %s %.1f us |", names[i], (hs[i + 1] - hs[i]) * 0.01);
        fprintf(stderr, " [gram: product %.1f us, radial function %.1f us, padding %.1f us]\n", (hs[11] - hs[1]) * 0.01, (hs[12] - hs[11]) * 0.01,
                (hs[2] - hs[12]) * 0.01);
    }
    *not_pd = small_fit_verdict(M, hflags, hscal, info);
    return 0;
}

static int fit_check_enqueue(mrbf_ctx *ctx, mrbf_model *M, const double *Y, double *h, hipEvent_t e0, hipEvent_t e1) {
    const int64_t n = M->n;
    const int k = M->k, q = M->q;
    double *V, *scal;
    MRBF_TRY(get_buf(ctx, S_STAGE_D, (size_t)n * k, &V));
    MRBF_TRY(get_buf(ctx, S_CHECK_SCAL, (size_t)8, &scal));
    MRBF_HIP(ctx, hipEventRecord(e0, ctx->stream));
    EvalHints hints;
    hints.check_call = true;
    MRBF_TRY(eval_model(ctx, M, n, M->C, V, nullptr, nullptr, hints));
    hipLaunchKernelGGL(residual_kernel, dim3(1), dim3(256), 0, ctx->stream, V, Y, n * k, scal);
    if (q > 0) {
        double *Pi, *T;
        MRBF_TRY(get_buf(ctx, S_PI, (size_t)n * q, &Pi));
        MRBF_TRY(get_buf(ctx, S_T2, (size_t)q * k, &T));
        MRBF_TRY(launch_poly_matrix(ctx, M->C, n, M->d, q, Pi, n));
        MRBF_TRY(tsmm_tn(ctx, n, q, k, 1.0, Pi, n, M->Wc, M->npad, 0.0, T, q));
        hipLaunchKernelGGL(max_abs_kernel, dim3(1), dim3(256), 0, ctx->stream, T, (int64_t)q * k, scal + 2);
    }
    MRBF_HIP(ctx, hipGetLastError());
    MRBF_HIP(ctx, hipMemcpyAsync(h, scal, 3 * sizeof(double), hipMemcpyDeviceToHost, ctx->stream));
    MRBF_HIP(ctx, hipEventRecord(e1, ctx->stream));
    return 0;
}
static int fit_check_finish(mrbf_ctx *ctx, const mrbf_model *M, const double *h, mrbf_fit_info *info, hipEvent_t e0, hipEvent_t e1) {
    info->rel_residual = std::sqrt(h[0]) / std::max(std::sqrt(h[1]), 1e-300);
    info->max_pitw = M->q > 0 ? h[2] : 0.0;
    MRBF_HIP(ctx, hipEventElapsedTime(&info->ms_check, e0, e1));
    return 0;
}
int fit_check(mrbf_ctx *ctx, mrbf_model *M, const double *Y, mrbf_fit_info *info) {
    double h_local[3] = {0, 0, 0};
    double *h = ctx->hpin ? reinterpret_cast<double *>(ctx->hpin + HPIN_RESIDUAL) : h_local;
    h[0] = h[1] = h[2] = 0.0;
    MRBF_TRY(fit_check_enqueue(ctx, M, Y, h, ctx->ev[0], ctx->ev[1]));
    MRBF_HIP(ctx, hipStreamSynchronize(ctx->stream));
    return fit_check_finish(ctx, M, h, info, ctx->ev[0], ctx->ev[1]);
}

int fit_model(mrbf_ctx *ctx, mrbf_model *M, const double *Y, mrbf_fit_info *info) {
    mrbf_fit_info local;
    if (!info) info = &local;
    std::memset(info, 0, sizeof(*info));
    info->n = (int32_t)M->n;
    info->q = M->q;
    info->rel_residual = NAN;
    info->max_pitw = NAN;
    const int order = cpd_order(M->kp.kid, M->kp.a, M->kp.b);
    int path = ctx->force_path;
    int small_nc_used = 0;
    bool checked = false;
    if (path == 0) path = (order <= M->deg + 1 && M->n > M->q) ? (M->q > 0 ? MRBF_PATH_PROJ_CHOL : MRBF_PATH_CHOL) : MRBF_PATH_LU;
    if (M->n < M->q) path = MRBF_PATH_MINNORM;
    if (path == MRBF_PATH_CHOL && M->q > 0) path = MRBF_PATH_PROJ_CHOL;
    if (path == MRBF_PATH_PROJ_CHOL && M->q == 0) path = MRBF_PATH_CHOL;
    if (path == MRBF_PATH_MINNORM) {
        MRBF_TRY(fit_minnorm(ctx, M, Y, info));
    } else if (path != MRBF_PATH_LU && !kp_nonsmooth(M->kp) && small_fit_applies(ctx, M->n, M->d, M->k, M->q, path)) {
        int not_pd = 0;
        MRBF_TRY(fit_small(ctx, M, Y, info, &not_pd, 0, &small_nc_used, &checked));
        if (not_pd) {
            info->fallbacks |= MRBF_FB_LU;
            if (ctx->force_path != 0)
                return fail(ctx, MRBF_ENOTPD, "Cholesky path forced but the matrix is not positive definite (info = %d)",
                            info->factor_info);
            path = MRBF_PATH_LU;
        }
    } else if (path != MRBF_PATH_LU) {
        int not_pd = 0, gave_up = 0;
        MRBF_TRY(fit_chol(ctx, M, Y, info, &not_pd, &gave_up));
        if (gave_up) {
            info->fallbacks |= MRBF_FB_CHOL_HOST_DRIVEN;
            MRBF_TRY(fit_chol(ctx, M, Y, info, &not_pd, &gave_up, 2));
            if (gave_up) return fail(ctx, MRBF_EHIP, "host-driven Cholesky reported a give-up code (0x%x)", info->giveup_code);
        }
        if (not_pd) {
            info->fallbacks |= MRBF_FB_LU;
            if (ctx->force_path != 0)
                return fail(ctx, MRBF_ENOTPD, "Cholesky path forced but the matrix is not positive definite (info = %d)",
                            info->factor_info);
            path = MRBF_PATH_LU;
        }
    }
    if (path == MRBF_PATH_LU) {
        if (small_lu_applies(ctx, M->n, M->d, M->k, M->q, M->kp))
            MRBF_TRY(fit_small_lu(ctx, M, Y, info));
        else
            MRBF_TRY(fit_lu(ctx, M, Y, info));
    }
    if (ctx->residual && !(checked && path != MRBF_PATH_LU)) MRBF_TRY(fit_check(ctx, M, Y, info));
    if (ctx->residual && small_nc_used > 1 && path != MRBF_PATH_LU && !(info->rel_residual < 1e-6)) {
        const double res_cluster = info->rel_residual;
        std::vector<double> wc((size_t)M->n * M->k);
        MRBF_HIP(ctx, hipMemcpy(wc.data(), M->W, wc.size() * sizeof(double), hipMemcpyDeviceToHost));
        int not_pd = 0, nc1 = 1;
        mrbf_fit_info again = *info;
        MRBF_TRY(fit_small(ctx, M, Y, &again, &not_pd, 1, &nc1));
        if (!not_pd) {
            MRBF_TRY(fit_check(ctx, M, Y, &again));
            std::vector<double> w1(wc.size());
            MRBF_HIP(ctx, hipMemcpy(w1.data(), M->W, w1.size() * sizeof(double), hipMemcpyDeviceToHost));
            if (std::memcmp(w1.data(), wc.data(), w1.size() * sizeof(double)) != 0 && (again.rel_residual < res_cluster || !(res_cluster == res_cluster)))
                ctx->small_nc = 1;
            *info = again;
        }
    }
    info->ms_total = info->ms_gram + info->ms_project + info->ms_factor + info->ms_solve;
    info->slow_launches = ctx->slow_launches;
    return 0;
}

}
```

Baseline: 175.7.

## Fuse RHS fetch into premul, split projection sums, widen eval combine and tail staging

Several independent changes. The RHS-row copy now runs inside the backsolve premul kernel as extra workgroups instead of a separate launch. The projection partial-sum reduction is split into its own coalesced vectorised kernel ahead of proj_reduce. eval_combine processes four points per block, one per wave, with vectorised gradient loads. tail_coeff stages G, LxInv and mean in LDS through dynamic shared memory. Each change aims to cut launch count or strided global reads, at the cost of more code paths and extra LDS use.

```diff
diff --git a/morbit.jl_amd/csrc/backsolve.hip b/morbit.jl_amd/csrc/backsolve.hip
--- a/morbit.jl_amd/csrc/backsolve.hip
+++ b/morbit.jl_amd/csrc/backsolve.hip
@@ -19,9 +19,22 @@
 
 __global__ __launch_bounds__(256) void premul_kernel(const double *__restrict__ L, int64_t lda, const double *__restrict__ linv_all,
                                                      double *__restrict__ Mbuf, int nb, unsigned *__restrict__ flags, int nflags,
-                                                     unsigned long long *__restrict__ xb, int nxb) {
+                                                     unsigned long long *__restrict__ xb, int nxb, const double *__restrict__ rhs_rows,
+                                                     double *__restrict__ Y, int64_t ldy, int k) {
     for (int e = blockIdx.x * 256 + threadIdx.x; e < nflags; e += gridDim.x * 256) flags[e] = 0u;
     for (int e = blockIdx.x * 256 + threadIdx.x; e < nxb; e += gridDim.x * 256) xb[e] = ~0ull;
+    if ((int)blockIdx.x >= 8 * (nb - 1)) {
+        const int64_t npad = (int64_t)nb * NB;
+        const int64_t idx = (int64_t)((int)blockIdx.x - 8 * (nb - 1)) * 256 + threadIdx.x;
+        const int64_t i = idx % npad;
+        const int l = 2 * (int)(idx / npad);
+        if (l < k) {
+            const v2d v = *(const gv2d *)(rhs_rows + l + i * lda);
+            Y[i + (int64_t)l * ldy] = v.x;
+            if (l + 1 < k) Y[i + (int64_t)(l + 1) * ldy] = v.y;
+        }
+        return;
+    }
     const int slab = blockIdx.x & 3, t = (blockIdx.x >> 2) & 1, j = blockIdx.x >> 3;
     const int i = j + 1 + t;
     if (i >= nb) return;
@@ -341,15 +354,18 @@
 }
 
 int backsolve_blocked(mrbf_ctx *ctx, int64_t npad, const double *L, int64_t lda, const double *linv_all, double *Y, int64_t ldy, int k);
+int launch_get_rhs_rows(mrbf_ctx *ctx, const double *rows, int64_t ld, int64_t npad, double *B, int64_t ldb, int k);
 
 int backsolve_persistent(mrbf_ctx *ctx, int64_t npad, const double *L, int64_t lda, const double *linv_all, double *Y, int64_t ldy, int k,
-                         int *status) {
+                         int *status, const double *rhs_rows) {
     using namespace bsolve;
     const int nb = (int)(npad / NB);
     static const int force_old = mrbf_env("MRBF_BACKSOLVE_LAUNCHES") ? atoi(mrbf_env("MRBF_BACKSOLVE_LAUNCHES")) : 0;
     const int ncu = ctx->ncu;
-    if (force_old || nb < 3 || nb > ncu || (lda & 1) || (reinterpret_cast<uintptr_t>(L) & 15))
+    if (force_old || nb < 3 || nb > ncu || (lda & 1) || (reinterpret_cast<uintptr_t>(L) & 15) || (reinterpret_cast<uintptr_t>(rhs_rows) & 15)) {
+        if (rhs_rows) MRBF_TRY(launch_get_rhs_rows(ctx, rhs_rows, lda, npad, Y, ldy, k));
         return backsolve_blocked(ctx, npad, L, lda, linv_all, Y, ldy, k);
+    }
     unsigned *flags;
     MRBF_TRY(get_buf(ctx, S_BSOLVE_FLAGS, (size_t)(nb + 1) * 32, &flags));
     const unsigned long long spin_ticks = (unsigned long long)std::max(1, ctx->spin_ms) * 100000ull;
@@ -357,8 +373,9 @@
     double *xb, *Mbuf;
     MRBF_TRY(get_buf(ctx, S_BSOLVE_X, (size_t)2 * nb * 4 * NB, &xb));
     MRBF_TRY(get_buf(ctx, S_BSOLVE_M, (size_t)nb * 2 * NB * NB, &Mbuf));
-    hipLaunchKernelGGL(premul_kernel, dim3((unsigned)(8 * (nb - 1))), dim3(256), 0, ctx->stream, L, lda, linv_all, Mbuf, nb, flags, (nb + 1) * 32,
-                       reinterpret_cast<unsigned long long *>(xb), 2 * nb * 4 * NB);
+    const int fetch_wgs = rhs_rows ? (int)((npad * ((k + 1) / 2) + 255) / 256) : 0;
+    hipLaunchKernelGGL(premul_kernel, dim3((unsigned)(8 * (nb - 1) + fetch_wgs)), dim3(256), 0, ctx->stream, L, lda, linv_all, Mbuf, nb, flags,
+                       (nb + 1) * 32, reinterpret_cast<unsigned long long *>(xb), 2 * nb * 4 * NB, rhs_rows, Y, ldy, k);
     static const bool want_stamps = mrbf_env("MRBF_BSOLVE_STAMPS") && atoi(mrbf_env("MRBF_BSOLVE_STAMPS")) != 0;
     long long *stamps = nullptr;
     if (want_stamps) {
diff --git a/morbit.jl_amd/csrc/common.hpp b/morbit.jl_amd/csrc/common.hpp
--- a/morbit.jl_amd/csrc/common.hpp
+++ b/morbit.jl_amd/csrc/common.hpp
@@ -36,7 +36,7 @@
     S_XC = 0, S_SQ, S_MEAN, S_PHI, S_PI, S_Q1, S_W1, S_G, S_R, S_TAU, S_RHS, S_T1, S_T2, S_IPIV, S_INFO,
     S_STAGE_A, S_STAGE_B, S_STAGE_C, S_STAGE_D, S_EVAL_E, S_EVAL_A, S_EVAL_J, S_EVAL_SA, S_EVAL_XC, S_EVAL_XSQ,
     S_OUT_A, S_OUT_B, S_CHOL_WS, S_MISC, S_MEGA_JOBS, S_MEGA_FLAGS, S_MEGA_WQ, S_MEGA_IT, S_BSOLVE_FLAGS, S_MEGA_TRACE, S_MEGA_JLOG,
-    S_T1W, S_PS_STATE, S_PS_STAT, S_PS_POLISH, S_BSOLVE_X, S_V0, S_QR_INV, S_DIAG_SCR, S_SMALL_WS, S_SMALL_DESC, S_SMALL_FLAGS, S_MEGA_STAT, S_BSOLVE_M, S_SMALL_CL, S_GW_PART, S_GW_RS, S_GW_GP, S_GW_M, S_CHECK_SCAL, S_TAIL_PART, S_PS_RANK, S_SD_IN, S_SD_OUT, S_SD_WS, S_NS_IN, S_NS_OUT, S_NS_WS, S_SD_STEP, S_SD_BATCH, S_AFF_BATCH, S_NS_BATCH, S_R4_BATCH, S_DB_BOX, S_DB_GATHER, S_DB_WS, S_SMALL_LU, S_EVAL_BATCH, S_HESS_WS, S_HESS_OUT, S_NSLOTS
+    S_T1W, S_PS_STATE, S_PS_STAT, S_PS_POLISH, S_BSOLVE_X, S_V0, S_QR_INV, S_DIAG_SCR, S_SMALL_WS, S_SMALL_DESC, S_SMALL_FLAGS, S_MEGA_STAT, S_BSOLVE_M, S_SMALL_CL, S_GW_PART, S_GW_RS, S_GW_GP, S_GW_M, S_CHECK_SCAL, S_TAIL_PART, S_PS_RANK, S_SD_IN, S_SD_OUT, S_SD_WS, S_NS_IN, S_NS_OUT, S_NS_WS, S_SD_STEP, S_SD_BATCH, S_AFF_BATCH, S_NS_BATCH, S_R4_BATCH, S_DB_BOX, S_DB_GATHER, S_DB_WS, S_SMALL_LU, S_EVAL_BATCH, S_HESS_WS, S_HESS_OUT, S_GW_SUM, S_MEAN_PART, S_NSLOTS
 };
 }
 
@@ -242,7 +242,9 @@
 int launch_cross_gram(mrbf_ctx *ctx, const double *X, int64_t m, const double *C, int64_t n, int d, const KP &kp, double *K);
 bool gram_w_applies(const mrbf_ctx *ctx, const mrbf_model *M);
 int launch_gram_w(mrbf_ctx *ctx, const mrbf_model *M, double *Phi, int64_t ld, double **Wpart_out, double **rspart_out, int *nseg_out);
-int launch_projection_small(mrbf_ctx *ctx, const mrbf_model *M, const double *Wpart, const double *rspart, int nseg, const double *linv,
+int launch_proj_sum(mrbf_ctx *ctx, const mrbf_model *M, const double *Wpart, const double *rspart, int nseg, double **Wsum_out,
+                    double **rsum_out);
+int launch_projection_small(mrbf_ctx *ctx, const mrbf_model *M, const double *Wsum, const double *rsum, const double *linv,
                             const double *Q1, double *W1, double *G, double *scal, int *flags, int K2, int skip, double *PA, double *PB,
                             double *v0);
 int eval_model(mrbf_ctx *ctx, const mrbf_model *M, int64_t m, const double *Xdev, double *vals_dev, double *jac_dev,
diff --git a/morbit.jl_amd/csrc/eval_fused.hip b/morbit.jl_amd/csrc/eval_fused.hip
--- a/morbit.jl_amd/csrc/eval_fused.hip
+++ b/morbit.jl_amd/csrc/eval_fused.hip
@@ -594,25 +594,47 @@
 }
 
 template <int KOUT>
-__global__ __launch_bounds__(128) void eval_combine_kernel(EvalDesc one, const EvalDesc *__restrict__ many, int l0, int D) {
+__global__ __launch_bounds__(256) void eval_combine_kernel(EvalDesc one, const EvalDesc *__restrict__ many, int l0, int D) {
     const EvalDesc &E = many ? many[blockIdx.y] : one;
-    const int64_t p = blockIdx.x, m = E.m, mpad = E.mpad;
-    if (p >= m) return;
+    const int lane = threadIdx.x & 63, wave = threadIdx.x >> 6;
+    const int64_t p = (int64_t)blockIdx.x * 4 + wave, m = E.m, mpad = E.mpad;
+    const bool active = p < m;
     const double *__restrict__ vpart = E.vpart, *__restrict__ sapart = E.sapart, *__restrict__ gpart = E.gpart;
     const double *__restrict__ Xq = E.Xq, *__restrict__ Xorig = E.X, *__restrict__ lam = E.lam;
     double *__restrict__ vals = E.vals, *__restrict__ jac = E.jac;
     const int nsplit = E.nsplit, d = E.d, k = E.k, q = E.q;
-    __shared__ double sa[KOUT], sv[KOUT];
-    __shared__ double pdot[KOUT][128];
-    const int tid = threadIdx.x;
-    if (tid < KOUT && l0 + tid < k) {
-        double v = 0.0, a = 0.0;
+    __shared__ double pdot[4][KOUT][128];
+    const int H = D >> 1;
+    const v2d zero2 = {0.0, 0.0};
+    v2d g[2], xq[2];
+    bool ok[2];
+#pragma unroll
+    for (int j = 0; j < 2; ++j) {
+        const int e2 = lane + 64 * j, l = e2 / H, t = 2 * (e2 % H);
+        ok[j] = active && l < KOUT && l0 + l < k && t < d;
+        g[j] = zero2;
+        xq[j] = zero2;
+        if (ok[j]) {
+            xq[j] = *(const v2d *)(Xq + p * D + t);
+            for (int s0 = 0; s0 < nsplit; s0 += 8) {
+                v2d x[8];
+#pragma unroll
+                for (int u = 0; u < 8; ++u)
+                    x[u] = s0 + u < nsplit ? *(const v2d *)(gpart + (((int64_t)(s0 + u) * mpad + p) * KOUT + l) * D + t) : zero2;
+#pragma unroll
+                for (int u = 0; u < 8; ++u)
+                    if (s0 + u < nsplit) g[j] += x[u];
+            }
+        }
+    }
+    double v = 0.0, a = 0.0;
+    if (active && lane < KOUT && l0 + lane < k) {
         for (int s0 = 0; s0 < nsplit; s0 += 8) {
             double xv[8], xa[8];
 #pragma unroll
             for (int u = 0; u < 8; ++u) {
-                xv[u] = s0 + u < nsplit ? vpart[((int64_t)(s0 + u) * mpad + p) * KOUT + tid] : 0.0;
-                xa[u] = s0 + u < nsplit ? sapart[((int64_t)(s0 + u) * mpad + p) * KOUT + tid] : 0.0;
+                xv[u] = s0 + u < nsplit ? vpart[((int64_t)(s0 + u) * mpad + p) * KOUT + lane] : 0.0;
+                xa[u] = s0 + u < nsplit ? sapart[((int64_t)(s0 + u) * mpad + p) * KOUT + lane] : 0.0;
             }
 #pragma unroll
             for (int u = 0; u < 8; ++u)
@@ -621,45 +643,49 @@
                     a += xa[u];
                 }
         }
-        sa[tid] = a;
-        sv[tid] = v;
     }
     if (vals && q > 1) {
 #pragma unroll
-        for (int l = 0; l < KOUT; ++l) {
-            double acc = 0.0;
-            if (l0 + l < k)
-                for (int t = tid; t < d; t += 128) acc = fma(lam[(int64_t)(t + 1) * k + l0 + l], Xorig[p * d + t], acc);
-            pdot[l][tid] = acc;
-        }
+        for (int l = 0; l < KOUT; ++l)
+#pragma unroll
+            for (int h = 0; h < 2; ++h) {
+                const int t0 = lane + 64 * h;
+                double acc = 0.0;
+                if (active && l0 + l < k)
+                    for (int t = t0; t < d; t += 128) acc = fma(lam[(int64_t)(t + 1) * k + l0 + l], Xorig[p * d + t], acc);
+                pdot[wave][l][t0] = acc;
+            }
     }
     __syncthreads();
-    if (vals && tid < KOUT && l0 + tid < k) {
-        double v = sv[tid];
-        if (q > 0) v += lam[l0 + tid];
+    if (vals && active && lane < KOUT && l0 + lane < k) {
+        if (q > 0) v += lam[l0 + lane];
         if (q > 1) {
             const int nt = d < 128 ? d : 128;
             double dsum = 0.0;
-            for (int t = 0; t < nt; ++t) dsum += pdot[tid][t];
+            for (int t = 0; t < nt; ++t) dsum += pdot[wave][lane][t];
             v += dsum;
         }
-        vals[p * k + l0 + tid] = v;
-    }
-    for (int e = tid; e < KOUT * d; e += blockDim.x) {
-        const int l = e / d, t = e % d;
-        if (l0 + l >= k) continue;
-        double g = 0.0;
-        for (int s0 = 0; s0 < nsplit; s0 += 8) {
-            double x[8];
-#pragma unroll
-            for (int u = 0; u < 8; ++u) x[u] = s0 + u < nsplit ? gpart[(((int64_t)(s0 + u) * mpad + p) * KOUT + l) * D + t] : 0.0;
-#pragma unroll
-            for (int u = 0; u < 8; ++u)
-                if (s0 + u < nsplit) g += x[u];
-        }
-        double v = fma(sa[l], Xq[p * D + t], -g);
-        if (q > 1) v += lam[(int64_t)(t + 1) * k + l0 + l];
-        jac[p * (int64_t)k * d + (int64_t)t * k + l0 + l] = v;
+        vals[p * k + l0 + lane] = v;
+    }
+    double sa[KOUT];
+#pragma unroll
+    for (int l = 0; l < KOUT; ++l) sa[l] = __shfl(a, l);
+#pragma unroll
+    for (int j = 0; j < 2; ++j) {
+        if (!ok[j]) continue;
+        const int e2 = lane + 64 * j, l = e2 / H, t = 2 * (e2 % H);
+        double sal = sa[0];
+#pragma unroll
+        for (int ll = 1; ll < KOUT; ++ll) sal = l == ll ? sa[ll] : sal;
+        double *o = jac + p * (int64_t)k * d + (int64_t)t * k + l0 + l;
+        double j0 = fma(sal, xq[j].x, -g[j].x);
+        if (q > 1) j0 += lam[(int64_t)(t + 1) * k + l0 + l];
+        o[0] = j0;
+        if (t + 1 < d) {
+            double j1 = fma(sal, xq[j].y, -g[j].y);
+            if (q > 1) j1 += lam[(int64_t)(t + 2) * k + l0 + l];
+            o[k] = j1;
+        }
     }
 }
 
@@ -772,7 +798,7 @@
         hipLaunchKernelGGL((eval_vals256_kernel<KID, FAST, KOUT>), dim3((grid.x + 1) / 2, grid.y, grid.z), dim3(512), 0, st, one, many, l0);
     }
     if constexpr (!FINAL && JAC)
-        hipLaunchKernelGGL(eval_combine_kernel<KOUT>, cgrid, dim3(128), 0, st, one, many, l0, D);
+        hipLaunchKernelGGL(eval_combine_kernel<KOUT>, dim3((cgrid.x + 3) / 4, cgrid.y), dim3(256), 0, st, one, many, l0, D);
     else if constexpr (!FINAL)
         hipLaunchKernelGGL(eval_combine_vals_kernel<KOUT>, dim3((cgrid.x + 3) / 4, cgrid.y), dim3(256), 0, st, one, many, l0);
     return 0;
diff --git a/morbit.jl_amd/csrc/gram_fused.hip b/morbit.jl_amd/csrc/gram_fused.hip
--- a/morbit.jl_amd/csrc/gram_fused.hip
+++ b/morbit.jl_amd/csrc/gram_fused.hip
@@ -220,8 +220,31 @@
     return acc;
 }
 
-__global__ __launch_bounds__(256) void proj_reduce_kernel(const double *__restrict__ Wpart, const double *__restrict__ rspart, int nseg,
-                                                          int64_t npad, int64_t n, int d, int q, const double *__restrict__ linv,
+__global__ __launch_bounds__(256) void proj_sum_kernel(const double *__restrict__ Wpart, const double *__restrict__ rspart, int nseg,
+                                                       int64_t npad, int64_t wblocks, double *__restrict__ Wsum,
+                                                       double *__restrict__ rsum) {
+    if ((int64_t)blockIdx.x >= wblocks) {
+        const int64_t r = ((int64_t)blockIdx.x - wblocks) * 256 + threadIdx.x;
+        if (r < npad) rsum[r] = sum_partials(rspart + r, nseg, npad);
+        return;
+    }
+    const int64_t o = ((int64_t)blockIdx.x * 256 + threadIdx.x) * 2;
+    const int64_t seg = 64 * npad;
+    v2d sv = {0.0, 0.0};
+    for (int s0 = 0; s0 < nseg; s0 += 8) {
+        v2d wv[8];
+#pragma unroll
+        for (int sgm = 0; sgm < 8; ++sgm) {
+            const v2d z = {0.0, 0.0};
+            wv[sgm] = s0 + sgm < nseg ? *(const v2d *)(Wpart + (int64_t)(s0 + sgm) * seg + o) : z;
+        }
+        sv += ((wv[0] + wv[1]) + (wv[2] + wv[3])) + ((wv[4] + wv[5]) + (wv[6] + wv[7]));
+    }
+    *(v2d *)(Wsum + o) = sv;
+}
+
+__global__ __launch_bounds__(256) void proj_reduce_kernel(const double *__restrict__ Wsum, const double *__restrict__ rsum, int64_t npad,
+                                                          int64_t n, int d, int q, const double *__restrict__ linv,
                                                           const double *__restrict__ Q1, double rsqrtn, double *__restrict__ W1,
                                                           double *__restrict__ Gp, double *__restrict__ trp) {
     __shared__ double Ws[64 * PJ_LS];
@@ -239,33 +262,18 @@
         const int a = g + 4 * u;
         qv[u] = (a < q && live) ? Q1[R0 + i + (int64_t)a * npad] : 0.0;
     }
-    const double rsv = (g == 0 && live) ? sum_partials(rspart + R0 + i, nseg, npad) * rsqrtn : 0.0;
+    const double rsv = (g == 0 && live) ? rsum[R0 + i] * rsqrtn : 0.0;
     if (q > 1) {
-        double lv[16];
+        double lv[16], wv[16];
 #pragma unroll
         for (int u = 0; u < 16; ++u) {
             const int e = tid + 256 * u, c = e & 63, t = e >> 6;
             lv[u] = (c < d && t <= c) ? linv[c + (int64_t)t * 128] : 0.0;
         }
 #pragma unroll
-        for (int half = 0; half < 2; ++half) {
-            double sv[8] = {0.0, 0.0, 0.0, 0.0, 0.0, 0.0, 0.0, 0.0};
-            for (int s0 = 0; s0 < nseg; s0 += 8) {
-                double wv[8][8];
-#pragma unroll
-                for (int u = 0; u < 8; ++u)
-#pragma unroll
-                    for (int sgm = 0; sgm < 8; ++sgm) {
-                        const int t = g * 16 + half * 8 + u;
-                        wv[u][sgm] = s0 + sgm < nseg ? Wpart[((int64_t)(s0 + sgm) * 64 + t) * npad + R0 + i] : 0.0;
-                    }
-#pragma unroll
-                for (int u = 0; u < 8; ++u)
-                    sv[u] += ((wv[u][0] + wv[u][1]) + (wv[u][2] + wv[u][3])) + ((wv[u][4] + wv[u][5]) + (wv[u][6] + wv[u][7]));
-            }
-#pragma unroll
-            for (int u = 0; u < 8; ++u) Ws[i * PJ_LS + (g * 16 + half * 8 + u)] = live ? sv[u] : 0.0;
-        }
+        for (int u = 0; u < 16; ++u) wv[u] = live ? Wsum[(int64_t)(g * 16 + u) * npad + R0 + i] : 0.0;
+#pragma unroll
+        for (int u = 0; u < 16; ++u) Ws[i * PJ_LS + (g * 16 + u)] = wv[u];
 #pragma unroll
         for (int u = 0; u < 16; ++u) {
             const int e = tid + 256 * u;
@@ -382,6 +390,18 @@
         const int a = g + 4 * u;
         qv[u] = (a < q && live) ? Q1[R0 + i + (int64_t)a * npad] : 0.0;
     }
+    constexpr int QT = PJ_QP / 16;
+    const int qt = (q + 15) >> 4;
+    const int iw = wave * 16 + l15;
+    const bool lw = R0 + iw < n;
+    double w1v[QT][4];
+#pragma unroll
+    for (int bt = 0; bt < QT; ++bt)
+#pragma unroll
+        for (int r = 0; r < 4; ++r) {
+            const int b = bt * 16 + l4 + 4 * r;
+            w1v[bt][r] = (b < q && lw) ? W1[R0 + iw + (int64_t)b * npad] : 0.0;
+        }
     constexpr int ME = (PJ_QP * PJ_LS + 255) / 256;
     double mv[ME];
 #pragma unroll
@@ -397,25 +417,24 @@
 #pragma unroll
     for (int u = 0; u < QA; ++u) Qs[i * PJ_LS + g + 4 * u] = qv[u];
     __syncthreads();
-    const int qq = q - skip, qt = (q + 15) >> 4, K = (q + 3) & ~3;
-#pragma unroll 1
-    for (int tile = wave; tile < qt * 4; tile += 4) {
-        const int bt = tile >> 2, it = tile & 3;
-        const v4d acc = pj_tile(Ms, Qs, bt, it, K, l15, l4);
-        const int ii = it * 16 + l15;
-        const bool lv = R0 + ii < n;
-        double w1[4], qb[4];
+    const int qq = q - skip, K = (q + 3) & ~3;
+#pragma unroll
+    for (int bt = 0; bt < QT; ++bt) {
+        if (bt >= qt) break;
+        const v4d acc = pj_tile(Ms, Qs, bt, wave, K, l15, l4);
+        const int ii = iw;
+        const bool lv = lw;
+        double qb[4];
 #pragma unroll
         for (int r = 0; r < 4; ++r) {
             const int b = bt * 16 + l4 + 4 * r;
-            w1[r] = (b < q && lv) ? W1[R0 + ii + (int64_t)b * npad] : 0.0;
             qb[r] = b < q ? Qs[ii * PJ_LS + b] : 0.0;
         }
 #pragma unroll
         for (int r = 0; r < 4; ++r) {
             const int b = bt * 16 + l4 + 4 * r;
             if (b >= q) continue;
-            const double v = lv ? w1[r] - acc[r] : 0.0;
+            const double v = lv ? w1v[bt][r] - acc[r] : 0.0;
             if (b >= skip) {
                 const int c = b - skip;
                 PA[R0 + ii + (int64_t)c * npad] = qb[r];
@@ -471,7 +490,22 @@
     return 0;
 }
 
-int launch_projection_small(mrbf_ctx *ctx, const mrbf_model *M, const double *Wpart, const double *rspart, int nseg, const double *linv,
+int launch_proj_sum(mrbf_ctx *ctx, const mrbf_model *M, const double *Wpart, const double *rspart, int nseg, double **Wsum_out,
+                    double **rsum_out) {
+    const int64_t npad = M->npad;
+    double *Wsum;
+    MRBF_TRY(get_buf(ctx, S_GW_SUM, (size_t)65 * npad, &Wsum));
+    double *rsum = Wsum + 64 * npad;
+    const int64_t wblocks = M->q > 1 ? npad / 8 : 0;
+    hipLaunchKernelGGL(proj_sum_kernel, dim3((unsigned)(wblocks + (npad + 255) / 256)), dim3(256), 0, ctx->stream, Wpart, rspart, nseg, npad,
+                       wblocks, Wsum, rsum);
+    MRBF_HIP(ctx, hipGetLastError());
+    *Wsum_out = Wsum;
+    *rsum_out = rsum;
+    return 0;
+}
+
+int launch_projection_small(mrbf_ctx *ctx, const mrbf_model *M, const double *Wsum, const double *rsum, const double *linv,
                             const double *Q1, double *W1, double *G, double *scal, int *flags, int K2, int skip, double *PA, double *PB,
                             double *v0) {
     const int64_t n = M->n, npad = M->npad;
@@ -480,7 +514,7 @@
     MRBF_TRY(get_buf(ctx, S_GW_GP, (size_t)nch * q * q + nch, &Gp));
     MRBF_TRY(get_buf(ctx, S_GW_M, (size_t)q * q, &Mh));
     double *trp = Gp + (size_t)nch * q * q;
-    hipLaunchKernelGGL(proj_reduce_kernel, dim3((unsigned)nch), dim3(256), 0, ctx->stream, Wpart, rspart, nseg, npad, n, M->d, q, linv, Q1,
+    hipLaunchKernelGGL(proj_reduce_kernel, dim3((unsigned)nch), dim3(256), 0, ctx->stream, Wsum, rsum, npad, n, M->d, q, linv, Q1,
                        1.0 / std::sqrt((double)n), W1, Gp, trp);
     hipLaunchKernelGGL(proj_shift_kernel, dim3((unsigned)((q * q + 255) / 256)), dim3(256), 0, ctx->stream, Gp, trp, nch, q,
                        (double)n * M->kp.phi0, (double)std::max<int64_t>(n - q, 1), G, Mh, scal, flags);
diff --git a/morbit.jl_amd/csrc/prep.hip b/morbit.jl_amd/csrc/prep.hip
--- a/morbit.jl_amd/csrc/prep.hip
+++ b/morbit.jl_amd/csrc/prep.hip
@@ -2,16 +2,30 @@
 
 namespace mrbf {
 
-__global__ void column_mean_kernel(const double *__restrict__ X, int64_t n, int d, double *__restrict__ mean) {
+__global__ __launch_bounds__(256) void column_slot_sums_kernel(const double *__restrict__ X, int64_t n, int d, double *__restrict__ part) {
+    const int64_t idx = (int64_t)blockIdx.x * 256 + threadIdx.x, step = (int64_t)256 * d, cnt = n * d;
+    if (idx >= step) return;
+    double s = 0.0;
+    int64_t o = idx;
+    for (; o + 15 * step < cnt; o += 16 * step) {
+        double v[16];
+#pragma unroll
+        for (int u = 0; u < 16; ++u) v[u] = X[o + u * step];
+#pragma unroll
+        for (int u = 0; u < 16; ++u) s += v[u];
+    }
+    for (; o < cnt; o += step) s += X[o];
+    part[idx] = s;
+}
+
+__global__ __launch_bounds__(256) void column_mean_kernel(const double *__restrict__ part, int64_t n, int d, double *__restrict__ mean) {
     __shared__ double red[256];
     const int t = blockIdx.x;
     if (t >= d) {
         if (threadIdx.x == 0) mean[t] = 0.0;
         return;
     }
-    double s = 0.0;
-    for (int64_t i = threadIdx.x; i < n; i += blockDim.x) s += X[i * d + t];
-    red[threadIdx.x] = s;
+    red[threadIdx.x] = part[(int64_t)threadIdx.x * d + t];
     __syncthreads();
     for (int w = 128; w > 0; w >>= 1) {
         if ((int)threadIdx.x < w) red[threadIdx.x] += red[threadIdx.x + w];
@@ -40,7 +54,10 @@
                       double *Xc, int64_t npad, int dpad, double *sq) {
     const double *mean = mean_or_null;
     if (!mean) {
-        hipLaunchKernelGGL(column_mean_kernel, dim3(dpad > d ? dpad : d), dim3(256), 0, ctx->stream, X, n, d, mean_out);
+        double *part;
+        MRBF_TRY(get_buf(ctx, S_MEAN_PART, (size_t)256 * d, &part));
+        hipLaunchKernelGGL(column_slot_sums_kernel, dim3((unsigned)d), dim3(256), 0, ctx->stream, X, n, d, part);
+        hipLaunchKernelGGL(column_mean_kernel, dim3(dpad > d ? dpad : d), dim3(256), 0, ctx->stream, part, n, d, mean_out);
         mean = mean_out;
     }
     const int rows_per_block = 4;
diff --git a/morbit.jl_amd/csrc/solve.hip b/morbit.jl_amd/csrc/solve.hip
--- a/morbit.jl_amd/csrc/solve.hip
+++ b/morbit.jl_amd/csrc/solve.hip
@@ -329,7 +329,7 @@
 
 int backsolve_blocked(mrbf_ctx *ctx, int64_t npad, const double *L, int64_t lda, const double *linv_all, double *Y, int64_t ldy, int k);
 int backsolve_persistent(mrbf_ctx *ctx, int64_t npad, const double *L, int64_t lda, const double *linv_all, double *Y, int64_t ldy, int k,
-                         int *status);
+                         int *status, const double *rhs_rows);
 int launch_update_lower(mrbf_ctx *ctx, const double *A, int64_t lda, const double *B, int64_t ldb, double *C, int64_t ldc, int64_t nt, int K,
                         const double *cvec, double cs, int64_t cn);
 int launch_pad_identity(mrbf_ctx *ctx, double *A, int64_t n, int64_t npad, int64_t ld);
@@ -345,12 +345,17 @@
     const int64_t i = idx / xt;
     A[(npad + l) + i * ld] = (l < k) ? B[i + (int64_t)l * npad] : 0.0;
 }
-__global__ void get_rhs_rows_kernel(const double *__restrict__ A, int64_t ld, int64_t npad, double *__restrict__ B, int k) {
+__global__ void get_rhs_rows_kernel(const double *__restrict__ rows, int64_t ld, int64_t npad, double *__restrict__ B, int64_t ldb, int k) {
     const int64_t idx = (int64_t)blockIdx.x * blockDim.x + threadIdx.x;
     if (idx >= npad * k) return;
     const int l = (int)(idx % k);
     const int64_t i = idx / k;
-    B[i + (int64_t)l * npad] = A[(npad + l) + i * ld];
+    B[i + (int64_t)l * ldb] = rows[l + i * ld];
+}
+int launch_get_rhs_rows(mrbf_ctx *ctx, const double *rows, int64_t ld, int64_t npad, double *B, int64_t ldb, int k) {
+    hipLaunchKernelGGL(get_rhs_rows_kernel, dim3(nblk(npad * k)), dim3(256), 0, ctx->stream, rows, ld, npad, B, ldb, k);
+    MRBF_HIP(ctx, hipGetLastError());
+    return 0;
 }
 __global__ void xc_to_tall_kernel(const double *__restrict__ Xc, int64_t n, int d, int dpad, double *__restrict__ Tall, int64_t lt,
                                   int64_t dq) {
@@ -516,48 +521,86 @@
     }
 }
 
-__global__ __launch_bounds__(1024) void tail_coeff_kernel(const double *__restrict__ part, int nch, int q, int k, int d, const double *__restrict__ T1,
-                                                         const double *__restrict__ G, double cg, const double *__restrict__ LxInv,
-                                                         double sqrtn, const double *__restrict__ mean, double *__restrict__ T2,
-                                                         double *__restrict__ lam_out) {
-    __shared__ double t2[129 * 16], zz[129 * 16], xx[129 * 16];
-    const int tid = threadIdx.x, nthr = blockDim.x;
-    for (int e = tid; e < 2 * k * q; e += nthr) {
+constexpr int TC_THR = 1024, TC_GST = 5, TC_LST = 4;
+static bool tail_coeff_stages(int q, int k, int d) {
+    return q * q <= TC_GST * TC_THR && d * d <= TC_LST * TC_THR &&
+           ((size_t)3 * k * q + (size_t)q * q + (size_t)d * (d + 1) / 2 + d) * sizeof(double) <= (size_t)64 << 10;
+}
+__global__ __launch_bounds__(TC_THR) void tail_coeff_kernel(const double *__restrict__ part, int nch, int q, int k, int d, const double *__restrict__ T1,
+                                                           const double *__restrict__ G, double cg, const double *__restrict__ LxInv,
+                                                           double sqrtn, const double *__restrict__ mean, double *__restrict__ T2,
+                                                           double *__restrict__ lam_out, int stage) {
+    extern __shared__ double tcs[];
+    const int kq = k * q;
+    double *t2 = tcs, *zz = tcs + kq, *xx = tcs + 2 * kq, *Gs = tcs + 3 * kq, *Ls = Gs + q * q, *ms = Ls + d * (d + 1) / 2;
+    const int tid = threadIdx.x, nthr = TC_THR;
+    double gst[TC_GST], lst[TC_LST], mst = 0.0;
+    if (stage) {
+#pragma unroll
+        for (int u = 0; u < TC_GST; ++u) {
+            const int e = tid + TC_THR * u;
+            gst[u] = e < q * q ? G[e] : 0.0;
+        }
+#pragma unroll
+        for (int u = 0; u < TC_LST; ++u) {
+            const int e = tid + TC_THR * u, j = d > 0 ? e / d : 0, i = d > 0 ? e % d : 0;
+            lst[u] = (e < d * d && i >= j) ? LxInv[i + (int64_t)j * 128] : 0.0;
+        }
+        if (tid < d) mst = mean[tid];
+    }
+    const double t1first = tid < kq ? T1[(tid % q) + (int64_t)(tid / q) * q] : 0.0;
+    for (int e = tid; e < 2 * kq; e += nthr) {
         double sv = 0.0;
         for (int c0 = 0; c0 < nch; c0 += 32) {
             double v[32];
 #pragma unroll
-            for (int u = 0; u < 32; ++u) v[u] = c0 + u < nch ? part[(size_t)(c0 + u) * 2 * k * q + e] : 0.0;
+            for (int u = 0; u < 32; ++u) v[u] = c0 + u < nch ? part[(size_t)(c0 + u) * 2 * kq + e] : 0.0;
 #pragma unroll
             for (int u = 0; u < 32; ++u) sv += v[u];
         }
-        if (e < k * q)
+        if (e < kq)
             t2[e] = sv;
         else
-            zz[e - k * q] = sv;
+            zz[e - kq] = sv;
+    }
+    if (stage) {
+#pragma unroll
+        for (int u = 0; u < TC_GST; ++u) {
+            const int e = tid + TC_THR * u;
+            if (e < q * q) Gs[e] = gst[u];
+        }
+#pragma unroll
+        for (int u = 0; u < TC_LST; ++u) {
+            const int e = tid + TC_THR * u, j = d > 0 ? e / d : 0, i = d > 0 ? e % d : 0;
+            if (e < d * d && i >= j) Ls[j * d - j * (j - 1) / 2 + (i - j)] = lst[u];
+        }
+        if (tid < d) ms[tid] = mst;
     }
     __syncthreads();
-    for (int e = tid; e < k * q; e += nthr) {
+    for (int e = tid; e < kq; e += nthr) {
         const int l = e / q, a = e % q;
+        const double t1v = e == tid ? t1first : T1[a + (int64_t)l * q];
+        const double *gcol = stage ? Gs + a * q : G + (int64_t)a * q;
         double corr = 0.0;
         for (int b0 = 0; b0 < q; b0 += 16) {
             double gv[16];
 #pragma unroll
-            for (int u = 0; u < 16; ++u) gv[u] = b0 + u < q ? G[b0 + u + (int64_t)a * q] : 0.0;
+            for (int u = 0; u < 16; ++u) gv[u] = b0 + u < q ? gcol[b0 + u] : 0.0;
 #pragma unroll
             for (int u = 0; u < 16; ++u) corr = fma(gv[u], b0 + u < q ? t2[l * q + b0 + u] : 0.0, corr);
         }
-        zz[e] = T1[a + (int64_t)l * q] - zz[e] + cg * corr;
+        zz[e] = t1v - zz[e] + cg * corr;
         T2[a + (int64_t)l * q] = t2[e];
     }
     __syncthreads();
     for (int e = tid; e < k * d; e += nthr) {
         const int l = e / d, j = e % d;
+        const double *lcol = stage ? Ls + (j * d - j * (j - 1) / 2 - j) : LxInv + (int64_t)j * 128;
         double acc = 0.0;
         for (int i0 = j; i0 < d; i0 += 16) {
             double iv[16];
 #pragma unroll
-            for (int u = 0; u < 16; ++u) iv[u] = i0 + u < d ? LxInv[i0 + u + (int64_t)j * 128] : 0.0;
+            for (int u = 0; u < 16; ++u) iv[u] = i0 + u < d ? lcol[i0 + u] : 0.0;
 #pragma unroll
             for (int u = 0; u < 16; ++u) acc = fma(iv[u], i0 + u < d ? zz[l * q + 1 + i0 + u] : 0.0, acc);
         }
@@ -566,18 +609,19 @@
     __syncthreads();
     if (tid < k) {
         const int l = tid;
+        const double *mp = stage ? ms : mean;
         double dsum = 0.0;
         for (int t0 = 1; t0 < q; t0 += 16) {
             double mv[16];
 #pragma unroll
-            for (int u = 0; u < 16; ++u) mv[u] = t0 + u < q ? mean[t0 + u - 1] : 0.0;
+            for (int u = 0; u < 16; ++u) mv[u] = t0 + u < q ? mp[t0 + u - 1] : 0.0;
 #pragma unroll
             for (int u = 0; u < 16; ++u) dsum = fma(mv[u], t0 + u < q ? xx[l * q + t0 + u] : 0.0, dsum);
         }
         xx[l * q] = zz[l * q] / sqrtn - dsum;
     }
     __syncthreads();
-    for (int e = tid; e < k * q; e += nthr) lam_out[(e % q) + (int64_t)(e / q) * q] = xx[e];
+    for (int e = tid; e < kq; e += nthr) lam_out[(e % q) + (int64_t)(e / q) * q] = xx[e];
 }
 
 __global__ __launch_bounds__(256) void tail_apply_kernel(const double *__restrict__ Bw, int64_t ldb, const double *__restrict__ Q1, int64_t ldq,
@@ -686,6 +730,8 @@
     else
         MRBF_TRY(launch_gram(ctx, ctx->gram_mode, M->C, M->Xc, M->sq, n, M->npad, M->d, M->dpad, M->kp, Phi, ld));
     MRBF_HIP(ctx, hipEventRecord(ctx->ev[1], ctx->stream));
+    double *Wsum = nullptr, *rsum = nullptr;
+    if (fused) MRBF_TRY(launch_proj_sum(ctx, M, Wpart, rspart, nseg, &Wsum, &rsum));
     if (side) MRBF_HIP(ctx, hipStreamWaitEvent(ctx->stream, ctx->evx[1], 0));
     if (fused) {
         const int skip = (q > 1 && round_up(2 * (q - 1), 16) < round_up(2 * q, 16)) ? 1 : 0;
@@ -694,7 +740,7 @@
         MRBF_TRY(get_buf(ctx, S_STAGE_C, (size_t)npad * K2, &PA));
         MRBF_TRY(get_buf(ctx, S_STAGE_D, (size_t)npad * K2, &PB));
         if (skip) MRBF_TRY(get_buf(ctx, S_V0, (size_t)npad, &v0));
-        MRBF_TRY(launch_projection_small(ctx, M, Wpart, rspart, nseg, LxInv, Q1, Wm, G, scal, dinfo, K2, skip, PA, PB, v0));
+        MRBF_TRY(launch_projection_small(ctx, M, Wsum, rsum, LxInv, Q1, Wm, G, scal, dinfo, K2, skip, PA, PB, v0));
         MRBF_TRY(launch_update_lower(ctx, PA, npad, PB, npad, Phi, ld, npad / 128, K2, v0, 1.0 / std::sqrt((double)n), n));
     } else if (q > 0) {
         MRBF_TRY(symm_panel(ctx, n, npad, q, Phi, ld, Q1, npad, Wm, npad, true, 1.0 / std::sqrt((double)n)));
@@ -735,11 +781,12 @@
     if (q > 0) MRBF_TRY(get_buf(ctx, S_T1W, (size_t)q * k, &T1w));
     auto solve_tail = [&](bool persistent) -> int {
         if (builtin) {
-            hipLaunchKernelGGL(get_rhs_rows_kernel, dim3(nblk(npad * k)), dim3(256), 0, ctx->stream, Phi, ld, npad, B, k);
-            if (persistent)
-                MRBF_TRY(backsolve_persistent(ctx, npad, Phi, ld, linv_all, B, npad, k, dinfo + 3));
-            else
+            if (persistent) {
+                MRBF_TRY(backsolve_persistent(ctx, npad, Phi, ld, linv_all, B, npad, k, dinfo + 3, Phi + npad));
+            } else {
+                MRBF_TRY(launch_get_rhs_rows(ctx, Phi + npad, ld, npad, B, npad, k));
                 MRBF_TRY(backsolve_blocked(ctx, npad, Phi, ld, linv_all, B, npad, k));
+            }
         } else {
             MRBF_BLAS(ctx, rocsolver_dpotrs(ctx->blas, rocblas_fill_lower, (int)n, k, Phi, (int)ld, B, (int)npad));
         }
@@ -750,8 +797,11 @@
             MRBF_TRY(get_buf(ctx, S_T2, (size_t)q * k, &T2));
             MRBF_TRY(get_buf(ctx, S_TAIL_PART, (size_t)nch * 2 * k * q, &part));
             hipLaunchKernelGGL(tail_dots_kernel, dim3((unsigned)nch), dim3(256), 0, ctx->stream, B, npad, Q1, Wm, npad, n, q, k, part);
-            hipLaunchKernelGGL(tail_coeff_kernel, dim3(1), dim3(1024), 0, ctx->stream, part, nch, q, k, q > 1 ? d : 0, T1, G, fused ? 1.0 : 0.5, LxInv,
-                               std::sqrt((double)n), M->mean, T2, T1w);
+            const int dt = q > 1 ? d : 0;
+            const bool stage = tail_coeff_stages(q, k, dt);
+            const size_t lds = ((size_t)3 * k * q + (stage ? (size_t)q * q + (size_t)dt * (dt + 1) / 2 + dt : 0)) * sizeof(double);
+            hipLaunchKernelGGL(tail_coeff_kernel, dim3(1), dim3(TC_THR), lds, ctx->stream, part, nch, q, k, dt, T1, G, fused ? 1.0 : 0.5, LxInv,
+                               std::sqrt((double)n), M->mean, T2, T1w, stage ? 1 : 0);
             hipLaunchKernelGGL(tail_apply_kernel, dim3((unsigned)nch), dim3(256), 0, ctx->stream, B, npad, Q1, npad, T2, T1w, n, M->npad, q, k, M->W,
                                M->Wc, M->lam);
             MRBF_HIP(ctx, hipGetLastError());
```

After: 177.4 (median of 6 runs). Within noise of the previous version (+1.0%).
